# XiYe20/NPVP

Hardware: AMD Instinct MI355X
Metric: predictor train frames/sec (higher is better)
Workload: dtype f32 (two-term fp16 split of amax-scaled operands, 3 MFMAs per product, fp32 accumulate: fp32-grade; small GEMMs: three-term bf16 split)

## Files before the change

include/npvp_hip.h:

```cpp
#ifndef NPVP_HIP_H
#define NPVP_HIP_H
#include <stddef.h>
#ifdef __cplusplus
extern "C" {
#endif

typedef void* npvp_stream_t;

int npvp_version(void);
const char* npvp_last_error(void);
long long npvp_launch_count(void);
void* npvp_stream_create_low_priority(int* least, int* greatest);
int npvp_stream_destroy(void* stream);
void* npvp_event_create(void);
int npvp_event_record(void* event, void* stream);
float npvp_event_elapsed_ms(void* event0, void* event1);
int npvp_event_destroy(void* event);

long long npvp_graph_node_counts(void* graph, long long* counts, long long* memset_bytes, int max_memsets);

long long npvp_gemm_workspace_bytes(int M, int N, int K);
int npvp_gemm_kernel_id(int a_kc, int b_kc, int M, int N, int K, int precision, int has_planes);
int npvp_gemm_route(int a_kc, int b_kc, int M, int N, int K, int precision, int has_planes, int plain_epilogue, int* out4);
int npvp_gemm_f32(int a_kc, int b_kc, int M, int N, int K, const float* A, long long lda, const float* B, long long ldb,
                  float* C, long long ldc, const float* bias, int act, const float* aux_in, float* aux_out,
                  const float* residual, long long ldr, float drop_p, int drop_mode, int drop_g1, int drop_g2,
                  const unsigned long long* seed, unsigned int salt, float alpha, int precision, float* colsum_a,
                  const void* b_pre, int accumulate, float* rowstats, const float* a_amax, const float* b_amax,
                  float* c_amax, unsigned int* range_flag, float adrop_p, int adrop_g1, int adrop_g2, unsigned int adrop_salt,
                  void* workspace, long long ws_bytes, npvp_stream_t stream);
int npvp_frame_stats_finalize(const float* part, int parts_per_frame, float values_per_part, float* mean, float* rstd,
                              int frames, float eps, npvp_stream_t stream);
int npvp_split_weight(const float* w, long long ld, int N, int K, void* F, void* D, npvp_stream_t stream);
int npvp_split_weights_batched(const void* desc, int count, npvp_stream_t stream);
int npvp_amax(const float* x, long long rows, long long cols, long long ld, float* slot, npvp_stream_t stream);

typedef struct npvp_reduce_job {
  const float* ws; float* out; long long ldc; int M, N, splits, accum; float alpha; int blocks; const float* cs_part; float* cs_out;
} npvp_reduce_job_t;
int npvp_wgrad_f16_chainable(int M, int N, int K);
long long npvp_wgrad_f16_chain_workspace_bytes(int M, int N, int K);
int npvp_wgrad_f16_chained(int M, int N, int K, const float* dy, long long lda, const float* x, long long ldb, float* dw,
                           long long ldc, float* db, int accumulate, const float* a_amax, const float* b_amax,
                           unsigned int* range_flag, float adrop_p, int adrop_g1, int adrop_g2, unsigned int adrop_salt,
                           const unsigned long long* seed, const void* prev_job, void* my_job, void* workspace,
                           long long ws_bytes, npvp_stream_t stream);
int npvp_splitk_reduce_job(const void* job, npvp_stream_t stream);
int npvp_splitk_reduce_multi(const void* jobs, int n, npvp_stream_t stream);
int npvp_linear_bwd_f16_takes(int R, int N, int K);
int npvp_linear_bwd_f16(int R, int N, int K, const float* dy, long long ldy, const float* dy_amax, const void* w_planes_d,
                        const float* w_amax, float* dx, long long ldx, int act, const float* aux_in, const float* residual,
                        long long ldr, float drop_p, int drop_mode, int drop_g1, int drop_g2, unsigned int drop_salt, float* dx_amax,
                        const float* x, long long ldxx, const float* x_amax, float* dw, long long ldw, float* db,
                        unsigned int* range_flag, float adrop_p, int adrop_g1, int adrop_g2, unsigned int adrop_salt,
                        const unsigned long long* seed, const void* prev_job, void* my_job, void* workspace, long long ws_bytes,
                        npvp_stream_t stream);
int npvp_split_weight_f16(const float* w, long long ld, int N, int K, void* F, void* D, float* amax_slot, npvp_stream_t stream);
int npvp_split_weights_f16(const void* desc, int count, void* amax_table, long long amax_bytes, npvp_stream_t stream);

int npvp_layernorm_fwd(const float* x, const float* w, const float* b, float* y, float* mean, float* rstd, long long rows,
                       int C, float eps, int relu, float* y_amax, npvp_stream_t stream);
long long npvp_layernorm_bwd_workspace_bytes(long long rows, int C);
int npvp_layernorm_bwd(const float* dy, const float* x, const float* w, const float* b, const float* mean,
                       const float* rstd, float* dx, float* dw, float* db, long long rows, int C, int relu,
                       const float* dres ,
                       int accumulate , float* dx_amax,
                       void* workspace, long long ws_bytes, npvp_stream_t stream);
int npvp_layernorm_bwd_reduce(const void* workspace, float* dw, float* db, long long rows, int C, int accumulate,
                              npvp_stream_t stream);

int npvp_layernorm_bwd_reduce_job(const void* workspace, float* dw, float* db, long long rows, int C, int accumulate, void* job);
int npvp_frameln_act_bwd_reduce_job(const void* workspace, float* dw, float* db, int frames, int per_frame, int accumulate, void* job);
int npvp_mlpdw_mid_bwd_reduce_job(const void* workspace, float* gw, float* gb, int frames, int Ch, void* job);
int npvp_sum_rows_multi(const void* jobs, int n, npvp_stream_t stream);

int npvp_layernorm_nchw_fwd(const float* x, const float* w, const float* b, float* out_nchw, float* mean, float* rstd, int frames,
                            int P, int C, float eps, int relu, npvp_stream_t stream);

int npvp_frame_stats(const float* x, const float* add, float* mean, float* rstd, int frames, int T, int per_frame,
                     float eps, npvp_stream_t stream);
int npvp_posfuse_fwd(const float* x, const float* add, const float* beta, const float* gamma, float* y, float* mean,
                     float* rstd, int N, int T, int per_frame, float eps, float* y_amax, npvp_stream_t stream);
int npvp_ln_posfuse_fwd(const float* x, const float* lw, const float* lb, float ln_eps, float* y1, float* ln_mean, float* ln_rstd,
// ... 5 lines not shown
                     int accumulate, void* workspace, long long ws_bytes , npvp_stream_t stream);

int npvp_posfuse_instance_fwd(const float* x, const float* add, const float* beta, const float* gamma, float* y, float* mean,
                              float* rstd, int N, int T, int P, int C, float eps, float* y_amax, npvp_stream_t stream);
int npvp_posfuse_instance_bwd(const float* dy, const float* x, const float* add, const float* gamma, const float* mean,
                              const float* rstd, float* du, float* dyxh, int N, int T, int P, int C, npvp_stream_t stream);

int npvp_frameln_act_fwd(const float* h, const float* mean, const float* rstd, const float* w, const float* b,
                         const float* res, float* out, int frames, int per_frame, float drop_p, unsigned int salt,
                         float dp_p, unsigned int dp_salt, int frames_per_sample, const unsigned long long* seed,
                         float* out_amax, npvp_stream_t stream);
long long npvp_frameln_act_bwd_workspace_bytes(int frames, int per_frame);
int npvp_frameln_act_bwd(const float* dout, const float* h, const float* mean, const float* rstd, const float* w,
                         const float* b, float* dh, float* dw, float* db, int frames, int per_frame, float drop_p,
                         unsigned int salt, float dp_p, unsigned int dp_salt, int frames_per_sample,
                         const unsigned long long* seed, int accumulate ,
                         float* dh_amax, void* workspace, long long ws_bytes, npvp_stream_t stream);
int npvp_frameln_act_bwd_reduce(const void* workspace, float* dw, float* db, int frames, int per_frame, int accumulate,
                                npvp_stream_t stream);
int npvp_dwconv3x3(const float* a, const float* wt, const float* bias, float* out, int frames, int H, int W, int Ch,
                   int flip, npvp_stream_t stream);
int npvp_dwconv3x3_stats(const float* a, const float* wt, const float* bias, float* out, float* mean, float* rstd, int frames,
                         int H, int W, int Ch, float eps, void* workspace, long long ws_bytes, npvp_stream_t stream);
int npvp_mlpdw_mid_fwd(const float* h1, const float* mean1, const float* rstd1, const float* w1n, const float* b1n,
                       const float* wt, const float* bias, float* h2, float* mean2, float* rstd2, int frames, int H, int W,
                       int Ch, float eps, void* workspace, long long ws_bytes, npvp_stream_t stream);
int npvp_mlpdw_mid_fwd_parts(const float* h1, const float* part1, int J1, float nb1, float* mean1, float* rstd1, const float* w1n,
                             const float* b1n, const float* wt, const float* bias, float* h2, float* part2, int frames, int H,
                             int W, int Ch, float eps, npvp_stream_t stream);
int npvp_frameln_act_fwd_parts(const float* h, const float* part, int J, float nb, float eps, float* mean, float* rstd,
                               const float* w, const float* b, const float* res, float* out, int frames, int per_frame,
                               float drop_p, unsigned int salt, float dp_p, unsigned int dp_salt, int frames_per_sample,
                               const unsigned long long* seed, float* out_amax, npvp_stream_t stream);
long long npvp_mlpdw_mid_bwd_workspace_bytes(int frames, int Ch);
int npvp_mlpdw_mid_bwd(const float* dh2, const float* h1, const float* mean1, const float* rstd1, const float* w1n,
                       const float* b1n, const float* wt, float* da1, float* dwt_db, float* psum, int frames, int H, int W,
                       int Ch, int accumulate, void* workspace, long long ws_bytes, npvp_stream_t stream);
int npvp_mlpdw_mid_bwd_reduce(const void* workspace, float* dwt_db, int frames, int Ch, int accumulate, npvp_stream_t stream);
int npvp_mlpdw_mid_bwd_reduce_into(const void* workspace, float* gw, float* gb, int frames, int Ch, npvp_stream_t stream);
int npvp_mlpdw_mid_bwd_n2(const float* da2, const float* h2, const float* mean2, const float* rstd2, const float* w2n,
                          const float* b2n, const float* psum2, int nparts2, float drop_p, unsigned int salt,
                          const unsigned long long* seed, const float* h1, const float* mean1, const float* rstd1,
                          const float* w1n, const float* b1n, const float* wt, float* da1, float* dwt_db, float* psum, int frames,
                          int H, int W, int Ch, int accumulate, void* workspace, long long ws_bytes, npvp_stream_t stream);
int npvp_frameln_act_bwd_pgrad(const float* dout, const float* h, const float* mean, const float* rstd, const float* w,
                               const float* b, float* psum, float* dw, float* db, int frames, int per_frame, float drop_p,
                               unsigned int salt, float dp_p, unsigned int dp_salt, int frames_per_sample,
                               const unsigned long long* seed, int accumulate, void* workspace, long long ws_bytes,
                               npvp_stream_t stream);
int npvp_frameln_act_bwd_apply(const float* dout, const float* h, const float* mean, const float* rstd, const float* w,
                               const float* b, const float* psum, int nparts, float* dh, float* dw, float* db, int frames,
                               int per_frame, int accumulate, float* dh_amax, void* workspace, long long ws_bytes,
                               npvp_stream_t stream);

int npvp_im2col3x3(const float* in, float* out, int frames, int H, int W, int C, int col2im, npvp_stream_t stream);
long long npvp_dwconv3x3_wgrad_workspace_bytes(int frames, int Ch);
int npvp_dwconv3x3_wgrad(const float* a, const float* dout, float* dwt_db, int frames, int H, int W, int Ch,
                         void* workspace, long long ws_bytes, npvp_stream_t stream);

int npvp_attn_fwd(const float* q, long long ld_q, const float* k, long long ld_k, const float* v, long long ld_v, float* o,
                  long long ld_o, int mode, int dim0, int P, int W, int ws, int Tq, int Tk, int heads, int head_dim,
                  int mask_mode, float drop_p, const unsigned long long* seed, unsigned int salt, float* o_amax,
                  npvp_stream_t stream);
int npvp_attn_bwd(const float* q, long long ld_q, const float* k, long long ld_k, const float* v, long long ld_v,
                  const float* go, long long ld_o, float* dq, long long ld_dq, float* dk, long long ld_dk, float* dv,
                  long long ld_dv, int mode, int dim0, int P, int W, int ws, int Tq, int Tk, int heads, int head_dim,
                  int mask_mode, float drop_p, const unsigned long long* seed, unsigned int salt, float* dq_amax,
                  float* dk_amax , float* dv_amax,
                  npvp_stream_t stream);
int npvp_attn_long_fwd(const float* q, long long ld_q, const float* k, long long ld_k, const float* v, long long ld_v, float* o,
                       long long ld_o, int mode, int dim0, int P, int W, int ws, int Tq, int Tk, int heads, int head_dim,
                       int mask_mode, float drop_p, const unsigned long long* seed, unsigned int salt, float* o_amax,
                       npvp_stream_t stream);
long long npvp_attn_long_bwd_workspace_bytes(int mode, int dim0, int P, int W, int ws, int Tq, int Tk, int heads);
int npvp_attn_long_bwd(const float* q, long long ld_q, const float* k, long long ld_k, const float* v, long long ld_v,
                       const float* go, long long ld_o, float* dq, long long ld_dq, float* dk, long long ld_dk, float* dv,
                       long long ld_dv, int mode, int dim0, int P, int W, int ws, int Tq, int Tk, int heads, int head_dim,
                       int mask_mode, float drop_p, const unsigned long long* seed, unsigned int salt, float* dq_amax,
                       float* dk_amax , float* dv_amax, void* workspace, long long ws_bytes,
                       npvp_stream_t stream);

int npvp_drop_apply(const float* x, float* out, long long rows, int ncols, float p, int mode, int g1, int g2,
                    const unsigned long long* seed, unsigned int salt, float* out_amax, npvp_stream_t stream);
int npvp_transpose(const float* in, float* out, int batch, int R, int C, npvp_stream_t stream);
int npvp_dwtb_accumulate(const float* dwtb, float* gw, float* gb, int C, npvp_stream_t stream);
int npvp_dwtb_build(const float* w, const float* b, float* wtb, int C, npvp_stream_t stream);
int npvp_reduce_mid(const float* in, float* out, int A, int B, long long Cc, float scale, int accumulate, npvp_stream_t stream);
int npvp_broadcast_mid(const float* in, float* out, int A, int B, long long Cc, float scale, npvp_stream_t stream);

long long npvp_colsum_workspace_bytes(long long rows, int N);
int npvp_colsum(const float* x, long long rows, int N, long long ld, float* out, int accumulate ,
                void* workspace, long long ws_bytes, npvp_stream_t stream);

int npvp_l1_mean(const float* a, const float* b, long long n, float lam, float* out, void* workspace, long long ws_bytes,
                 npvp_stream_t stream);
int npvp_l1_mean_bwd(const float* a, const float* b, long long n, const float* gout, float lam, float* da, npvp_stream_t stream);
int npvp_sum_all(const float* x, long long n, float* out, void* workspace, long long ws_bytes, npvp_stream_t stream);

int npvp_grad_norm_clip(const float* g, long long n, float max_norm, float* out2, void* workspace, long long ws_bytes,
                        npvp_stream_t stream);
int npvp_adamw_step(float* p, float* g, float* m, float* v, long long n, const float* hyper, float beta1, float beta2,
                    float eps, float weight_decay, const float* clip, long long clip_begin, long long clip_end,
                    int write_back_grad, npvp_stream_t stream);

long long npvp_sqdiff_workspace_bytes(int N, long long per_image);
int npvp_sqdiff_per_image(const float* x, const float* y, int N, long long per_image, float data_range, float scale, float* out,
// ... 56 lines not shown
```

npvp_amd/_lib.py:

```python
import ctypes
import os

_HERE = os.path.dirname(os.path.abspath(__file__))
LIB_PATH = os.path.join(_HERE, "libnpvp_hip.so")

c_int, c_ll, c_f, c_u, c_p = ctypes.c_int, ctypes.c_longlong, ctypes.c_float, ctypes.c_uint, ctypes.c_void_p

SIGNATURES = {
    "npvp_version": (c_int, []),
    "npvp_last_error": (ctypes.c_char_p, []),
    "npvp_launch_count": (c_ll, []),
    "npvp_dp_unique_id": (c_int, [c_p]),
    "npvp_dp_init": (c_int, [c_int, c_int, c_p]),
    "npvp_dp_world": (c_int, []),
    "npvp_dp_rank": (c_int, []),
    "npvp_dp_allreduce_async": (c_int, [c_p, c_ll, c_p]),
    "npvp_dp_wait": (c_int, [c_p]),
    "npvp_dp_finalize": (c_int, []),
    "npvp_stream_create_low_priority": (c_p, [c_p, c_p]),
    "npvp_stream_destroy": (c_int, [c_p]),
    "npvp_event_create": (c_p, []),
    "npvp_event_record": (c_int, [c_p, c_p]),
    "npvp_event_elapsed_ms": (c_f, [c_p, c_p]),
    "npvp_event_destroy": (c_int, [c_p]),
    "npvp_graph_node_counts": (c_ll, [c_p, c_p, c_p, c_int]),
    "npvp_gemm_workspace_bytes": (c_ll, [c_int, c_int, c_int]),
    "npvp_gemm_kernel_id": (c_int, [c_int, c_int, c_int, c_int, c_int, c_int, c_int]),
    "npvp_gemm_route": (c_int, [c_int, c_int, c_int, c_int, c_int, c_int, c_int, c_int, c_p]),
    "npvp_gemm_f32": (c_int, [c_int, c_int, c_int, c_int, c_int, c_p, c_ll, c_p, c_ll, c_p, c_ll, c_p, c_int, c_p, c_p,
                              c_p, c_ll, c_f, c_int, c_int, c_int, c_p, c_u, c_f, c_int, c_p, c_p, c_int, c_p, c_p, c_p, c_p, c_p,
                              c_f, c_int, c_int, c_u, c_p, c_ll, c_p]),
    "npvp_amax": (c_int, [c_p, c_ll, c_ll, c_ll, c_p, c_p]),
    "npvp_wgrad_f16_chainable": (c_int, [c_int, c_int, c_int]),
    "npvp_wgrad_f16_chain_workspace_bytes": (c_ll, [c_int, c_int, c_int]),
    "npvp_wgrad_f16_chained": (c_int, [c_int, c_int, c_int, c_p, c_ll, c_p, c_ll, c_p, c_ll, c_p, c_int, c_p, c_p, c_p, c_f, c_int, c_int,
                                       c_u, c_p, c_p, c_p, c_p, c_ll, c_p]),
    "npvp_splitk_reduce_job": (c_int, [c_p, c_p]),
    "npvp_splitk_reduce_multi": (c_int, [c_p, c_int, c_p]),
    "npvp_linear_bwd_f16_takes": (c_int, [c_int, c_int, c_int]),
    "npvp_linear_bwd_f16": (c_int, [c_int, c_int, c_int, c_p, c_ll, c_p, c_p, c_p, c_p, c_ll, c_int, c_p, c_p, c_ll, c_f, c_int, c_int, c_int,
                                    c_u, c_p, c_p, c_ll, c_p, c_p, c_ll, c_p, c_p, c_f, c_int, c_int, c_u, c_p, c_p, c_p, c_p, c_ll, c_p]),
    "npvp_split_weight_f16": (c_int, [c_p, c_ll, c_int, c_int, c_p, c_p, c_p, c_p]),
    "npvp_split_weights_f16": (c_int, [c_p, c_int, c_p, c_ll, c_p]),
    "npvp_frame_stats_finalize": (c_int, [c_p, c_int, c_f, c_p, c_p, c_int, c_f, c_p]),
    "npvp_split_weight": (c_int, [c_p, c_ll, c_int, c_int, c_p, c_p, c_p]),
    "npvp_split_weights_batched": (c_int, [c_p, c_int, c_p]),
    "npvp_layernorm_fwd": (c_int, [c_p, c_p, c_p, c_p, c_p, c_p, c_ll, c_int, c_f, c_int, c_p, c_p]),
    "npvp_layernorm_bwd_workspace_bytes": (c_ll, [c_ll, c_int]),
    "npvp_layernorm_bwd": (c_int, [c_p, c_p, c_p, c_p, c_p, c_p, c_p, c_p, c_p, c_ll, c_int, c_int, c_p, c_int, c_p, c_p, c_ll, c_p]),
    "npvp_layernorm_bwd_reduce": (c_int, [c_p, c_p, c_p, c_ll, c_int, c_int, c_p]),
    "npvp_layernorm_bwd_reduce_job": (c_int, [c_p, c_p, c_p, c_ll, c_int, c_int, c_p]),
    "npvp_frameln_act_bwd_reduce_job": (c_int, [c_p, c_p, c_p, c_int, c_int, c_int, c_p]),
    "npvp_mlpdw_mid_bwd_reduce_job": (c_int, [c_p, c_p, c_p, c_int, c_int, c_p]),
    "npvp_sum_rows_multi": (c_int, [c_p, c_int, c_p]),
    "npvp_layernorm_nchw_fwd": (c_int, [c_p, c_p, c_p, c_p, c_p, c_p, c_int, c_int, c_int, c_f, c_int, c_p]),
    "npvp_frameln_act_bwd_reduce": (c_int, [c_p, c_p, c_p, c_int, c_int, c_int, c_p]),
    "npvp_frame_stats": (c_int, [c_p, c_p, c_p, c_p, c_int, c_int, c_int, c_f, c_p]),
    "npvp_posfuse_fwd": (c_int, [c_p, c_p, c_p, c_p, c_p, c_p, c_p, c_int, c_int, c_int, c_f, c_p, c_p]),
    "npvp_posfuse_instance_fwd": (c_int, [c_p, c_p, c_p, c_p, c_p, c_p, c_p, c_int, c_int, c_int, c_int, c_f, c_p, c_p]),
    "npvp_posfuse_instance_bwd": (c_int, [c_p, c_p, c_p, c_p, c_p, c_p, c_p, c_p, c_int, c_int, c_int, c_int, c_p]),
    "npvp_ln_posfuse_fwd": (c_int, [c_p, c_p, c_p, c_f, c_p, c_p, c_p, c_p, c_p, c_p, c_p, c_p, c_p, c_int, c_int, c_int, c_int, c_f,
                                    c_p, c_p, c_p]),
    "npvp_posfuse_bwd_fused": (c_int, [c_int, c_int, c_int]),
    "npvp_posfuse_bwd": (c_int, [c_p, c_p, c_p, c_p, c_p, c_p, c_p, c_p, c_p, c_p, c_int, c_int, c_int, c_int, c_p, c_ll, c_p]),
    "npvp_frameln_act_fwd": (c_int, [c_p, c_p, c_p, c_p, c_p, c_p, c_p, c_int, c_int, c_f, c_u, c_f, c_u, c_int, c_p, c_p, c_p]),
    "npvp_frameln_act_bwd_workspace_bytes": (c_ll, [c_int, c_int]),
    "npvp_frameln_act_bwd": (c_int, [c_p, c_p, c_p, c_p, c_p, c_p, c_p, c_p, c_p, c_int, c_int, c_f, c_u, c_f, c_u, c_int,
                                     c_p, c_int, c_p, c_p, c_ll, c_p]),
    "npvp_dwconv3x3": (c_int, [c_p, c_p, c_p, c_p, c_int, c_int, c_int, c_int, c_int, c_p]),
    "npvp_dwconv3x3_stats": (c_int, [c_p, c_p, c_p, c_p, c_p, c_p, c_int, c_int, c_int, c_int, c_f, c_p, c_ll, c_p]),
    "npvp_mlpdw_mid_fwd": (c_int, [c_p, c_p, c_p, c_p, c_p, c_p, c_p, c_p, c_p, c_p, c_int, c_int, c_int, c_int, c_f, c_p, c_ll, c_p]),
    "npvp_mlpdw_mid_fwd_parts": (c_int, [c_p, c_p, c_int, c_f, c_p, c_p, c_p, c_p, c_p, c_p, c_p, c_p, c_int, c_int, c_int, c_int, c_f, c_p]),
    "npvp_frameln_act_fwd_parts": (c_int, [c_p, c_p, c_int, c_f, c_f, c_p, c_p, c_p, c_p, c_p, c_p, c_int, c_int, c_f, c_u, c_f, c_u, c_int,
                                           c_p, c_p, c_p]),
    "npvp_mlpdw_mid_bwd_workspace_bytes": (c_ll, [c_int, c_int]),
    "npvp_mlpdw_mid_bwd": (c_int, [c_p, c_p, c_p, c_p, c_p, c_p, c_p, c_p, c_p, c_p, c_int, c_int, c_int, c_int, c_int, c_p, c_ll, c_p]),
    "npvp_mlpdw_mid_bwd_reduce": (c_int, [c_p, c_p, c_int, c_int, c_int, c_p]),
    "npvp_mlpdw_mid_bwd_reduce_into": (c_int, [c_p, c_p, c_p, c_int, c_int, c_p]),
    "npvp_mlpdw_mid_bwd_n2": (c_int, [c_p, c_p, c_p, c_p, c_p, c_p, c_p, c_int, c_f, c_u, c_p, c_p, c_p, c_p, c_p, c_p, c_p, c_p, c_p,
                                      c_p, c_int, c_int, c_int, c_int, c_int, c_p, c_ll, c_p]),
    "npvp_frameln_act_bwd_pgrad": (c_int, [c_p, c_p, c_p, c_p, c_p, c_p, c_p, c_p, c_p, c_int, c_int, c_f, c_u, c_f, c_u, c_int,
                                           c_p, c_int, c_p, c_ll, c_p]),
    "npvp_frameln_act_bwd_apply": (c_int, [c_p, c_p, c_p, c_p, c_p, c_p, c_p, c_int, c_p, c_p, c_p, c_int, c_int, c_int, c_p, c_p, c_ll, c_p]),
    "npvp_im2col3x3": (c_int, [c_p, c_p, c_int, c_int, c_int, c_int, c_int, c_p]),
    "npvp_dwconv3x3_wgrad_workspace_bytes": (c_ll, [c_int, c_int]),
    "npvp_dwconv3x3_wgrad": (c_int, [c_p, c_p, c_p, c_int, c_int, c_int, c_int, c_p, c_ll, c_p]),
    "npvp_attn_fwd": (c_int, [c_p, c_ll, c_p, c_ll, c_p, c_ll, c_p, c_ll, c_int, c_int, c_int, c_int, c_int, c_int, c_int,
                              c_int, c_int, c_int, c_f, c_p, c_u, c_p, c_p]),
    "npvp_attn_bwd": (c_int, [c_p, c_ll, c_p, c_ll, c_p, c_ll, c_p, c_ll, c_p, c_ll, c_p, c_ll, c_p, c_ll, c_int, c_int,
                              c_int, c_int, c_int, c_int, c_int, c_int, c_int, c_int, c_f, c_p, c_u, c_p, c_p, c_p, c_p]),
    "npvp_attn_long_fwd": (c_int, [c_p, c_ll, c_p, c_ll, c_p, c_ll, c_p, c_ll, c_int, c_int, c_int, c_int, c_int, c_int, c_int,
                                   c_int, c_int, c_int, c_f, c_p, c_u, c_p, c_p]),
    "npvp_attn_long_bwd_workspace_bytes": (c_ll, [c_int, c_int, c_int, c_int, c_int, c_int, c_int, c_int]),
    "npvp_attn_long_bwd": (c_int, [c_p, c_ll, c_p, c_ll, c_p, c_ll, c_p, c_ll, c_p, c_ll, c_p, c_ll, c_p, c_ll, c_int, c_int,
                                   c_int, c_int, c_int, c_int, c_int, c_int, c_int, c_int, c_f, c_p, c_u, c_p, c_p, c_p, c_p, c_ll, c_p]),
    "npvp_drop_apply": (c_int, [c_p, c_p, c_ll, c_int, c_f, c_int, c_int, c_int, c_p, c_u, c_p, c_p]),
    "npvp_transpose": (c_int, [c_p, c_p, c_int, c_int, c_int, c_p]),
    "npvp_dwtb_accumulate": (c_int, [c_p, c_p, c_p, c_int, c_p]),
    "npvp_dwtb_build": (c_int, [c_p, c_p, c_p, c_int, c_p]),
    "npvp_reduce_mid": (c_int, [c_p, c_p, c_int, c_int, c_ll, c_f, c_int, c_p]),
    "npvp_broadcast_mid": (c_int, [c_p, c_p, c_int, c_int, c_ll, c_f, c_p]),
    "npvp_colsum_workspace_bytes": (c_ll, [c_ll, c_int]),
    "npvp_colsum": (c_int, [c_p, c_ll, c_int, c_ll, c_p, c_int, c_p, c_ll, c_p]),
    "npvp_grad_norm_clip": (c_int, [c_p, c_ll, c_f, c_p, c_p, c_ll, c_p]),
    "npvp_l1_mean": (c_int, [c_p, c_p, c_ll, c_f, c_p, c_p, c_ll, c_p]),
    "npvp_l1_mean_bwd": (c_int, [c_p, c_p, c_ll, c_p, c_f, c_p, c_p]),
    "npvp_sum_all": (c_int, [c_p, c_ll, c_p, c_p, c_ll, c_p]),
    "npvp_adamw_step": (c_int, [c_p, c_p, c_p, c_p, c_ll, c_p, c_f, c_f, c_f, c_f, c_p, c_ll, c_ll, c_int, c_p]),
    "npvp_sqdiff_workspace_bytes": (c_ll, [c_int, c_ll]),
    "npvp_sqdiff_per_image": (c_int, [c_p, c_p, c_int, c_ll, c_f, c_f, c_p, c_p, c_ll, c_p]),
    "npvp_ssim_workspace_bytes": (c_ll, [c_int, c_int, c_int, c_int]),
    "npvp_u8hwc_to_f32chw": (c_int, [c_p, c_p, c_ll, c_int, c_int, c_int, c_p, c_p, c_p]),
    "npvp_bias_act": (c_int, [c_p, c_p, c_p, c_p, c_ll, c_ll, c_int, c_int, c_int, c_p]),
    "npvp_act_bwd": (c_int, [c_p, c_p, c_p, c_ll, c_int, c_p]),
    "npvp_bn_workspace_bytes": (c_int, [c_int]),
    "npvp_bn_stats": (c_int, [c_p, c_ll, c_ll, c_int, c_int, c_p, c_p, c_ll, c_p]),
    "npvp_bn_act_apply": (c_int, [c_p, c_p, c_p, c_p, c_p, c_ll, c_f, c_f, c_p, c_p, c_ll, c_ll, c_int, c_int, c_int, c_p, c_p, c_p, c_p]),
    "npvp_bn_act_bwd": (c_int, [c_p, c_p, c_p, c_p, c_p, c_p, c_ll, c_ll, c_int, c_int, c_int, c_int, c_p, c_p, c_p, c_p, c_ll, c_p]),
    "npvp_bn_act_apply_sync": (c_int, [c_p, c_p, c_p, c_p, c_p, c_f, c_f, c_p, c_p, c_ll, c_ll, c_int, c_int, c_int, c_p, c_p, c_p, c_p]),
    "npvp_bn_bwd_sums": (c_int, [c_p, c_p, c_p, c_p, c_p, c_p, c_ll, c_ll, c_int, c_int, c_int, c_p, c_p, c_p, c_p, c_ll, c_p]),
    "npvp_bn_act_bwd_apply": (c_int, [c_p, c_p, c_p, c_p, c_p, c_p, c_p, c_p, c_ll, c_ll, c_int, c_int, c_int, c_p, c_p]),
    "npvp_reflect_pad": (c_int, [c_p, c_p, c_int, c_int, c_int, c_int, c_int, c_int, c_int, c_p]),
    "npvp_nonlocal_attn_fwd": (c_int, [c_p, c_ll, c_p, c_ll, c_p, c_ll, c_p, c_ll, c_p, c_int, c_int, c_int, c_int, c_int, c_p]),
    "npvp_nonlocal_attn_bwd": (c_int, [c_p, c_ll, c_p, c_ll, c_p, c_ll, c_p, c_ll, c_p, c_p, c_p, c_ll, c_p, c_ll, c_p, c_ll, c_int, c_int,
                                       c_int, c_int, c_int, c_p]),
    "npvp_nonlocal_attn_grid_fwd": (c_int, [c_p, c_ll, c_p, c_ll, c_p, c_ll, c_p, c_ll, c_p, c_int, c_int, c_int, c_int, c_int, c_p]),
    "npvp_nonlocal_attn_grid_bwd": (c_int, [c_p, c_ll, c_p, c_ll, c_p, c_ll, c_p, c_ll, c_p, c_p, c_p, c_ll, c_p, c_ll, c_p, c_ll, c_int,
                                            c_int, c_int, c_int, c_int, c_p]),
    "npvp_ssim_per_image": (c_int, [c_p, c_p, c_int, c_int, c_int, c_int, c_p, c_int, c_p, c_p, c_ll, c_p]),
}

_lib = None


def lib():
    global _lib
# ... 39 lines not shown
```

npvp_amd/csrc/common.h:

```cpp
#pragma once
#include <hip/hip_runtime.h>
#include <stdint.h>

#define NPVP_OK 0
#define NPVP_ERR_ARG (-1)
#define NPVP_ERR_LAUNCH (-2)
#define NPVP_ERR_WORKSPACE (-3)

extern "C" void npvp_set_error(const char* msg);

extern "C" long long npvp_launch_count(void);
namespace npvp { extern long long g_launches; }
#define NPVP_LAUNCH(...)                                                    \
  do {                                                                      \
    __atomic_fetch_add(&npvp::g_launches, 1ll, __ATOMIC_RELAXED);           \
    hipLaunchKernelGGL(__VA_ARGS__);                                        \
  } while (0)

#define NPVP_CHECK_ARG(cond, msg)                    \
  do {                                               \
    if (!(cond)) {                                   \
      npvp_set_error(msg);                           \
      return NPVP_ERR_ARG;                           \
    }                                                \
// ... 134 lines not shown
__host__ __device__ __forceinline__ uint32_t mix32(uint32_t h) {
  h ^= h >> 16; h *= 0x85ebca6bu;
  h ^= h >> 13; h *= 0xc2b2ae35u;
  h ^= h >> 16;
  return h;
}
__host__ __device__ __forceinline__ uint32_t rng_u32(uint64_t seed, uint32_t salt, uint64_t idx) {
  const uint32_t k0 = mix32((uint32_t)seed ^ mix32(salt * 0x9e3779b9u + 0x7f4a7c15u));
  const uint32_t k1 = mix32((uint32_t)(seed >> 32) + mix32(salt ^ 0x85ebca6bu));
  const uint32_t h = mix32((uint32_t)idx ^ k0);
  return mix32(h + k1 + (uint32_t)(idx >> 32) * 0x9e3779b9u);
}
__device__ __forceinline__ float drop_scale(uint64_t seed, uint32_t salt, uint64_t idx, uint32_t thresh, float inv_keep) {
  return rng_u32(seed, salt, idx) >= thresh ? inv_keep : 0.f;
}
__host__ __device__ __forceinline__ uint32_t drop_threshold(float p) {
  double t = (double)p * 4294967296.0;
  if (t < 0) t = 0;
  if (t > 4294967295.0) t = 4294967295.0;
  return (uint32_t)t;
}

struct DropSpec {
  unsigned int thresh; float inv_keep; unsigned int salt; int mode; int g1; int g2;
  unsigned int m1, m2; int s1, s2;
};
__host__ __device__ __forceinline__ void div_magic(unsigned int d, unsigned int& m, int& s) {
  int l = 0;
  while (l < 31 && (1u << l) < d) ++l;
  s = 31 + l;
  m = (unsigned int)(((1ull << s) + d - 1ull) / d);
}
__device__ __forceinline__ unsigned int div_by_magic(unsigned int n, unsigned int m, int s) {
  return (unsigned int)(((unsigned long long)n * m) >> s);
}
__device__ __forceinline__ unsigned int drop_group(const DropSpec& d, long long row) {
  const unsigned int q1 = div_by_magic((unsigned int)row, d.m1, d.s1);
  return q1 - div_by_magic(q1, d.m2, d.s2) * (unsigned int)d.g2;
}
__device__ __forceinline__ float drop_spec_scale(const DropSpec& d, uint64_t seed, long long row, int col, int ncols) {
  const uint64_t key = d.mode == 0 ? (uint64_t)row * (uint64_t)ncols + (uint64_t)col : (uint64_t)drop_group(d, row);
  return rng_u32(seed, d.salt, key) >= d.thresh ? d.inv_keep : 0.f;
}
inline DropSpec make_drop_spec(float p, unsigned int salt, int mode, int g1, int g2) {
  DropSpec d;
  d.thresh = p > 0.f ? drop_threshold(p) : 0u;
  d.inv_keep = p > 0.f ? 1.f / (1.f - p) : 1.f;
  d.salt = salt; d.mode = mode; d.g1 = g1 > 0 ? g1 : 1; d.g2 = g2 > 0 ? g2 : 1;
  div_magic((unsigned int)d.g1, d.m1, d.s1);
  div_magic((unsigned int)d.g2, d.m2, d.s2);
  return d;
}

__device__ __forceinline__ float4 ld4(const float* p) { return *reinterpret_cast<const float4*>(p); }
__device__ __forceinline__ void st4(float* p, float4 v) { *reinterpret_cast<float4*>(p) = v; }

}
```

npvp_amd/csrc/gemm.h:

```cpp
#pragma once
#include <type_traits>
#include "common.h"

namespace npvp {

typedef float f32x16 __attribute__((ext_vector_type(16)));
typedef __bf16 bf16x8 __attribute__((ext_vector_type(8)));
typedef __bf16 bf16x4 __attribute__((ext_vector_type(4)));

struct ReduceJob {
  const float* ws; float* out; long long ldc; int M, N, splits, accum; float alpha; int blocks; const float* cs_part; float* cs_out;
};

struct GemmParams {
  const float* A; const float* B; float* C;
  const float* bias;
  const float* residual;
  float* aux_out;
  const float* aux_in;
  float* rowstats;
  float* colsum;
  const unsigned long long* seed;
  long long lda, ldb, ldc, ldr;
  int M, N, K;
  int act;
  DropSpec drop;
  DropSpec adrop;
  int tiles_m, tiles_n;
  int splits;
  float alpha;
  const void* b_pre;
  long long b_pre_plane;
  int colgroups;
  int accum;
  const float* a_amax; const float* b_amax; float* c_amax;
  unsigned int* range_flag;
  ReduceJob prev;
};

__device__ __forceinline__ void splitk_reduce_body(const ReduceJob& j, int bid, int nblocks, float& cmax) {
  const long long total4 = (long long)j.M * j.N / 4, cs4 = j.cs_out ? j.M / 4 : 0;
  for (long long i = (long long)bid * 256 + threadIdx.x; i < total4 + cs4; i += (long long)nblocks * 256) {
    if (i >= total4) {
      const long long e = (i - total4) * 4;
      float4 s = make_float4(0.f, 0.f, 0.f, 0.f);
      for (int zz = 0; zz < j.splits; ++zz) {
        const float4 v = ld4(j.cs_part + (long long)zz * j.M + e);
        s.x += v.x; s.y += v.y; s.z += v.z; s.w += v.w;
      }
      if (j.accum) { const float4 o = ld4(j.cs_out + e); s.x += o.x; s.y += o.y; s.z += o.z; s.w += o.w; }
      st4(j.cs_out + e, s);
      continue;
    }
    const long long e = i * 4;
    const int m = (int)(e / j.N), n = (int)(e - (long long)m * j.N);
    float4 s = make_float4(0.f, 0.f, 0.f, 0.f);
    for (int zz = 0; zz < j.splits; ++zz) {
      const float4 v = ld4(j.ws + (long long)zz * j.M * j.N + e);
      s.x += v.x; s.y += v.y; s.z += v.z; s.w += v.w;
    }
    s.x *= j.alpha; s.y *= j.alpha; s.z *= j.alpha; s.w *= j.alpha;
    if (j.accum) { const float4 o = ld4(j.out + (long long)m * j.ldc + n); s.x += o.x; s.y += o.y; s.z += o.z; s.w += o.w; }
    st4(j.out + (long long)m * j.ldc + n, s);
    cmax = amax4(cmax, s);
  }
}

__device__ __forceinline__ void store_colsum(const GemmParams& p, long long idx, float v) {
  p.colsum[idx] = (p.accum && p.splits == 1) ? p.colsum[idx] + v : v;
}

constexpr int EPI_LD = 36;
constexpr int EPI_FLOATS = 32 * EPI_LD;

__device__ __forceinline__ void epi_transpose(const f32x16& acc, float* scr, int lane, float4 (&v)[4]) {
  const int r = lane & 31, h = lane >> 5;
#pragma unroll
  for (int g = 0; g < 16; ++g) scr[(((g & 3) + 8 * (g >> 2)) + 4 * h) * EPI_LD + r] = acc[g];
  const int rr = lane >> 3, cq = lane & 7;
#pragma unroll
// ... 236 lines not shown
```

npvp_amd/csrc/gemm.hip:

```cpp
#include "gemm.h"
#include "partials.h"
#include <type_traits>

namespace npvp {

constexpr int BM = 128, BN = 128, BK = 32, GEMM_THREADS = 256;

template <bool KC> struct Stager;

template <> struct Stager<true> {
  static constexpr int LD = 129;
  float4 r[4];
  __device__ __forceinline__ void load(const float* src, long long ld, int row0, int nrows, int k0) {
    const int t = threadIdx.x;
    const int kc = (t & 7) * 4;
#pragma unroll
    for (int i = 0; i < 4; ++i) {
      const int row = row0 + (t >> 3) + 32 * i;
      r[i] = (row < nrows) ? ld4(src + (long long)row * ld + k0 + kc) : make_float4(0.f, 0.f, 0.f, 0.f);
    }
  }
  __device__ __forceinline__ void store(float* s) const {
    const int t = threadIdx.x;
    const int kc = (t & 7) * 4;
// ... 443 lines not shown
  const int M = f.M, N = f.N, K = f.K;
  const bool want_h = f.precision == 6;
  const int precision = want_h ? 4 : f.precision;
  int s128 = pick_splits(M, N, K);
  if (s128 > 1 && (!f.plain || f.ws_bytes < npvp_gemm_workspace_bytes(M, N, K))) s128 = 1;
  const bool planes_ok = f.planes && f.a_kc && K % 16 == 0 && N % 8 == 0;
  const bool wgrad = !f.a_kc && !f.b_kc && f.plain && !f.rowstats;
  auto fits = [&](int s) { return s == 1 || (s > 1 && f.ws_bytes >= splitk_workspace_bytes(s, M, N)); };
  GemmPlan pl = {precision == 0 ? 0 : 1, 0, s128, 0, false};
  int v = 0, s = 0;
  if (want_h && planes_ok && f.amax && (v = gemm_f16_variant(M, N, K)) != 0) {
    pl.id = v == 1 ? 5 : 7; pl.variant = v; pl.splits = 1; pl.planes = true;
  } else if (want_h && wgrad && f.amax && fits(s = f16_wgrad_splits(M, N, K))) {
    pl.id = 6; pl.splits = s;
  } else if (!want_h && precision == 4 && planes_ok && s128 == 1 && (v = wide_variant(M, N, K)) != 0) {
    pl.id = v == 1 ? 2 : 4; pl.variant = v; pl.planes = true;
  } else if (precision == 4 && wgrad && fits(s = wide_wgrad_splits(M, N, K))) {
    pl.id = 3; pl.splits = s;
  } else {
    pl.planes = !want_h && precision == 4 && planes_ok && s128 == 1 && !f.rowstats;
  }
  pl.steps = K / pl.splits / (precision == 0 ? BK : 16);
  return pl;
}

static GemmPlan plan_query(int a_kc, int b_kc, int M, int N, int K, int precision, int has_planes, bool plain) {
  return plan_gemm(GemmFacts{a_kc, b_kc, M, N, K, precision, has_planes != 0, plain, true, false, npvp_gemm_workspace_bytes(M, N, K)});
}

extern "C" int npvp_gemm_kernel_id(int a_kc, int b_kc, int M, int N, int K, int precision, int has_planes) {
  return plan_query(a_kc, b_kc, M, N, K, precision, has_planes, true).id;
}

extern "C" int npvp_gemm_route(int a_kc, int b_kc, int M, int N, int K, int precision, int has_planes, int plain_epilogue, int* out4) {
  NPVP_CHECK_ARG(out4 && M > 0 && N > 0 && K > 0, "gemm_route: empty problem or no result array");
  NPVP_CHECK_ARG(precision == 0 || precision == 4 || precision == 5 || precision == 6, "gemm_route: precision must be 0, 4, 5 or 6");
  NPVP_CHECK_ARG(K % BK == 0 && M % 4 == 0 && N % 4 == 0 && !(a_kc == 0 && b_kc == 1), "gemm_route: not a problem npvp_gemm_f32 accepts");
  const GemmPlan r = plan_query(a_kc, b_kc, M, N, K, precision, has_planes, plain_epilogue != 0);
  out4[0] = r.id; out4[1] = r.variant; out4[2] = r.splits; out4[3] = r.steps;
  return NPVP_OK;
}

static int finish_splitk(const GemmParams& p, float* C, long long ldc, float* colsum_a, hipStream_t stream) {
  const long long total4 = (long long)p.M * p.N / 4;
  int blocks = (int)((total4 + 255) / 256); if (blocks > 2048) blocks = 2048;
  const bool cs_here = colsum_a && ((uintptr_t)colsum_a % 16) == 0;
  NPVP_LAUNCH(splitk_reduce_kernel, dim3(blocks), dim3(256), 0, stream, (const float*)p.C, C, p.M, p.N, ldc, p.splits, p.alpha,
              p.accum, cs_here ? (const float*)p.colsum : nullptr, cs_here ? colsum_a : nullptr, p.c_amax);
  NPVP_CHECK_LAUNCH();
  if (!colsum_a || cs_here) return NPVP_OK;
  return finish_partials(make_partials(p.colsum, 0, p.splits, p.splits, p.M, colsum_a, p.accum).job, 0, stream, "gemm: column-sum reduce launch failed");
}

extern "C" int npvp_gemm_f32(int a_kc, int b_kc, int M, int N, int K, const float* A, long long lda, const float* B,
                             long long ldb, float* C, long long ldc, const float* bias, int act, const float* aux_in,
                             float* aux_out, const float* residual, long long ldr, float drop_p, int drop_mode,
                             int drop_g1, int drop_g2, const unsigned long long* seed, unsigned int salt, float alpha,
                             int precision, float* colsum_a, const void* b_pre, int accumulate, float* rowstats,
                             const float* a_amax, const float* b_amax, float* c_amax, unsigned int* range_flag,
                             float adrop_p, int adrop_g1, int adrop_g2, unsigned int adrop_salt,
                             void* workspace, long long ws_bytes, hipStream_t stream) {
  NPVP_CHECK_ARG(M > 0 && N > 0 && K > 0, "gemm: empty problem");
  NPVP_CHECK_ARG(precision == 0 || precision == 4 || precision == 5 || precision == 6,
                 "gemm: precision must be 0 (exact fp32-input MFMA), 4 (three-term bf16 split, 6 MFMAs per product: "
                 "fp32-grade), 5 (two-term bf16 split, 3 MFMAs per product, ~2^-16) or 6 (two-term fp16 split with amax-scaled "
                 "operands, 3 MFMAs per product: fp32-grade; shapes it does not take run as 4)");
  const bool want_h = precision == 6;
  NPVP_CHECK_ARG(K % BK == 0, "gemm: K must be a multiple of 32");
  NPVP_CHECK_ARG(M % 4 == 0 && N % 4 == 0, "gemm: M and N must be multiples of 4");
  NPVP_CHECK_ARG(((uintptr_t)A % 16) == 0 && ((uintptr_t)B % 16) == 0 && ((uintptr_t)C % 16) == 0, "gemm: pointers must be 16-byte aligned");
  NPVP_CHECK_ARG(lda % 4 == 0 && ldb % 4 == 0, "gemm: lda/ldb must be multiples of 4 floats");
  NPVP_CHECK_ARG(ldc % 4 == 0 && (!residual || (ldr % 4 == 0 && ((uintptr_t)residual % 16) == 0)) && (!bias || ((uintptr_t)bias % 16) == 0) &&
                 (!aux_in || ((uintptr_t)aux_in % 16) == 0) && (!aux_out || ((uintptr_t)aux_out % 16) == 0),
                 "gemm: ldc / ldr must be multiples of 4 floats and bias / aux / residual 16-byte aligned (float4 epilogue)");
  NPVP_CHECK_ARG(!(a_kc == 0 && b_kc == 1), "gemm: (a_kc=0,b_kc=1) is not used by the path");
  NPVP_CHECK_ARG((act != 3 && act != 4) || aux_in, "gemm: act 3/4 need aux_in");
  NPVP_CHECK_ARG(drop_p >= 0.f && drop_p < 1.f, "gemm: dropout p out of range");
  NPVP_CHECK_ARG(drop_p == 0.f || seed, "gemm: dropout needs a device seed");
  NPVP_CHECK_ARG(!colsum_a || a_kc == 0, "gemm: colsum_a is the column sum of a [K][M] operand (a_kc = 0)");
  NPVP_CHECK_ARG(!b_pre || ((uintptr_t)b_pre % 16) == 0, "gemm: b_pre must be 16-byte aligned");

  NPVP_CHECK_ARG(adrop_p >= 0.f && adrop_p < 0.5f, "gemm: adrop_p must be in [0, 0.5) (the masked operand must stay inside its amax scale)");
  NPVP_CHECK_ARG(adrop_p == 0.f || (seed && want_h && adrop_g1 > 0 && adrop_g2 > 0 && (a_kc || adrop_g1 % 16 == 0)),
                 "gemm: adrop needs precision 6, a device seed and (for a weight gradient) groups of a multiple of 16 rows");
  NPVP_CHECK_ARG(!rowstats || ((precision == 4 || want_h) && a_kc && b_kc && M % 64 == 0 && N % 128 == 0 && act == 0 && !aux_out && !residual &&
                               drop_p == 0.f && !accumulate),
                 "gemm: rowstats needs the default (bf16x6) forward layout, M % 64 == 0, N % 128 == 0 and a bias-only epilogue");

  const bool plain = !bias && act == 0 && !aux_out && !residual && drop_p == 0.f;
  const GemmPlan plan = plan_gemm(GemmFacts{a_kc, b_kc, M, N, K, precision, b_pre != nullptr, plain,
                                            a_amax && b_amax, rowstats != nullptr, workspace ? ws_bytes : 0});
  NPVP_CHECK_ARG(adrop_p == 0.f || plan.id >= 5, "gemm: adrop was requested but this shape does not run on the fp16 kernels (npvp_gemm_kernel_id tells)");

  GemmParams p;
  p.A = A; p.B = B; p.bias = bias; p.residual = residual; p.aux_out = aux_out; p.aux_in = aux_in;
  p.seed = seed; p.lda = lda; p.ldb = ldb; p.ldr = ldr; p.M = M; p.N = N; p.act = act;
  p.drop = make_drop_spec(drop_p, salt, drop_mode, drop_g1, drop_g2);
  p.adrop = make_drop_spec(adrop_p, adrop_salt, 1, adrop_g1, adrop_g2);
  p.alpha = alpha;
  p.rowstats = rowstats;
  p.a_amax = a_amax; p.b_amax = b_amax; p.c_amax = c_amax; p.range_flag = range_flag;
  p.prev = ReduceJob{};
  p.accum = accumulate ? 1 : 0;
  p.b_pre = plan.planes ? b_pre : nullptr;
  p.b_pre_plane = (long long)N * K;
  p.splits = plan.splits;
  if (plan.splits > 1) aim_at_workspace(p, K, plan.splits, workspace, colsum_a != nullptr);
  else { p.K = K; p.C = C; p.ldc = ldc; p.colsum = colsum_a; }
  p.tiles_m = (M + BM - 1) / BM; p.tiles_n = (N + BN - 1) / BN;
  p.colgroups = (plan.id <= 1 && plan.splits == 1) ? pick_colgroups((long long)N * K * 4, p.tiles_m, p.tiles_n) : 1;

  const dim3 grid(p.tiles_m * p.tiles_n, plan.splits), block(GEMM_THREADS);
  switch (plan.id) {
    case 5: case 7: launch_gemm_f16(p, plan.variant, stream); break;
    case 6: launch_gemm_wgrad_f16(p, stream); break;
    case 2: case 4: launch_gemm_wide(p, plan.variant, stream); break;
    case 3: launch_gemm_wgrad_wide(p, stream); break;
    case 0:
      if (a_kc && b_kc) NPVP_LAUNCH((gemm_f32_kernel<true, true>), grid, block, 0, stream, p);
      else if (a_kc) NPVP_LAUNCH((gemm_f32_kernel<true, false>), grid, block, 0, stream, p);
      else NPVP_LAUNCH((gemm_f32_kernel<false, false>), grid, block, 0, stream, p);
      break;
    default:
      if (precision == 5) {
        if (a_kc && b_kc) NPVP_LAUNCH((gemm_split_db_kernel<2, true, true, false>), grid, block, 0, stream, p);
        else if (a_kc) NPVP_LAUNCH((gemm_split_db_kernel<2, true, false, false>), grid, block, 0, stream, p);
        else NPVP_LAUNCH((gemm_split_db_kernel<2, false, false, false>), grid, block, 0, stream, p);
      } else if (rowstats) NPVP_LAUNCH((gemm_split_db_kernel<3, true, true, false, true>), grid, block, 0, stream, p);
      else if (plan.planes) NPVP_LAUNCH((gemm_split_db_kernel<3, true, true, true>), grid, block, 0, stream, p);
      else if (a_kc && b_kc) NPVP_LAUNCH((gemm_split_db_kernel<3, true, true, false>), grid, block, 0, stream, p);
      else if (a_kc) NPVP_LAUNCH((gemm_split_db_kernel<3, true, false, false>), grid, block, 0, stream, p);
      else NPVP_LAUNCH((gemm_split_db_kernel<3, false, false, false>), grid, block, 0, stream, p);
  }
  NPVP_CHECK_LAUNCH();
  return plan.splits > 1 ? finish_splitk(p, C, ldc, colsum_a, stream) : NPVP_OK;
}
```

npvp_amd/csrc/gemm_f16.hip:

```cpp
#include "gemm.h"
#include <cstdlib>

namespace npvp {

typedef _Float16 f16x8 __attribute__((ext_vector_type(8)));
typedef _Float16 f16x4 __attribute__((ext_vector_type(4)));
typedef __attribute__((address_space(1))) const void* gptr_t;
typedef __attribute__((address_space(3))) void* lptr_t;
typedef float f32x4 __attribute__((ext_vector_type(4)));

__device__ __forceinline__ void split_f16_scaled(const f32x4 v, const float s, f16x4& hi, f16x4& lo) {
  unsigned int h01, h23, l01, l23;
  asm("v_fma_mixlo_f16 %0, %1, %2, 0" : "=v"(h01) : "v"(v[0]), "v"(s));
  asm("v_fma_mixlo_f16 %0, %1, %2, 0" : "=v"(h23) : "v"(v[2]), "v"(s));
  asm("v_fma_mixhi_f16 %0, %1, %2, 0" : "+v"(h01) : "v"(v[1]), "v"(s));
  asm("v_fma_mixhi_f16 %0, %1, %2, 0" : "+v"(h23) : "v"(v[3]), "v"(s));
  asm("v_fma_mixlo_f16 %0, %1, %2, -%3 op_sel_hi:[0,0,1]" : "=v"(l01) : "v"(v[0]), "v"(s), "v"(h01));
  asm("v_fma_mixlo_f16 %0, %1, %2, -%3 op_sel_hi:[0,0,1]" : "=v"(l23) : "v"(v[2]), "v"(s), "v"(h23));
  asm("v_fma_mixhi_f16 %0, %1, %2, -%3 op_sel:[0,0,1] op_sel_hi:[0,0,1]" : "+v"(l01) : "v"(v[1]), "v"(s), "v"(h01));
  asm("v_fma_mixhi_f16 %0, %1, %2, -%3 op_sel:[0,0,1] op_sel_hi:[0,0,1]" : "+v"(l23) : "v"(v[3]), "v"(s), "v"(h23));
  typedef unsigned int u32x2 __attribute__((ext_vector_type(2)));
  const u32x2 hp = {h01, h23}, lp = {l01, l23};
  hi = __builtin_bit_cast(f16x4, hp);
  lo = __builtin_bit_cast(f16x4, lp);
}

template <int NW>
__device__ __forceinline__ bool block_any(bool pred, int* flags, int wave) {
  const bool w = __builtin_amdgcn_ballot_w64(pred) != 0ull;
  if ((threadIdx.x & 63) == 0) flags[wave] = w ? 1 : 0;
  __syncthreads();
  int any = 0;
#pragma unroll
  for (int i = 0; i < NW; ++i) any |= flags[i];
  __syncthreads();
  return __builtin_amdgcn_readfirstlane(any) != 0;
}

template <int TM, int TN, int WM, int WN, int NST>
constexpr int gemm_f16_lds_bytes() {
  constexpr int NW = WM * WN, BM = WM * TM * 32, BN = WN * TN * 32;
  constexpr int STAGE = 2 * 2 * (BM * 16 + 64) + 2 * 2 * (BN * 16);
  constexpr int EPI_BYTES = (4 + NW * EPI_FLOATS + BM) * 4;
  return NST * STAGE > EPI_BYTES ? NST * STAGE : EPI_BYTES;
}

template <int TM, int TN, int WM, int WN, bool ROWSTATS, int NST>
__device__ __forceinline__ void gemm_f16_body(const GemmParams& p, char* lds, const int bid, const int nwg) {
  constexpr int NW = WM * WN, THREADS = 64 * NW;
  constexpr int BM = WM * TM * 32, BN = WN * TN * 32;
  constexpr int APASS = BM / (THREADS / 4);
  static_assert((APASS == 1 || APASS == 2) && BN % 64 == 0, "A staging: a thread stages one or two rows of the tile");
  constexpr int KGS_A = BM * 16 + 64, A_PLANE = 2 * KGS_A, A_BYTES = 2 * A_PLANE;
  constexpr int KGS_B = BN * 16, B_PLANE = 2 * KGS_B, B_BYTES = 2 * B_PLANE;
  constexpr int STAGE = A_BYTES + B_BYTES;
  constexpr int CPS = BN / 64;
  constexpr int NCHUNK = 4 * CPS, CPW = (NCHUNK + NW - 1) / NW;
  static_assert(NST == 2 || NST == 3, "two or three LDS stages");
  static_assert(gemm_f16_lds_bytes<TM, TN, WM, WN, NST>() >= NST * STAGE, "lds size formula");

  int tile_m, tile_n;
  tile_of_block_unsplit(p, nwg, bid, tile_m, tile_n);
  const int m0 = tile_m * BM, n0 = tile_n * BN;
  const int t = threadIdx.x, lane = t & 63, wave = __builtin_amdgcn_readfirstlane(t >> 6);
  const int wm = wave / WN, wn = wave % WN, r = lane & 31, h = lane >> 5;
  const int nk = p.K >> 4;
  const float sa = amax_scale(amax_slot_read(p.a_amax));
  const unsigned int cpeek = amax_peek_block(p.c_amax);

  f32x16 acc[TM][TN];

  const int quad = t & 3, rl = t >> 2;
  const char* a_base = reinterpret_cast<const char*>(p.A + (long long)m0 * p.lda);
  const unsigned int a_off0 = (unsigned int)(((long long)(min(m0 + rl, p.M - 1) - m0) * p.lda + 4 * quad) * 4);
  const unsigned int a_off1 = (unsigned int)(((long long)(min(m0 + rl + BM / 2, p.M - 1) - m0) * p.lda + 4 * quad) * 4);
  const int a_dst = (quad >> 1) * KGS_A + (quad & 1) * 8 + rl * 16;
  float sa0 = sa, sa1 = sa;
  if (p.adrop.thresh) {
    const unsigned long long aseed = *p.seed;
    sa0 *= drop_spec_scale(p.adrop, aseed, min(m0 + rl, p.M - 1), 0, 1);
    sa1 *= drop_spec_scale(p.adrop, aseed, min(m0 + rl + BM / 2, p.M - 1), 0, 1);
  }
  const char* b_base = reinterpret_cast<const char*>(p.b_pre);
  unsigned int b_off[CPW];
  int b_dst[CPW];
#pragma unroll
  for (int i = 0; i < CPW; ++i) {
    const int c = wave + NW * i;
    const int slab = c / CPS, part = c - slab * CPS, s = slab >> 1, kg = slab & 1;
    const int col = min(n0 + part * 64 + lane, p.N - 1);
    b_off[i] = (unsigned int)(((long long)s * (p.b_pre_plane >> 3) + (long long)kg * p.N + col) * 16);
    b_dst[i] = A_BYTES + s * B_PLANE + kg * KGS_B + part * 1024;
  }
  const long long b_step = 32ll * p.N;
  const unsigned int lds_u32 = (unsigned int)(size_t)((lptr_t)lds);

  const int fa_off = h * KGS_A + (wm * TM * 32 + r) * 16;
  const int fb_off = A_BYTES + h * KGS_B + (wn * TN * 32 + r) * 16;

  f32x4 ea0, ea1 = {0.f, 0.f, 0.f, 0.f}, eb0, eb1 = {0.f, 0.f, 0.f, 0.f};
#define NPVP_H_ALOAD(R0, R1, KT)                                                                           \
  { const char* ab_ = a_base + ((long long)min((KT), nk - 1) << 6);                                        \
    asm volatile("global_load_dwordx4 %0, %1, %2" : "=v"(R0) : "v"(a_off0), "s"(ab_) : "memory");          \
    if constexpr (APASS == 2) asm volatile("global_load_dwordx4 %0, %1, %2" : "=v"(R1) : "v"(a_off1), "s"(ab_) : "memory"); }
#define NPVP_H_WAIT_BUT_NEWEST(...)                                                                        \
  { if constexpr (APASS == 2) asm volatile("s_waitcnt vmcnt(2) lgkmcnt(0)" : __VA_ARGS__ :: "memory");     \
    else asm volatile("s_waitcnt vmcnt(1) lgkmcnt(0)" : __VA_ARGS__ :: "memory"); }
#define NPVP_H_WAIT_BUT_THIS_STEP(...)                                                                     \
  asm volatile("s_waitcnt vmcnt(%2) lgkmcnt(0)" : __VA_ARGS__ : "n"(CPW + APASS) : "memory");
#define NPVP_H_ASTORE(ST, V, ROWOFF)                                                     \
  { if (ROWOFF) rm1 = fmaxf(fmaxf(rm1, fmaxf(fabsf((V)[0]), fabsf((V)[1]))), fmaxf(fabsf((V)[2]), fabsf((V)[3])));  \
    else rm0 = fmaxf(fmaxf(rm0, fmaxf(fabsf((V)[0]), fabsf((V)[1]))), fmaxf(fabsf((V)[2]), fabsf((V)[3])));         \
    f16x4 hi_, lo_; split_f16_scaled((V), (ROWOFF) ? sa1 : sa0, hi_, lo_);               \
    *reinterpret_cast<f16x4*>((ST) + a_dst + (ROWOFF)) = hi_;                            \
    *reinterpret_cast<f16x4*>((ST) + A_PLANE + a_dst + (ROWOFF)) = lo_; }
#define NPVP_H_BLOAD(ST, KT)                                                             \
  { const char* bb_ = b_base + (long long)min((KT), nk - 1) * b_step;                    \
    _Pragma("unroll") for (int i_ = 0; i_ < CPW; ++i_)                                   \
      if (NCHUNK % NW == 0 || wave + NW * i_ < NCHUNK) {                                 \
        const unsigned int m0_ = lds_u32 + (unsigned int)((ST) - lds) + (unsigned int)b_dst[i_];          \
        asm volatile("s_mov_b32 m0, %0\n\ts_nop 0\n\tglobal_load_lds_dwordx4 %1, %2"                     \
                     :: "s"(m0_), "v"(b_off[i_]), "s"(bb_) : "memory", "m0"); } }
  static_assert(NCHUNK % NW == 0, "the hand-counted waits assume CPW LDS-DMA pieces per wave and step");

  __shared__ int guard_flags[NW];
  float rm0 = 0.f, rm1 = 0.f;
  bool rescued = false;
  const float zrow = 1.f;
  float rf0 = zrow, rf1 = zrow;
  const f32x16 zero16 = {0.f, 0.f, 0.f, 0.f, 0.f, 0.f, 0.f, 0.f, 0.f, 0.f, 0.f, 0.f, 0.f, 0.f, 0.f, 0.f};
  auto run_tile = [&]() __attribute__((always_inline)) {
  NPVP_H_BLOAD(lds, 0)
  NPVP_H_ALOAD(ea0, ea1, 0)
  asm volatile("s_waitcnt vmcnt(0)" : "+v"(ea0), "+v"(ea1) :: "memory");
  NPVP_H_ASTORE(lds, ea0, 0)
  if constexpr (APASS == 2) NPVP_H_ASTORE(lds, ea1, (BM / 2) * 16)
  if constexpr (NST == 3) NPVP_H_BLOAD(lds + STAGE, 1)
  NPVP_H_ALOAD(ea0, ea1, 1)
  NPVP_H_ALOAD(eb0, eb1, 2)
  NPVP_H_WAIT_BUT_NEWEST("+v"(ea0), "+v"(ea1))
  __builtin_amdgcn_s_barrier();

#define NPVP_H_STEP(KT, CUR, NXT, R0, R1, RN0, RN1) NPVP_H_STEP_(KT, CUR, NXT, NXT, R0, R1, RN0, RN1, false)
#define NPVP_H_STEP3(KT, CUR, NXT, B2, R0, R1, RN0, RN1) NPVP_H_STEP_(KT, CUR, NXT, B2, R0, R1, RN0, RN1, false)
#define NPVP_H_STEP_(KT, CUR, NXT, B2, R0, R1, RN0, RN1, FIRST)                                            \
  {                                                                                                        \
    const char* st_ = lds + (CUR) * STAGE;                                                                 \
    char* nx_ = lds + (NXT) * STAGE;                                                                       \
    NPVP_H_BLOAD(lds + (B2) * STAGE, (KT) + (NST - 1))                                                     \
    f16x8 fb_[2][TN];                                                                                      \
    _Pragma("unroll") for (int s_ = 0; s_ < 2; ++s_)                                                       \
      _Pragma("unroll") for (int j_ = 0; j_ < TN; ++j_)                                                    \
        fb_[s_][j_] = *reinterpret_cast<const f16x8*>(st_ + fb_off + s_ * B_PLANE + j_ * 512);             \
    _Pragma("unroll") for (int i_ = 0; i_ < TM; ++i_) {                                                    \
      f16x8 fa_[2];                                                                                        \
      _Pragma("unroll") for (int s_ = 0; s_ < 2; ++s_)                                                     \
        fa_[s_] = *reinterpret_cast<const f16x8*>(st_ + fa_off + s_ * A_PLANE + i_ * 512);                 \
      if (i_ == 0) { NPVP_H_ASTORE(nx_, R0, 0) if constexpr (APASS == 2) NPVP_H_ASTORE(nx_, R1, (BM / 2) * 16) } \
      if (i_ == TM - 1) { NPVP_H_ALOAD(R0, R1, (KT) + 3) }                                                 \
                                                                                 \
      _Pragma("unroll") for (int j_ = 0; j_ < TN; ++j_) acc[i_][j_] = __builtin_amdgcn_mfma_f32_32x32x16_f16(fa_[1], fb_[0][j_], (FIRST) ? zero16 : acc[i_][j_], 0, 0, 0); \
      _Pragma("unroll") for (int j_ = 0; j_ < TN; ++j_) acc[i_][j_] = __builtin_amdgcn_mfma_f32_32x32x16_f16(fa_[0], fb_[1][j_], acc[i_][j_], 0, 0, 0); \
      _Pragma("unroll") for (int j_ = 0; j_ < TN; ++j_) acc[i_][j_] = __builtin_amdgcn_mfma_f32_32x32x16_f16(fa_[0], fb_[0][j_], acc[i_][j_], 0, 0, 0); \
    }                                                                                                      \
    __builtin_amdgcn_sched_barrier(0);        \
    if constexpr (NST == 3) { NPVP_H_WAIT_BUT_THIS_STEP("+v"(RN0), "+v"(RN1)) }                            \
    else { NPVP_H_WAIT_BUT_NEWEST("+v"(RN0), "+v"(RN1)) }                                                  \
    __builtin_amdgcn_s_barrier();                                                                          \
  }

  if constexpr (NST == 2) {
  NPVP_H_STEP_(0, 0, 1, 1, ea0, ea1, eb0, eb1, true)
  int kt = 1;
  for (; kt + 1 < nk; kt += 2) {
    NPVP_H_STEP(kt, 1, 0, eb0, eb1, ea0, ea1)
    NPVP_H_STEP(kt + 1, 0, 1, ea0, ea1, eb0, eb1)
  }
  if (kt < nk) NPVP_H_STEP(kt, 1, 0, eb0, eb1, ea0, ea1)
  } else {
  NPVP_H_STEP_(0, 0, 1, 2, ea0, ea1, eb0, eb1, true)
  int kt = 1;
  for (; kt + 5 < nk; kt += 6) {
    NPVP_H_STEP3(kt, 1, 2, 0, eb0, eb1, ea0, ea1)
    NPVP_H_STEP3(kt + 1, 2, 0, 1, ea0, ea1, eb0, eb1)
    NPVP_H_STEP3(kt + 2, 0, 1, 2, eb0, eb1, ea0, ea1)
    NPVP_H_STEP3(kt + 3, 1, 2, 0, ea0, ea1, eb0, eb1)
    NPVP_H_STEP3(kt + 4, 2, 0, 1, eb0, eb1, ea0, ea1)
    NPVP_H_STEP3(kt + 5, 0, 1, 2, ea0, ea1, eb0, eb1)
  }
  if (kt < nk) NPVP_H_STEP3(kt, 1, 2, 0, eb0, eb1, ea0, ea1)
  if (kt + 1 < nk) NPVP_H_STEP3(kt + 1, 2, 0, 1, ea0, ea1, eb0, eb1)
  if (kt + 2 < nk) NPVP_H_STEP3(kt + 2, 0, 1, 2, eb0, eb1, ea0, ea1)
  if (kt + 3 < nk) NPVP_H_STEP3(kt + 3, 1, 2, 0, ea0, ea1, eb0, eb1)
  if (kt + 4 < nk) NPVP_H_STEP3(kt + 4, 2, 0, 1, eb0, eb1, ea0, ea1)
  }
  asm volatile("s_waitcnt vmcnt(0)" : "+v"(ea0), "+v"(ea1), "+v"(eb0), "+v"(eb1) :: "memory");
  if constexpr (NST == 3) __builtin_amdgcn_s_barrier();
  };
  run_tile();
  {
    rm0 = fmaxf(rm0, __shfl_xor(rm0, 1)); rm0 = fmaxf(rm0, __shfl_xor(rm0, 2));
    rm1 = fmaxf(rm1, __shfl_xor(rm1, 1)); rm1 = fmaxf(rm1, __shfl_xor(rm1, 2));
    const int et = (int)((__float_as_uint(sa) >> 23) & 0xffu);
    const int e0 = (int)((__float_as_uint(rm0) >> 23) & 0xffu), e1 = (int)((__float_as_uint(rm1) >> 23) & 0xffu);
    const int d0 = 268 - et - e0, d1 = 268 - et - e1;
    const bool ok0 = e0 >= 16 && e0 != 255 && d0 > 0 && d0 <= 120, ok1 = e1 >= 16 && e1 != 255 && d1 > 0 && d1 <= 120;
    if (block_any<NW>((ok0 && d0 >= 18) || (ok1 && d1 >= 18), guard_flags, wave)) {
      const float g0 = sa0 * pow2_recip(sa), g1 = sa1 * pow2_recip(sa);
      rf0 = ok0 ? __uint_as_float((unsigned int)(127 - d0) << 23) : 1.f;
      rf1 = ok1 ? __uint_as_float((unsigned int)(127 - d1) << 23) : 1.f;
      sa0 = (ok0 ? amax_scale(rm0) : sa) * g0;
      sa1 = (ok1 ? amax_scale(rm1) : sa) * g1;
      rescued = true;
      run_tile();
    }
  }
#undef NPVP_H_STEP
#undef NPVP_H_STEP3
#undef NPVP_H_WAIT_BUT_THIS_STEP
#undef NPVP_H_STEP_
#undef NPVP_H_BLOAD
#undef NPVP_H_ASTORE
#undef NPVP_H_ALOAD
#undef NPVP_H_WAIT_BUT_NEWEST

  const float ia = pow2_recip(sa), ib = pow2_recip(amax_scale(amax_slot_read(p.b_amax)));
  float alpha = p.alpha;
  {
    const float f = ia * ib, af = p.alpha * f, mag = fabsf(af);
    const bool fold = f >= 1.17549435e-38f && f <= 3.0e38f && ((mag >= 1.17549435e-38f && mag <= 3.0e38f) || p.alpha == 0.f);
    if (fold) alpha = af;
    else {
#pragma unroll
      for (int i = 0; i < TM; ++i)
#pragma unroll
        for (int j = 0; j < TN; ++j)
#pragma unroll
          for (int g = 0; g < 16; ++g) acc[i][j][g] = acc[i][j][g] * ia * ib;
    }
  }

  const int row_base = m0 + wm * TM * 32, col_base = n0 + wn * TN * 32;
  float cmax = 0.f;
  float* scr = reinterpret_cast<float*>(lds) + 4 + wave * EPI_FLOATS;
  if (rescued) {
    float* rowfac = reinterpret_cast<float*>(lds) + 4 + NW * EPI_FLOATS;
    if (quad == 0) { rowfac[rl] = rf0; if (APASS == 2) rowfac[rl + BM / 2] = rf1; }
    __syncthreads();
#pragma unroll
    for (int i = 0; i < TM; ++i)
#pragma unroll
      for (int g = 0; g < 16; ++g) {
        const float f = rowfac[wm * TM * 32 + i * 32 + (g & 3) + 8 * (g >> 2) + 4 * h];
// ... 556 lines not shown
```

npvp_amd/csrc/mlpdw.hip:

```cpp
#include "partials.h"
#include <cstring>
#include <cstdlib>

namespace npvp {

__global__ void dwconv3x3_kernel(const float* __restrict__ a, const float* __restrict__ wt, const float* __restrict__ bias,
                                 float* __restrict__ out, int H, int W, int Ch, long long total4, int flip) {
  const int c4n = Ch / 4, P = H * W;
  for (long long i = (long long)blockIdx.x * blockDim.x + threadIdx.x; i < total4; i += (long long)gridDim.x * blockDim.x) {
    const int c = (int)(i % c4n) * 4;
    const long long fp = i / c4n;
    const int p = (int)(fp % P);
    const long long f = fp / P;
    const int h = p / W, w = p - h * W;
    float4 acc = bias ? ld4(bias + c) : make_float4(0.f, 0.f, 0.f, 0.f);
    const float* af = a + f * P * Ch + c;
#pragma unroll
    for (int ky = -1; ky <= 1; ++ky) {
      const int hh = h + ky;
      if (hh < 0 || hh >= H) continue;
#pragma unroll
      for (int kx = -1; kx <= 1; ++kx) {
        const int ww = w + kx;
        if (ww < 0 || ww >= W) continue;
// ... 119 lines not shown
    for (int e = 0; e < VEC; ++e) r0[w].v[e] = 0.f;
  load_row(r1, 0);
  float shift = 0.f, s1 = 0.f, s2 = 0.f;
#pragma unroll 1
  for (int h = 0; h < HH; ++h) {
    if (h + 1 < HH) load_row(r2, h + 1);
    else {
#pragma unroll
      for (int w = 0; w < WW; ++w)
#pragma unroll
        for (int e = 0; e < VEC; ++e) r2[w].v[e] = 0.f;
    }
#pragma unroll
    for (int w = 0; w < WW; ++w) {
      Vec<VEC> acc = bv;
#pragma unroll
      for (int kx = -1; kx <= 1; ++kx) {
        const int ww = w + kx;
        if (ww < 0 || ww >= WW) continue;
#pragma unroll
        for (int e = 0; e < VEC; ++e)
          acc.v[e] += wv[kx + 1].v[e] * r0[ww].v[e] + wv[3 + kx + 1].v[e] * r1[ww].v[e] + wv[6 + kx + 1].v[e] * r2[ww].v[e];
      }
      stv<VEC>(of + (h * WW + w) * Ch + c, acc);
      if (h == 0 && w == 0) shift = acc.v[0];
#pragma unroll
      for (int e = 0; e < VEC; ++e) { const float a = acc.v[e] - shift; s1 += a; s2 += a * a; }
    }
#pragma unroll
    for (int w = 0; w < WW; ++w) { r0[w] = r1[w]; r1[w] = r2[w]; }
  }
  const float n = (float)(HH * WW * VEC), m1 = s1 / n, mean_t = shift + m1, m2_t = s2 - s1 * m1;
  const float mean_b = block_sum<4>(mean_t, red) / 256.f;
  const float d = mean_t - mean_b;
  const float m2_b = block_sum<4>(m2_t + n * d * d, red);
  if (threadIdx.x == 0) { part[blockIdx.x * 2] = mean_b; part[blockIdx.x * 2 + 1] = m2_b; }
}

#ifndef NPVP_MID_BWD_WAVES
#define NPVP_MID_BWD_WAVES 2
#endif
struct MidN2 {
  const float* h2; const float* mean2; const float* rstd2; const float* w2n; const float* b2n;
  const float* psum2; int nparts2;
  const unsigned long long* seed; unsigned int drop_thresh; float drop_inv_keep; unsigned int salt;
};

template <int VEC, bool FUSE2>
__global__ __launch_bounds__(256, NPVP_MID_BWD_WAVES) void mlpdw_mid_bwd_kernel(const float* __restrict__ dh2, const float* __restrict__ h1,
                                                            const float* __restrict__ mean1, const float* __restrict__ rstd1,
                                                            const float* __restrict__ w1n, const float* __restrict__ b1n,
                                                            const float* __restrict__ wt, float* __restrict__ da1,
                                                            float* __restrict__ part, float* __restrict__ psum, int Ch,
                                                            int frames, int frames_per_chunk, MidN2 n2) {
  constexpr int HH = 8, WW = 8;
  __shared__ float red[4];
  const unsigned long long seed2 = (FUSE2 && n2.seed && n2.drop_thresh) ? *n2.seed : 0ull;
  const int c = (blockIdx.x * blockDim.x + threadIdx.x) * VEC;
  const int nblk = gridDim.x;
  Vec<VEC> wv[9], aw[9], ab;
#pragma unroll
  for (int t = 0; t < 9; ++t) {
    wv[t] = ldv<VEC>(wt + t * Ch + c);
#pragma unroll
    for (int e = 0; e < VEC; ++e) aw[t].v[e] = 0.f;
  }
#pragma unroll
  for (int e = 0; e < VEC; ++e) ab.v[e] = 0.f;
  const int f0 = blockIdx.y * frames_per_chunk, f1 = min(frames, f0 + frames_per_chunk);
  for (long long f = f0; f < f1; ++f) {
    const float mu = mean1[f], rs = rstd1[f];
    const float* hf = h1 + f * (HH * WW) * Ch;
    const float* gf = dh2 + f * (HH * WW) * Ch;
    float* of = da1 + f * (HH * WW) * Ch;
    float mu2 = 0.f, rs2 = 0.f, c1 = 0.f, c2 = 0.f;
    const float* h2f = nullptr;
    if constexpr (FUSE2) {
      mu2 = n2.mean2[f]; rs2 = n2.rstd2[f];
      h2f = n2.h2 + f * (HH * WW) * Ch;
      const int j = threadIdx.x;
      const float p1 = j < n2.nparts2 ? n2.psum2[(f * n2.nparts2 + j) * 2] : 0.f;
      const float p2 = j < n2.nparts2 ? n2.psum2[(f * n2.nparts2 + j) * 2 + 1] : 0.f;
      const float inv = 1.f / (float)(HH * WW * Ch);
      c1 = block_sum<4>(p1, red) * inv;
      c2 = block_sum<4>(p2, red) * inv;
    }
    Vec<VEC> a0[WW], a1r[WW], a2[WW], g0[WW], g1[WW], g2[WW], gp1[WW], xh1[WW], gp2[WW], xh2[WW];
    auto load_row = [&](Vec<VEC>* arow, Vec<VEC>* grow, Vec<VEC>* gprow, Vec<VEC>* xhrow, int hh) {
      if constexpr (FUSE2) {
#pragma unroll
        for (int w0 = 0; w0 < WW; w0 += 4) {
#pragma unroll
          for (int w = w0; w < w0 + 4; ++w) {
            const int off = (hh * WW + w) * Ch + c;
            const Vec<VEC> d2 = ldv<VEC>(gf + off), x2 = ldv<VEC>(h2f + off), w2 = ldv<VEC>(n2.w2n + off), b2 = ldv<VEC>(n2.b2n + off);
#pragma unroll
            for (int e = 0; e < VEC; ++e) {
              const float xh2 = (x2.v[e] - mu2) * rs2;
              float m = 1.f;
              if (n2.drop_thresh)
                m = drop_scale(seed2, n2.salt, (unsigned long long)(f * (HH * WW) * Ch + off + e), n2.drop_thresh, n2.drop_inv_keep);
              const float dyln = d2.v[e] * m * gelu_grad_f(xh2 * w2.v[e] + b2.v[e]);
              grow[w].v[e] = rs2 * (dyln * w2.v[e] - c1 - xh2 * c2);
            }
          }
          __builtin_amdgcn_sched_barrier(0);
        }
      }
#pragma unroll
      for (int w = 0; w < WW; ++w) {
        const int pix = hh * WW + w, off = pix * Ch + c;
        const Vec<VEC> x = ldv<VEC>(hf + off), ww = ldv<VEC>(w1n + off), bb = ldv<VEC>(b1n + off);
        if constexpr (!FUSE2) grow[w] = ldv<VEC>(gf + off);
#pragma unroll
        for (int e = 0; e < VEC; ++e) {
          const float xh = (x.v[e] - mu) * rs, y = xh * ww.v[e] + bb.v[e];
          float E;
          const float phi = gelu_phi(y, E);
          arow[w].v[e] = y * phi;
          gprow[w].v[e] = fmaf(y * 0.39894228040143267794f, E, phi) * ww.v[e];
          xhrow[w].v[e] = xh;
        }
      }
    };
#pragma unroll
    for (int w = 0; w < WW; ++w)
#pragma unroll
// ... 227 lines not shown
  NPVP_CHECK_ARG(frames > 0 && H == 8 && W == 8 && Ch > 0 && Ch % 1024 == 0, "dwconv_stats: needs an 8x8 grid and Ch % 1024 == 0");
  const int J = Ch / 1024;
  NPVP_CHECK_ARG(workspace && ws_bytes >= (long long)frames * J * 8, "dwconv_stats: workspace too small");
  const long long nthreads = (long long)frames * (Ch / 4);
  NPVP_LAUNCH((dwconv3x3_win_kernel<8, 8, true>), dim3((unsigned)(nthreads / 256)), dim3(256), 0, stream, a, wt, bias, out,
                     Ch, nthreads, 0, (float*)workspace);
  NPVP_CHECK_LAUNCH();
  NPVP_LAUNCH(frame_stats_finalize_kernel, dim3((frames + 255) / 256), dim3(256), 0, stream, (const float*)workspace, J,
                     65536.f, mean, rstd, frames, eps);
  NPVP_CHECK_LAUNCH();
  return NPVP_OK;
}

extern "C" int npvp_mlpdw_mid_fwd(const float* h1, const float* mean1, const float* rstd1, const float* w1n, const float* b1n,
                                  const float* wt, const float* bias, float* h2, float* mean2, float* rstd2, int frames,
                                  int H, int W, int Ch, float eps, void* workspace, long long ws_bytes, hipStream_t stream) {
  NPVP_CHECK_ARG(frames > 0 && H == 8 && W == 8 && Ch > 0 && Ch % 512 == 0, "mlpdw_mid_fwd: needs an 8x8 grid and Ch % 512 == 0");
  const int J = Ch / 512;
  NPVP_CHECK_ARG(workspace && ws_bytes >= (long long)frames * J * 8, "mlpdw_mid_fwd: workspace too small");
  const long long nthreads = (long long)frames * (Ch / 2);
  NPVP_LAUNCH((mlpdw_mid_fwd_kernel<2>), dim3((unsigned)(nthreads / 256)), dim3(256), 0, stream, h1, mean1, rstd1, w1n, b1n,
                     wt, bias, h2, (float*)workspace, Ch, (const float*)nullptr, 0, 0.f, 0.f, (float*)nullptr, (float*)nullptr);
  NPVP_CHECK_LAUNCH();
  NPVP_LAUNCH(frame_stats_finalize_kernel, dim3((frames + 255) / 256), dim3(256), 0, stream, (const float*)workspace, J,
                     32768.f, mean2, rstd2, frames, eps);
  NPVP_CHECK_LAUNCH();
  return NPVP_OK;
}

extern "C" int npvp_mlpdw_mid_fwd_parts(const float* h1, const float* part1, int J1, float nb1, float* mean1, float* rstd1,
                                        const float* w1n, const float* b1n, const float* wt, const float* bias, float* h2,
                                        float* part2, int frames, int H, int W, int Ch, float eps, hipStream_t stream) {
  NPVP_CHECK_ARG(frames > 0 && H == 8 && W == 8 && Ch > 0 && Ch % 512 == 0, "mlpdw_mid_fwd_parts: needs an 8x8 grid and Ch % 512 == 0");
  NPVP_CHECK_ARG(part1 && J1 > 0 && nb1 > 0.f && mean1 && rstd1 && part2, "mlpdw_mid_fwd_parts: bad arguments");
  const long long nthreads = (long long)frames * (Ch / 2);
  NPVP_LAUNCH((mlpdw_mid_fwd_kernel<2>), dim3((unsigned)(nthreads / 256)), dim3(256), 0, stream, h1, (const float*)nullptr,
                     (const float*)nullptr, w1n, b1n, wt, bias, h2, part2, Ch, part1, J1, nb1, eps, mean1, rstd1);
  NPVP_CHECK_LAUNCH();
  return NPVP_OK;
}

static int mid_chunks(int frames) { return frames < 128 ? frames : 128; }

static Partials mid_partials(const void* ws, float* out, float* out_b, int frames, int Ch, int accumulate) {
  return make_partials(ws, 0, frames, mid_chunks(frames), 10 * Ch, out, accumulate, out_b, out_b ? Ch : 0, out_b ? 1 : 0);
}

extern "C" long long npvp_mlpdw_mid_bwd_workspace_bytes(int frames, int Ch) {
  return mid_partials(nullptr, nullptr, nullptr, frames, Ch, 0).bytes;
}

static int mid_bwd_launch(const float* dh2, const float* h1, const float* mean1, const float* rstd1, const float* w1n,
                          const float* b1n, const float* wt, float* da1, float* dwt_db, float* psum, int frames, int H, int W,
                          int Ch, int accumulate, void* workspace, long long ws_bytes, hipStream_t stream, const MidN2* n2) {
  NPVP_CHECK_ARG(frames > 0 && H == 8 && W == 8 && Ch > 0 && Ch % 512 == 0, "mlpdw_mid_bwd: needs an 8x8 grid and Ch % 512 == 0");
  NPVP_CHECK_ARG(workspace && ws_bytes >= npvp_mlpdw_mid_bwd_workspace_bytes(frames, Ch), "mlpdw_mid_bwd: workspace too small");
  const Partials P = mid_partials(workspace, dwt_db, nullptr, frames, Ch, accumulate);
  if (n2)
    NPVP_LAUNCH((mlpdw_mid_bwd_kernel<1, true>), dim3(Ch / 256, P.job.nb), dim3(256), 0, stream, dh2, h1, mean1, rstd1, w1n,
                       b1n, wt, da1, P.part(), psum, Ch, frames, P.per, *n2);
  else
    NPVP_LAUNCH((mlpdw_mid_bwd_kernel<1, false>), dim3(Ch / 256, P.job.nb), dim3(256), 0, stream, dh2, h1, mean1, rstd1, w1n,
                       b1n, wt, da1, P.part(), psum, Ch, frames, P.per, MidN2{});
  NPVP_CHECK_LAUNCH();
  return finish_partials(P.job, accumulate, stream, "mlpdw_mid_bwd: reduce launch failed");
}

extern "C" int npvp_mlpdw_mid_bwd(const float* dh2, const float* h1, const float* mean1, const float* rstd1, const float* w1n,
                                  const float* b1n, const float* wt, float* da1, float* dwt_db, float* psum, int frames, int H,
                                  int W, int Ch, int accumulate, void* workspace, long long ws_bytes, hipStream_t stream) {
  return mid_bwd_launch(dh2, h1, mean1, rstd1, w1n, b1n, wt, da1, dwt_db, psum, frames, H, W, Ch, accumulate, workspace, ws_bytes,
                        stream, nullptr);
}

extern "C" int npvp_mlpdw_mid_bwd_n2(const float* da2, const float* h2, const float* mean2, const float* rstd2, const float* w2n,
                                     const float* b2n, const float* psum2, int nparts2, float drop_p, unsigned int salt,
                                     const unsigned long long* seed, const float* h1, const float* mean1, const float* rstd1,
                                     const float* w1n, const float* b1n, const float* wt, float* da1, float* dwt_db, float* psum,
                                     int frames, int H, int W, int Ch, int accumulate, void* workspace, long long ws_bytes,
                                     hipStream_t stream) {
  NPVP_CHECK_ARG(h2 && mean2 && rstd2 && w2n && b2n && psum2 && nparts2 > 0 && nparts2 <= 256, "mlpdw_mid_bwd_n2: bad norm2 arguments");
  NPVP_CHECK_ARG(drop_p >= 0.f && drop_p < 1.f && (drop_p == 0.f || seed), "mlpdw_mid_bwd_n2: bad dropout arguments");
  MidN2 n2;
  n2.h2 = h2; n2.mean2 = mean2; n2.rstd2 = rstd2; n2.w2n = w2n; n2.b2n = b2n; n2.psum2 = psum2; n2.nparts2 = nparts2;
  n2.seed = seed; n2.drop_thresh = drop_p > 0.f ? drop_threshold(drop_p) : 0u;
  n2.drop_inv_keep = drop_p > 0.f ? 1.f / (1.f - drop_p) : 1.f; n2.salt = salt;
  return mid_bwd_launch(da2, h1, mean1, rstd1, w1n, b1n, wt, da1, dwt_db, psum, frames, H, W, Ch, accumulate, workspace, ws_bytes,
                        stream, &n2);
}

__global__ void mid_bwd_reduce_into_kernel(const float* __restrict__ part, float* __restrict__ gw, float* __restrict__ gb, int Ch,
                                           int nchunks) {
  const int i = blockIdx.x * blockDim.x + threadIdx.x;
  if (i >= 10 * Ch) return;
  float s = 0.f;
  for (int k = 0; k < nchunks; ++k) s += part[(long long)k * 10 * Ch + i];
  const int tap = i / Ch, c = i - tap * Ch;
  if (tap < 9) gw[c * 9 + tap] += s; else gb[c] += s;
}

extern "C" int npvp_mlpdw_mid_bwd_reduce_into(const void* workspace, float* gw, float* gb, int frames, int Ch,
                                              hipStream_t stream) {
  NPVP_CHECK_ARG(workspace && gw && gb && frames > 0 && Ch > 0, "mlpdw_mid_bwd_reduce_into: bad arguments");
  const SumRowsJob j = mid_partials(workspace, gw, gb, frames, Ch, 1).job;
  NPVP_LAUNCH(mid_bwd_reduce_into_kernel, dim3((10 * Ch + 255) / 256), dim3(256), 0, stream, j.in, gw, gb, Ch, j.nb);
  NPVP_CHECK_LAUNCH();
  return NPVP_OK;
}

extern "C" int npvp_mlpdw_mid_bwd_reduce_job(const void* workspace, float* gw, float* gb, int frames, int Ch, void* job) {
  NPVP_CHECK_ARG(workspace && gw && gb && frames > 0 && Ch > 0 && job, "mlpdw_mid_bwd_reduce_job: bad arguments");
  return put_job(job, mid_partials(workspace, gw, gb, frames, Ch, 1).job);
}

extern "C" int npvp_mlpdw_mid_bwd_reduce(const void* workspace, float* dwt_db, int frames, int Ch, int accumulate,
                                         hipStream_t stream) {
  return finish_partials(mid_partials(workspace, dwt_db, nullptr, frames, Ch, accumulate).job, 0, stream, "mlpdw_mid_bwd_reduce: launch failed");
}

extern "C" int npvp_im2col3x3(const float* in, float* out, int frames, int H, int W, int C, int col2im, hipStream_t stream) {
  NPVP_CHECK_ARG(frames > 0 && H > 0 && W > 0 && C % 4 == 0, "im2col: bad shape");
  const long long total4 = (long long)frames * H * W * (col2im ? 1 : 9) * C / 4;
  long long blocks = (total4 + 255) / 256; if (blocks > 8192) blocks = 8192;
  NPVP_LAUNCH(im2col3x3_kernel, dim3((unsigned)blocks), dim3(256), 0, stream, in, out, H, W, C, total4, col2im);
  NPVP_CHECK_LAUNCH();
  return NPVP_OK;
}

static Partials dw_partials(const void* ws, float* dwt_db, int frames, int Ch) {
  return make_partials(ws, 0, frames, dw_chunks(frames), 10 * Ch, dwt_db, 0);
}

extern "C" long long npvp_dwconv3x3_wgrad_workspace_bytes(int frames, int Ch) { return dw_partials(nullptr, nullptr, frames, Ch).bytes; }

extern "C" int npvp_dwconv3x3_wgrad(const float* a, const float* dout, float* dwt_db, int frames, int H, int W, int Ch,
                                    void* workspace, long long ws_bytes, hipStream_t stream) {
  NPVP_CHECK_ARG(frames > 0 && H > 0 && W > 0 && Ch % 4 == 0, "dwconv_wgrad: bad shape");
  NPVP_CHECK_ARG(workspace && ws_bytes >= npvp_dwconv3x3_wgrad_workspace_bytes(frames, Ch), "dwconv_wgrad: workspace too small");
  const Partials P = dw_partials(workspace, dwt_db, frames, Ch);
  if (H == 8 && W == 8)
    NPVP_LAUNCH((dwconv3x3_wgrad_win_kernel<8, 8>), dim3((Ch / 4 + 255) / 256, P.job.nb), dim3(256), 0, stream, a, dout,
// ... 8 lines not shown
```

npvp_amd/csrc/norm.hip:

```cpp
#include "partials.h"
#include <cstring>
#include <cstdlib>

namespace npvp {

template <int NV>
__global__ __launch_bounds__(256) void ln_fwd_kernel(const float* __restrict__ x, const float* __restrict__ w,
                                                     const float* __restrict__ b, float* __restrict__ y,
                                                     float* __restrict__ mean, float* __restrict__ rstd, long long rows,
                                                     float eps, int relu, float* __restrict__ amax) {
  constexpr int C = NV * 256;
  __shared__ float ared[4];
  const unsigned int peek = amax_peek_block(amax);
  const int lane = threadIdx.x & 63;
  float4 ww[NV], bb[NV];
#pragma unroll
  for (int i = 0; i < NV; ++i) { ww[i] = ld4(w + (i * 64 + lane) * 4); bb[i] = ld4(b + (i * 64 + lane) * 4); }
  float am = 0.f;
  for (long long row = (long long)blockIdx.x * 4 + (threadIdx.x >> 6); row < rows; row += (long long)gridDim.x * 4) {
    float4 v[NV];
    float s = 0.f;
#pragma unroll
    for (int i = 0; i < NV; ++i) {
      v[i] = ld4(x + row * C + (i * 64 + lane) * 4);
// ... 553 lines not shown
    const long long g0 = f * p.per_frame + e;
    float4 o;
    o.x = gelu_f((v.x - mu) * rs * ww.x + bb.x) * fln_scale(p, seed, fsc, g0 + 0);
    o.y = gelu_f((v.y - mu) * rs * ww.y + bb.y) * fln_scale(p, seed, fsc, g0 + 1);
    o.z = gelu_f((v.z - mu) * rs * ww.z + bb.z) * fln_scale(p, seed, fsc, g0 + 2);
    o.w = gelu_f((v.w - mu) * rs * ww.w + bb.w) * fln_scale(p, seed, fsc, g0 + 3);
    if (p.res) { const float4 r = ld4(p.res + g0); o.x += r.x; o.y += r.y; o.z += r.z; o.w += r.w; }
    st4(out + g0, o);
    am = amax4(am, o);
  }
  amax_slot_commit_block(amax, am, ared, peek);
}

__global__ __launch_bounds__(256) void frameln_act_fwd_parts_kernel(FlnParams p, const float* __restrict__ part, int J, float nb,
                                                                    float eps, float* __restrict__ mean_out,
                                                                    float* __restrict__ rstd_out, float* __restrict__ out,
                                                                    float* __restrict__ amax) {
  __shared__ float ared[16];
  const unsigned int peek = amax_peek_block(amax);
  const int bpf = p.per_frame / 4096;
  const long long f = blockIdx.x / bpf;
  const int e0 = (blockIdx.x - (int)f * bpf) * 4096;
  const unsigned long long seed = (p.seed && (p.drop_thresh || p.dp_thresh)) ? *p.seed : 0ull;
  float mu, rs;
  frame_stats_merge(part, f, J, nb, eps, mu, rs);
  if (e0 == 0 && threadIdx.x == 0) { mean_out[f] = mu; rstd_out[f] = rs; }
  const float fsc = fln_frame_scale(p, seed, f);
  float am = 0.f;
#pragma unroll
  for (int k = 0; k < 4; ++k) {
    const int e = e0 + (k * 256 + threadIdx.x) * 4;
    const long long g0 = f * p.per_frame + e;
    const float4 v = ld4(p.h + g0), ww = ld4(p.w + e), bb = ld4(p.b + e);
    float4 o;
    o.x = gelu_f((v.x - mu) * rs * ww.x + bb.x) * fln_scale(p, seed, fsc, g0 + 0);
    o.y = gelu_f((v.y - mu) * rs * ww.y + bb.y) * fln_scale(p, seed, fsc, g0 + 1);
    o.z = gelu_f((v.z - mu) * rs * ww.z + bb.z) * fln_scale(p, seed, fsc, g0 + 2);
    o.w = gelu_f((v.w - mu) * rs * ww.w + bb.w) * fln_scale(p, seed, fsc, g0 + 3);
    if (p.res) { const float4 r = ld4(p.res + g0); o.x += r.x; o.y += r.y; o.z += r.z; o.w += r.w; }
    st4(out + g0, o);
    am = amax4(am, o);
  }
  amax_slot_commit_block(amax, am, ared, peek);
}

constexpr int FLN_PARTS = 4;
__global__ __launch_bounds__(512) void frameln_act_bwd_stats_kernel(FlnParams p, const float* __restrict__ dout,
                                                                    float* __restrict__ psum) {
  __shared__ float red[8];
  const long long f = blockIdx.x;
  const unsigned long long seed = (p.seed && (p.drop_thresh || p.dp_thresh)) ? *p.seed : 0ull;
  const float mu = p.mean[f], rs = p.rstd[f];
  const float fsc = fln_frame_scale(p, seed, f);
  float s1 = 0.f, s2 = 0.f;
  const int span = p.per_frame / FLN_PARTS, e0 = blockIdx.y * span, e1 = blockIdx.y == FLN_PARTS - 1 ? p.per_frame : e0 + span;
  for (int e = e0 + threadIdx.x * 4; e < e1; e += 512 * 4) {
    const long long g0 = f * p.per_frame + e;
    const float4 v = ld4(p.h + g0), ww = ld4(p.w + e), bb = ld4(p.b + e), d = ld4(dout + g0);
    const float hx = (v.x - mu) * rs, hy = (v.y - mu) * rs, hz = (v.z - mu) * rs, hw = (v.w - mu) * rs;
    const float gx = d.x * fln_scale(p, seed, fsc, g0 + 0) * gelu_grad_f(hx * ww.x + bb.x) * ww.x;
    const float gy = d.y * fln_scale(p, seed, fsc, g0 + 1) * gelu_grad_f(hy * ww.y + bb.y) * ww.y;
    const float gz = d.z * fln_scale(p, seed, fsc, g0 + 2) * gelu_grad_f(hz * ww.z + bb.z) * ww.z;
    const float gw = d.w * fln_scale(p, seed, fsc, g0 + 3) * gelu_grad_f(hw * ww.w + bb.w) * ww.w;
    s1 += gx + gy + gz + gw;
    s2 += gx * hx + gy * hy + gz * hz + gw * hw;
  }
  s1 = block_sum<8>(s1, red);
  s2 = block_sum<8>(s2, red);
  if (threadIdx.x == 0) { psum[(f * FLN_PARTS + blockIdx.y) * 2] = s1; psum[(f * FLN_PARTS + blockIdx.y) * 2 + 1] = s2; }
}

__global__ void frameln_act_bwd_fused_kernel(FlnParams p, const float* __restrict__ dout, const float* __restrict__ psum,
                                             float* __restrict__ dh, float* __restrict__ part, int frames,
                                             int frames_per_chunk, int nparts, float* __restrict__ amax) {
  const int e = (blockIdx.x * blockDim.x + threadIdx.x) * 4;
  __shared__ float ared[16];
  const unsigned int peek = amax_peek_block(amax);
  float am = 0.f;
  if (e >= p.per_frame) { amax_slot_commit_block(amax, am, ared, peek); return; }
  const unsigned long long seed = (p.seed && (p.drop_thresh || p.dp_thresh)) ? *p.seed : 0ull;
  const float4 ww = ld4(p.w + e), bb = ld4(p.b + e);
  float4 aw = make_float4(0.f, 0.f, 0.f, 0.f), ab = make_float4(0.f, 0.f, 0.f, 0.f);
  const int f0 = blockIdx.y * frames_per_chunk;
  const int f1 = min(frames, f0 + frames_per_chunk);
  for (long long f = f0; f < f1; ++f) {
    const long long g0 = f * p.per_frame + e;
    const float mu = p.mean[f], rs = p.rstd[f];
    const float fsc = fln_frame_scale(p, seed, f);
    float a1 = 0.f, a2 = 0.f;
    for (int j = 0; j < nparts; ++j) { a1 += psum[(f * nparts + j) * 2]; a2 += psum[(f * nparts + j) * 2 + 1]; }
    a1 /= p.per_frame; a2 /= p.per_frame;
    const float4 v = ld4(p.h + g0), d = ld4(dout + g0);
    const float hx = (v.x - mu) * rs, hy = (v.y - mu) * rs, hz = (v.z - mu) * rs, hw = (v.w - mu) * rs;
    const float dx_ = d.x * fln_scale(p, seed, fsc, g0 + 0) * gelu_grad_f(hx * ww.x + bb.x);
    const float dy_ = d.y * fln_scale(p, seed, fsc, g0 + 1) * gelu_grad_f(hy * ww.y + bb.y);
    const float dz_ = d.z * fln_scale(p, seed, fsc, g0 + 2) * gelu_grad_f(hz * ww.z + bb.z);
    const float dw_ = d.w * fln_scale(p, seed, fsc, g0 + 3) * gelu_grad_f(hw * ww.w + bb.w);
    aw.x += dx_ * hx; aw.y += dy_ * hy; aw.z += dz_ * hz; aw.w += dw_ * hw;
    ab.x += dx_; ab.y += dy_; ab.z += dz_; ab.w += dw_;
    float4 o;
    o.x = rs * (dx_ * ww.x - a1 - hx * a2); o.y = rs * (dy_ * ww.y - a1 - hy * a2);
    o.z = rs * (dz_ * ww.z - a1 - hz * a2); o.w = rs * (dw_ * ww.w - a1 - hw * a2);
    st4(dh + g0, o);
    am = amax4(am, o);
  }
  amax_slot_commit_block(amax, am, ared, peek);
  float* o = part + (long long)blockIdx.y * 2 * p.per_frame;
  st4(o + e, aw);
  st4(o + p.per_frame + e, ab);
}

__global__ __launch_bounds__(256) void frameln_act_bwd_pgrad_kernel(FlnParams p, const float* __restrict__ dout,
                                                                    float* __restrict__ psum, float* __restrict__ part, int frames,
                                                                    int frames_per_chunk) {
  __shared__ float red[4];
  const int e = (blockIdx.x * blockDim.x + threadIdx.x) * 4;
  const int nblk = gridDim.x;
  const unsigned long long seed = (p.seed && (p.drop_thresh || p.dp_thresh)) ? *p.seed : 0ull;
  const float4 ww = ld4(p.w + e), bb = ld4(p.b + e);
  float4 aw = make_float4(0.f, 0.f, 0.f, 0.f), ab = make_float4(0.f, 0.f, 0.f, 0.f);
  const int f0 = blockIdx.y * frames_per_chunk;
  const int f1 = min(frames, f0 + frames_per_chunk);
  for (long long f = f0; f < f1; ++f) {
    const long long g0 = f * p.per_frame + e;
    const float mu = p.mean[f], rs = p.rstd[f];
    const float fsc = fln_frame_scale(p, seed, f);
    const float4 v = ld4(p.h + g0), d = ld4(dout + g0);
    const float hx = (v.x - mu) * rs, hy = (v.y - mu) * rs, hz = (v.z - mu) * rs, hw = (v.w - mu) * rs;
    const float dx_ = d.x * fln_scale(p, seed, fsc, g0 + 0) * gelu_grad_f(hx * ww.x + bb.x);
    const float dy_ = d.y * fln_scale(p, seed, fsc, g0 + 1) * gelu_grad_f(hy * ww.y + bb.y);
    const float dz_ = d.z * fln_scale(p, seed, fsc, g0 + 2) * gelu_grad_f(hz * ww.z + bb.z);
    const float dw_ = d.w * fln_scale(p, seed, fsc, g0 + 3) * gelu_grad_f(hw * ww.w + bb.w);
    aw.x += dx_ * hx; aw.y += dy_ * hy; aw.z += dz_ * hz; aw.w += dw_ * hw;
    ab.x += dx_; ab.y += dy_; ab.z += dz_; ab.w += dw_;
    const float gx = dx_ * ww.x, gy = dy_ * ww.y, gz = dz_ * ww.z, gw = dw_ * ww.w;
    const float s1 = block_sum<4>((gx + gy) + (gz + gw), red);
    const float s2 = block_sum<4>((gx * hx + gy * hy) + (gz * hz + gw * hw), red);
    if (threadIdx.x == 0) { psum[(f * nblk + blockIdx.x) * 2] = s1; psum[(f * nblk + blockIdx.x) * 2 + 1] = s2; }
  }
  float* o = part + (long long)blockIdx.y * 2 * p.per_frame;
  st4(o + e, aw);
  st4(o + p.per_frame + e, ab);
}

struct SumRowsPlan { int cw, threads; };
static SumRowsPlan plan_sum_rows(const SumRowsJob& q) {
  if (q.mode == 0 && q.nb < 64 && q.ncols >= 4096 && q.ncols % 4 == 0 && q.stride % 4 == 0 && (!q.out_b || q.split % 4 == 0)
      && ((uintptr_t)q.in & 15) == 0)
    return {sum_rows_wide_cols(), 1024};
  if (q.nb >= 64 && q.ncols <= 8192) return {16, 1024};
  return {64, q.nb >= 64 ? 1024 : 256};
}

int launch_sum_rows(const SumRowsJob& q, hipStream_t stream) {
  if (q.mode != 0) return NPVP_ERR_ARG;
  const SumRowsPlan pl = plan_sum_rows(q);
  const auto kernel = pl.cw == sum_rows_wide_cols() ? sum_rows_wide_kernel : pl.cw == 16 ? sum_rows_kernel<16> : sum_rows_kernel<64>;
  NPVP_LAUNCH(kernel, dim3((q.ncols + pl.cw - 1) / pl.cw), dim3(pl.threads), 0, stream, q.in, q.out, q.nb, q.stride, q.ncols, q.accum,
              q.out_b, q.out_b ? q.split : 0);
  return hipGetLastError() == hipSuccess ? NPVP_OK : NPVP_ERR_LAUNCH;
}

struct SumRowsBatch { SumRowsJob j[SRJ_MAX]; int first[SRJ_MAX + 1]; int cw[SRJ_MAX]; int n; };

__global__ __launch_bounds__(1024) void sum_rows_multi_kernel(SumRowsBatch b) {
  __shared__ float red[1024];
  int lo = 0, hi = b.n - 1;
  while (lo < hi) { const int mid = (lo + hi + 1) >> 1; if (b.first[mid] <= (int)blockIdx.x) lo = mid; else hi = mid - 1; }
  const SumRowsJob& J = b.j[lo];
  const int CW = b.cw[lo], sh = CW == 16 ? 4 : 6;
  if (CW == sum_rows_wide_cols()) {
    sum_rows_wide(J.in, J.out, J.out_b, J.nb, J.stride, J.ncols, J.out_b ? J.split : 0, J.accum,
                  (((int)blockIdx.x - b.first[lo]) * 1024 + (int)threadIdx.x) * 4);
    return;
  }
  const int cx = threadIdx.x & (CW - 1), rl = threadIdx.x >> sh, nrl = 1024 >> sh;
  const int c = ((int)blockIdx.x - b.first[lo]) * CW + cx;
  float s = 0.f;
  if (c < J.ncols)
// ... 228 lines not shown
extern "C" int npvp_frameln_act_fwd_parts(const float* h, const float* part, int J, float nb, float eps, float* mean, float* rstd,
                                          const float* w, const float* b, const float* res, float* out, int frames,
                                          int per_frame, float drop_p, unsigned int salt, float dp_p, unsigned int dp_salt,
                                          int frames_per_sample, const unsigned long long* seed, float* amax, hipStream_t stream) {
  NPVP_CHECK_ARG(frames > 0 && per_frame % 4096 == 0 && part && J > 0 && nb > 0.f && mean && rstd, "frameln_act_fwd_parts: bad arguments");
  NPVP_CHECK_ARG((drop_p == 0.f && dp_p == 0.f) || seed, "frameln_act: dropout needs a device seed");
  NPVP_CHECK_ARG((long long)frames * (per_frame / 4096) < (1ll << 31), "frameln_act_fwd_parts: too many blocks");
  FlnParams p;
  fill_fln(p, h, nullptr, nullptr, w, b, res, frames, per_frame, drop_p, salt, dp_p, dp_salt, frames_per_sample, seed);
  NPVP_LAUNCH(frameln_act_fwd_parts_kernel, dim3((unsigned)((long long)frames * (per_frame / 4096))), dim3(256), 0, stream, p,
                     part, J, nb, eps, mean, rstd, out, amax);
  NPVP_CHECK_LAUNCH();
  return NPVP_OK;
}

static int fln_chunks(int frames) {
  if (frames >= 512) return 32;
  const int c = frames / 2 < 16 ? frames / 2 : 16;
  return c < 1 ? 1 : c;
}

static Partials fln_partials(const void* ws, float* dw, float* db, int frames, int per_frame, int accumulate) {
  return make_partials(ws, (long long)frames * 2 * FLN_PARTS, frames, fln_chunks(frames), 2 * per_frame, dw, accumulate, db, per_frame);
}

extern "C" long long npvp_frameln_act_bwd_workspace_bytes(int frames, int per_frame) {
  return fln_partials(nullptr, nullptr, nullptr, frames, per_frame, 0).bytes;
}

static int fln_bwd_fused(const FlnParams& p, const float* dout, const float* psum, int nparts, float* dh, const Partials& P, int frames,
                         int accumulate, float* amax, hipStream_t stream, const char* error) {
  NPVP_LAUNCH(frameln_act_bwd_fused_kernel, dim3((p.per_frame / 4 + 255) / 256, P.job.nb), dim3(256), 0, stream, p,
                     dout, psum, dh, P.part(), frames, P.per, nparts, amax);
  NPVP_CHECK_LAUNCH();
  return finish_partials(P.job, accumulate, stream, error);
}

extern "C" int npvp_frameln_act_bwd(const float* dout, const float* h, const float* mean, const float* rstd, const float* w,
                                    const float* b, float* dh, float* dw, float* db, int frames, int per_frame,
                                    float drop_p, unsigned int salt, float dp_p, unsigned int dp_salt,
                                    int frames_per_sample, const unsigned long long* seed, int accumulate, float* amax,
                                    void* workspace, long long ws_bytes, hipStream_t stream) {
  NPVP_CHECK_ARG(frames > 0 && per_frame % 4 == 0, "frameln_act_bwd: bad shape");
  const Partials P = fln_partials(workspace, dw, db, frames, per_frame, accumulate);
  NPVP_CHECK_ARG(workspace && ws_bytes >= P.bytes, "frameln_act_bwd: workspace too small");
  FlnParams p;
  fill_fln(p, h, mean, rstd, w, b, nullptr, frames, per_frame, drop_p, salt, dp_p, dp_salt, frames_per_sample, seed);
  NPVP_CHECK_ARG(per_frame % (4 * FLN_PARTS) == 0, "frameln_act_bwd: per_frame must be a multiple of 16");
  NPVP_LAUNCH(frameln_act_bwd_stats_kernel, dim3(frames, FLN_PARTS), dim3(512), 0, stream, p, dout, (float*)workspace);
  NPVP_CHECK_LAUNCH();
  return fln_bwd_fused(p, dout, (const float*)workspace, FLN_PARTS, dh, P, frames, accumulate, amax, stream, "frameln_act_bwd: reduce launch failed");
}

extern "C" int npvp_frameln_act_bwd_apply(const float* dout, const float* h, const float* mean, const float* rstd, const float* w,
                                          const float* b, const float* psum, int nparts, float* dh, float* dw, float* db,
                                          int frames, int per_frame, int accumulate, float* amax, void* workspace,
                                          long long ws_bytes, hipStream_t stream) {
  NPVP_CHECK_ARG(frames > 0 && per_frame % 4 == 0 && psum && nparts > 0, "frameln_act_bwd_apply: bad arguments");
  const Partials P = fln_partials(workspace, dw, db, frames, per_frame, accumulate);
  NPVP_CHECK_ARG(workspace && ws_bytes >= P.bytes, "frameln_act_bwd_apply: workspace too small");
  FlnParams p;
  fill_fln(p, h, mean, rstd, w, b, nullptr, frames, per_frame, 0.f, 0u, 0.f, 0u, 1, nullptr);
  return fln_bwd_fused(p, dout, psum, nparts, dh, P, frames, accumulate, amax, stream, "frameln_act_bwd_apply: reduce launch failed");
}

extern "C" int npvp_frameln_act_bwd_pgrad(const float* dout, const float* h, const float* mean, const float* rstd, const float* w,
                                          const float* b, float* psum, float* dw, float* db, int frames, int per_frame,
                                          float drop_p, unsigned int salt, float dp_p, unsigned int dp_salt, int frames_per_sample,
                                          const unsigned long long* seed, int accumulate, void* workspace, long long ws_bytes,
                                          hipStream_t stream) {
  NPVP_CHECK_ARG(frames > 0 && per_frame % 1024 == 0 && psum, "frameln_act_bwd_pgrad: per_frame must be a multiple of 1024");
  const Partials P = fln_partials(workspace, dw, db, frames, per_frame, accumulate);
  NPVP_CHECK_ARG(workspace && ws_bytes >= P.bytes, "frameln_act_bwd_pgrad: workspace too small");
  FlnParams p;
  fill_fln(p, h, mean, rstd, w, b, nullptr, frames, per_frame, drop_p, salt, dp_p, dp_salt, frames_per_sample, seed);
  NPVP_LAUNCH(frameln_act_bwd_pgrad_kernel, dim3(per_frame / 1024, P.job.nb), dim3(256), 0, stream, p, dout, psum,
                     P.part(), frames, P.per);
  NPVP_CHECK_LAUNCH();
  return finish_partials(P.job, accumulate, stream, "frameln_act_bwd_pgrad: reduce launch failed");
}

extern "C" int npvp_frameln_act_bwd_reduce_job(const void* workspace, float* dw, float* db, int frames, int per_frame, int accumulate,
                                               void* job) {
  NPVP_CHECK_ARG(workspace && dw && db && frames > 0 && job, "frameln_act_bwd_reduce_job: bad arguments");
  return put_job(job, fln_partials(workspace, dw, db, frames, per_frame, accumulate).job);
}

extern "C" int npvp_frameln_act_bwd_reduce(const void* workspace, float* dw, float* db, int frames, int per_frame,
                                           int accumulate, hipStream_t stream) {
  NPVP_CHECK_ARG(workspace && dw && db && frames > 0, "frameln_act_bwd_reduce: bad arguments");
  return finish_partials(fln_partials(workspace, dw, db, frames, per_frame, accumulate).job, 0, stream, "frameln_act_bwd_reduce: launch failed");
}
```

npvp_amd/ops.py:

```python
import ctypes
import os

import torch

from ._lib import lib, check
from . import sched as _S
from .sched import (_p, _ptr, _stream, _ws, AmaxSlot, GemmProbe, HbmProbe, ProbeEvent, probe_pair, AuxStream, StepContext, current, use, scoped,
                    remember, rng, GradSink, WgradStream, WgradChain, ReduceQueue, RangeGuard)


def amax_of(t, slot=None):
    if slot is not None:
        return slot
    for cand in (t, t._base):
        tag = getattr(cand, "_npvp_amax", None) if cand is not None else None
        if tag is not None and tag[1] == cand._version:
            return tag[0]
    s = AmaxSlot.new(t.device)
    t2 = t if t.dim() == 2 else t.reshape(-1, t.shape[-1])
    if t2.stride(1) != 1:
        t2 = t2.contiguous()
    check(lib().npvp_amax(_ptr(t2), t2.shape[0], t2.shape[1], t2.stride(0), _ptr(s), _stream()), "npvp_amax")
    t._npvp_amax = (s, t._version)
    return s
# ... 178 lines not shown
    def refresh_all(cls, owner=None):
        cls.epoch += 1
        if not cls.enabled:
            return
        if cls._dirty or cls._tables is None:
            owner = None
            groups = {}
            for ent in cls._entries():
                if ent.w.is_cuda:
                    groups.setdefault((ent.w.untyped_storage().data_ptr(), ent.fmt, ent.w.device), []).append(ent)
            cls._tables = []
            kept = {}
            for gkey, ents in groups.items():
                own_id, fmt, dev = gkey
                ids = tuple(id(e) for e in ents)
                old = cls._group_tensors.get(gkey)
                if old is not None and old[0] == ids and (fmt != 6 or all(e.amax_t is old[2] for e in ents)):
                    table, amax_t = old[1], old[2]
                else:
                    amax_t = None
                    if fmt == 6:
                        amax_t = torch.zeros(len(ents), AmaxSlot.FLOATS, dtype=torch.float32, device=dev)
                        for i, ent in enumerate(ents):
                            ent.amax_t = amax_t
                            ent.amax.ptr, ent.amax.chunk = amax_t.data_ptr() + AmaxSlot.BYTES * i, amax_t
                    rows = []
                    for ent in ents:
                        N, K = ent.w.shape
                        r = [ent.w.data_ptr(), ent.w.stride(0), N, K, ent.planes[0].data_ptr(), ent.planes[1].data_ptr()]
                        rows.append(r + [ent.amax.ptr, 0] if fmt == 6 else r)
                    table = torch.tensor(rows, dtype=torch.int64).to(dev)
                kept[gkey] = (ids, table, amax_t)
                cls._tables.append((fmt, table, amax_t, ents, own_id))
            cls._group_tensors = kept
            cls._dirty = False
        only = None if owner is None else owner.untyped_storage().data_ptr()
        for fmt, table, amax_t, ents, own_id in cls._tables:
            if only is not None and own_id != only:
                continue
            with torch.cuda.device(table.device):
                if fmt == 6:
                    check(lib().npvp_split_weights_f16(_p(table.data_ptr()), table.shape[0], _p(amax_t.data_ptr()),
                                                       amax_t.numel() * 4, _stream()), "npvp_split_weights_f16")
                else:
                    check(lib().npvp_split_weights_batched(_p(table.data_ptr()), table.shape[0], _stream()), "npvp_split_weights_batched")
            for ent in ents:
                ent.version = ent.w._version




def gemm(a_kc, b_kc, M, N, K, A, lda, B, ldb, out, bias=None, act=0, aux_in=None, aux_out=None, residual=None,
         drop=NO_DROP, alpha=1.0, colsum_a=None, b_pre=None, accumulate=False, rowstats=None, precision=None,
         replay=False, a_amax=None, b_amax=None, c_amax=None, a_drop=NO_DROP, range_flag=None):
    for t in (A, B, out, bias, aux_in, aux_out, residual, colsum_a):
        if t is not None and not (t.is_cuda and t.dtype is torch.float32):
            _chk(t)
    prec = GEMM_PRECISION if precision is None else precision
    planes = None
    if b_pre is not None:
        planes, b_amax = b_pre
    if prec == 6:
        kid = _gemm_kernel_id(a_kc, b_kc, M, N, K, 6, planes is not None)
        if kid == 5 or kid == 7:
            if a_amax is None:
                a_amax = amax_of(A)
        elif kid == 6:
            if a_amax is None:
                a_amax = amax_of(A)
            if b_amax is None:
                b_amax = amax_of(B)
        else:
            planes = None
    wsb = _gemm_ws_bytes(M, N, K)
    ws, wsn = (None, 0)
    if wsb > 0:
        ws, wsn = _ws(wsb, A.device)
    masked = drop.p > 0.0 or a_drop.p > 0.0
    seed = _S._cur.rng.seed_tensor(A.device) if masked else None
    if DropRecorder.sites is not None and not replay:
        DropRecorder.note(drop, "elem" if drop.mode == 0 else "group", M * N if drop.mode == 0 else drop.g2)
    probe = GemmProbe.armed
    if probe:
        kid = _gemm_kernel_id(a_kc, b_kc, M, N, K, prec, planes is not None)
        probe = GemmProbe.only is None or kid in GemmProbe.only
    if probe:
        e0, e1 = probe_pair()
    rc = lib().npvp_gemm_f32(
        a_kc, b_kc, M, N, K, A.data_ptr(), lda, B.data_ptr(), ldb, out.data_ptr(), out.stride(0),
        None if bias is None else bias.data_ptr(), act, None if aux_in is None else aux_in.data_ptr(),
        None if aux_out is None else aux_out.data_ptr(), None if residual is None else residual.data_ptr(),
        0 if residual is None else residual.stride(0), drop.p, drop.mode, drop.g1, drop.g2,
        None if seed is None else seed.data_ptr(), drop.salt, alpha, prec, None if colsum_a is None else colsum_a.data_ptr(),
        None if planes is None else planes.data_ptr(), 1 if accumulate else 0, None if rowstats is None else rowstats.data_ptr(),
        None if a_amax is None else a_amax.data_ptr(), None if b_amax is None else b_amax.data_ptr(),
        None if c_amax is None else c_amax.data_ptr(), None if range_flag is None else range_flag.data_ptr(),
        a_drop.p, a_drop.g1, a_drop.g2, a_drop.salt, None if ws is None else ws.data_ptr(), wsn, _stream())
    if rc:
        check(rc, "npvp_gemm_f32")
    if probe:
        e1.record()
        GemmProbe.records.append((e0, e1, 2.0 * M * N * K, 4.0 * (M * K + N * K + M * N), ((a_kc, b_kc), kid)))
    return out


_KID_CACHE, _WSB_CACHE = {}, {}


def _gemm_kernel_id(a_kc, b_kc, M, N, K, prec, has_planes):
    key = (a_kc, b_kc, M, N, K, prec, has_planes)
    v = _KID_CACHE.get(key)
    if v is None:
        v = _KID_CACHE[key] = lib().npvp_gemm_kernel_id(a_kc, b_kc, M, N, K, prec, int(has_planes))
    return v


def _gemm_ws_bytes(M, N, K):
    v = _WSB_CACHE.get((M, N, K))
    if v is None:
        v = _WSB_CACHE[(M, N, K)] = lib().npvp_gemm_workspace_bytes(M, N, K)
    return v


def _planes(w, want, R):
    return WeightPlanes.get(w, want) if R >= 256 else None


def _new_slot(dev, want=True):
    return AmaxSlot.new(dev) if (want and GEMM_PRECISION == 6) else None


def linear_fwd(x, w, b, act=0, aux_out=None, residual=None, drop=NO_DROP, rowstats=None, x_amax=None, y_amax=None):
    R, K = x.shape
    N = w.shape[0]
    y = torch.empty(R, N, dtype=torch.float32, device=x.device)
    return gemm(1, 1, R, N, K, x, x.stride(0), w, w.stride(0), y, bias=b, act=act, aux_out=aux_out, residual=residual,
                drop=drop, b_pre=_planes(w, "F", R), rowstats=rowstats, a_amax=x_amax, c_amax=y_amax)


def linear_frame_stats_supported(R, N):
    return GEMM_PRECISION in (4, 6) and R % 64 == 0 and N % 128 == 0


def linear_dgrad(dy, w, act=0, aux_in=None, drop=NO_DROP, residual=None, dy_amax=None, dx_amax=None, a_drop=NO_DROP, out=None,
                 accumulate=False):
    R, N = dy.shape
    K = w.shape[1]
    dx = torch.empty(R, K, dtype=torch.float32, device=dy.device) if out is None else out
    return gemm(1, 0, R, K, N, dy, dy.stride(0), w, w.stride(0), dx, act=act, aux_in=aux_in, drop=drop, residual=residual,
                b_pre=_planes(w, "D", R), replay=True, a_amax=dy_amax, c_amax=dx_amax, a_drop=a_drop, accumulate=accumulate)


def masked_grad(dy2, drop, w):
    if not drop.on:
        return dy2, NO_DROP
    R, N = dy2.shape
    K = w.shape[1]
    if (drop.mode == 1 and drop.g1 % 16 == 0 and drop.p < 0.5 and GEMM_PRECISION == 6 and R <= DROP_PATH_IN_GEMM_ROWS
            and _planes(w, "D", R) is not None and _gemm_kernel_id(1, 0, R, K, N, 6, True) in (5, 7)
            and _gemm_kernel_id(0, 0, N, K, R, 6, False) == 6):
        return dy2, drop
    return drop_apply(dy2, drop), NO_DROP


DROP_PATH_IN_GEMM_ROWS = 1 << 30


def linear_wgrad(dy, x, with_bias_grad=False, into=None, into_b=None, dy_amax=None, x_amax=None, a_drop=NO_DROP):
    R, N = dy.shape
    K = x.shape[1]
    acc = into is not None
    dw = into if acc else torch.empty(N, K, dtype=torch.float32, device=dy.device)
    db = (into_b if acc else torch.empty(N, dtype=torch.float32, device=dy.device)) if with_bias_grad else None
    prec = WGRAD_PRECISION if GEMM_PRECISION == 4 else None
    watch = GEMM_PRECISION == 6 and _gemm_kernel_id(0, 0, N, K, R, 6, False) == 6
    if watch and _S._cur.range_guard.fallback and not a_drop.on:
        prec, watch = 4, False
    if watch and _S._cur.range_guard.strict and not a_drop.on:
        flag = _S._cur.range_guard.flag(dy.device)
        tw = torch.empty(N, K, dtype=torch.float32, device=dy.device)
        tb = torch.empty(N, dtype=torch.float32, device=dy.device) if with_bias_grad else None
        gemm(0, 0, N, K, R, dy, dy.stride(0), x, x.stride(0), tw, colsum_a=tb, a_amax=dy_amax, b_amax=x_amax, range_flag=flag)
        if _S._cur.range_guard.poll(dy.device):
            _S._cur.range_guard.fallback = False
            gemm(0, 0, N, K, R, dy, dy.stride(0), x, x.stride(0), tw, colsum_a=tb, precision=4)
        if acc:
            dw.add_(tw)
            if tb is not None:
                db.add_(tb)
        else:
            dw, db = tw, tb
        return (dw, db) if with_bias_grad else dw
    flag = _S._cur.range_guard.flag(dy.device) if watch else None
    on_side = _S._cur.wgrad.in_flush
    if (watch and acc and prec is None and _S._cur.chain.enabled and _S._cur.chain.takes(N, K, R)
            and (on_side or (not _S._cur.wgrad.enabled and _S._cur.grad_sink.listener is None))
            and dy.stride(1) == 1 and x.stride(1) == 1 and dw.stride(1) == 1):
        _S._cur.chain.launch(dy, x, dw, db, amax_of(dy, dy_amax), amax_of(x, x_amax), a_drop, flag)
        if not on_side:
            _S._cur.reduce._arm()
        return (dw, db) if with_bias_grad else dw
    gemm(0, 0, N, K, R, dy, dy.stride(0), x, x.stride(0), dw, colsum_a=db, accumulate=acc, precision=prec, a_amax=dy_amax, b_amax=x_amax,
         a_drop=a_drop, range_flag=flag)
    return (dw, db) if with_bias_grad else dw


class FusedLinearBwd:
    enabled = True
    MAX_ROWS = 16384
    with_gradient_stream = False
    _ok = {}

    @classmethod
    def takes(cls, R, N, K):
        key = (R, N, K)
        v = cls._ok.get(key)
        if v is None:
            v = cls._ok[key] = bool(lib().npvp_linear_bwd_f16_takes(R, N, K)) and _S._cur.chain.takes(N, K, R)
        return v and R <= cls.MAX_ROWS


def linear_bwd(dy, x, w, b, sk, act=0, aux_in=None, drop=NO_DROP, residual=None, dy_amax=None, dx_amax=None, a_drop=NO_DROP):
    R, N = dy.shape
    K = w.shape[1]
    has_b = b is not None
    if (FusedLinearBwd.enabled and GEMM_PRECISION == 6 and sk and has_b == (sk[1] is not None) and FusedLinearBwd.takes(R, N, K)
            and (FusedLinearBwd.with_gradient_stream or not _S._cur.wgrad.enabled) and not _S._cur.range_guard.fallback and not _S._cur.range_guard.strict and dy.stride(1) == 1 and x.stride(1) == 1):
        pl = _planes(w, "D", R)
        gw = sk[0][0]
        if pl is not None and gw.stride(1) == 1:
            planes, w_amax = pl
            gb = sk[1][0] if has_b else None
            dev = dy.device
            dy_amax, x_amax = amax_of(dy, dy_amax), amax_of(x)
            dx = torch.empty(R, K, dtype=torch.float32, device=dev)
            ws, wsn = _ws(_S._cur.chain._wsb[(N, K, R)], dev)
            st = _stream()
            seed = _S._cur.rng.seed_tensor(dev) if (drop.on or a_drop.on) else None
            outs = (gw.data_ptr(),) if gb is None else (gw.data_ptr(), gb.data_ptr())
            chain = not _S._cur.wgrad.enabled
            if chain:
                job = ctypes.create_string_buffer(64)
                prev = _S._cur.chain._pending.pop(st, None)
                job_addr, prev_addr = ctypes.addressof(job), (ctypes.addressof(prev[0]) if prev is not None else None)
            else:
                job_addr, prev_addr = _S._cur.reduce.splitk_slot(outs), None
            probe = GemmProbe.armed and (GemmProbe.only is None or 8 in GemmProbe.only)
            if probe:
                e0, e1 = probe_pair()
            check(lib().npvp_linear_bwd_f16(R, N, K, dy.data_ptr(), dy.stride(0), dy_amax.data_ptr(), planes.data_ptr(), w_amax.data_ptr(),
                                            dx.data_ptr(), dx.stride(0), act, _ptr(aux_in), _ptr(residual),
                                            0 if residual is None else residual.stride(0), drop.p, drop.mode, drop.g1, drop.g2, drop.salt,
                                            _ptr(dx_amax), x.data_ptr(), x.stride(0), x_amax.data_ptr(), gw.data_ptr(), gw.stride(0),
                                            _ptr(gb), _ptr(_S._cur.range_guard.flag(dev)), a_drop.p, a_drop.g1, a_drop.g2, a_drop.salt, _ptr(seed),
                                            prev_addr, job_addr, ws.data_ptr(), wsn, st), "npvp_linear_bwd_f16")
            if probe:
                e1.record()
                GemmProbe.records.append((e0, e1, 4.0 * R * N * K, 4.0 * (2 * R * N + 2 * R * K + 2 * N * K), ((1, 0), 8)))
            if chain:
                if prev is not None and prev[4] is not None:
                    _S._cur.grad_sink.wrote(*prev[4])
                _S._cur.chain._pending[st] = (job, ws, gw, gb, sk)
                _S._cur.reduce._arm()
            else:
                _S._cur.reduce.splitk_added(outs, ws, sk)
            return dx, None, None
    dx = linear_dgrad(dy, w, act=act, aux_in=aux_in, drop=drop, residual=residual, dy_amax=dy_amax, dx_amax=dx_amax, a_drop=a_drop)
    gw, gb = _lin_grads(dy, x, w, b, sk, a_drop=a_drop)
    return dx, gw, gb


def colsum(x):
    R, N = x.shape
    L = lib()
    out = torch.empty(N, dtype=torch.float32, device=x.device)
    ws, wsn = _ws(L.npvp_colsum_workspace_bytes(R, N), x.device)
    check(L.npvp_colsum(_ptr(x), R, N, x.stride(0), _ptr(out), 0, _ptr(ws), wsn, _stream()), "npvp_colsum")
    return out


def drop_apply(x2d, drop):
    out = torch.empty_like(x2d)
    slot = _new_slot(x2d.device)
    check(lib().npvp_drop_apply(_ptr(x2d), _ptr(out), x2d.shape[0], x2d.shape[1], drop.p, drop.mode, drop.g1, drop.g2,
                                _ptr(_S._cur.rng.seed_tensor(x2d.device)), drop.salt, _ptr(slot), _stream()), "npvp_drop_apply")
    return tag_amax(out, slot)


def transpose(x):
    _chk(x)
    x = _c(x)
    B, R, C = x.shape
    out = torch.empty(B, C, R, dtype=torch.float32, device=x.device)
    check(lib().npvp_transpose(_ptr(x), _ptr(out), B, R, C, _stream()), "npvp_transpose")
    return out


def reduce_mid(x, scale=1.0, out=None, accumulate=False):
    _chk(x)
    x = _c(x)
    A, B, C = x.shape
    if out is None:
        out = torch.empty(A, C, dtype=torch.float32, device=x.device)
    check(lib().npvp_reduce_mid(_ptr(x), _ptr(out), A, B, C, scale, 1 if accumulate else 0, _stream()), "npvp_reduce_mid")
    return out


class ActSink:
    __slots__ = ("buf",)
    enabled = True

    def __init__(self):
        self.buf = None

    def target(self, shape, dev):
        if self.buf is None:
            self.buf = torch.empty(shape, dtype=torch.float32, device=dev)
            return self.buf, False
        if self.buf.numel() != torch.Size(shape).numel():
            raise RuntimeError(f"ActSink: a consumer contributes a gradient of shape {tuple(shape)} to a buffer of shape {tuple(self.buf.shape)}")
# ... 514 lines not shown

class _AttnPacked(torch.autograd.Function):

    @staticmethod
    def forward(ctx, qk, v, cfg):
        remember(ctx)
        _chk(qk, v)
        C = v.shape[1]
        o = torch.empty_like(v)
        _attn_fwd(qk[:, :C], qk[:, C:], v, o, cfg)
        ctx.save_for_backward(qk, v)
        ctx.cfg = cfg
        return o

    @scoped
    def backward(ctx, go):
        qk, v = ctx.saved_tensors
        C = v.shape[1]
        go = _c(go)
        dqk, dv = torch.empty_like(qk), torch.empty_like(v)
        _attn_bwd(qk[:, :C], qk[:, C:], v, go, dqk[:, :C], dqk[:, C:], dv, ctx.cfg, packed=dqk)
        return dqk, dv, None


class _Attn(torch.autograd.Function):

    @staticmethod
    def forward(ctx, q, k, v, cfg):
        remember(ctx)
        _chk(q, k, v)
        o = torch.empty_like(q)
        _attn_fwd(q, k, v, o, cfg)
        ctx.save_for_backward(q, k, v)
        ctx.cfg = cfg
        return o

    @scoped
    def backward(ctx, go):
        q, k, v = ctx.saved_tensors
        go = _c(go)
        dq, dk, dv = torch.empty_like(q), torch.empty_like(k), torch.empty_like(v)
        _attn_bwd(q, k, v, go, dq, dk, dv, ctx.cfg)
        return dq, dk, dv, None


def attn_packed(qk, v, cfg):
    return _AttnPacked.apply(qk, v, cfg)


def attn(q, k, v, cfg):
    return _Attn.apply(q, k, v, cfg)


def _fln_bwd(dout, h, mean, rstd, w, b, frames, PF, d, dp, T, sk, psum=None, nparts=0, want_amax=True):
    L = lib()
    dev = h.device
    dh = torch.empty_like(h)
    slot = _new_slot(dev, want_amax)
    tag_amax(dh, slot)
    dw, db = (sk[0][0], sk[1][0]) if sk else (torch.empty_like(w), torch.empty_like(b))
    ws, wsn = _ws(L.npvp_frameln_act_bwd_workspace_bytes(frames, PF), dev)
    mode = _sink_mode(sk)
    if psum is None:
        seed = _S._cur.rng.seed_tensor(dev) if (d.on or dp.on) else None
        check(L.npvp_frameln_act_bwd(_ptr(dout), _ptr(h), _ptr(mean), _ptr(rstd), _ptr(w), _ptr(b), _ptr(dh), _ptr(dw), _ptr(db),
                                     frames, PF, d.p, d.salt, dp.p, dp.salt, T, _ptr(seed), mode, _ptr(slot), _ptr(ws), wsn,
                                     _stream()), "npvp_frameln_act_bwd")
    else:
        pe = HbmProbe.begin()
        check(L.npvp_frameln_act_bwd_apply(_ptr(dout), _ptr(h), _ptr(mean), _ptr(rstd), _ptr(w), _ptr(b), _ptr(psum), nparts,
                                           _ptr(dh), _ptr(dw), _ptr(db), frames, PF, mode, _ptr(slot), _ptr(ws), wsn, _stream()),
              "npvp_frameln_act_bwd_apply")
        HbmProbe.end(pe, "npvp::frameln_act_bwd_fused_kernel", 4.0 * 3 * frames * PF)
    if sk:
        _reduce_partials(sk, ws, dw, db, L.npvp_frameln_act_bwd_reduce, L.npvp_frameln_act_bwd_reduce_job, "npvp_frameln_act_bwd_reduce",
                         (frames, PF, 1), True)
        return dh, None, None
    return dh, dw, db


def _fln_pgrad(dout, h, mean, rstd, w, b, frames, PF, d, sk):
    L = lib()
    dev = h.device
    psum = torch.empty(frames * (PF // 1024) * 2, dtype=torch.float32, device=dev)
    dw, db = (sk[0][0], sk[1][0]) if sk else (torch.empty_like(w), torch.empty_like(b))
    ws, wsn = _ws(L.npvp_frameln_act_bwd_workspace_bytes(frames, PF), dev)
    seed = _S._cur.rng.seed_tensor(dev) if d.on else None
    check(L.npvp_frameln_act_bwd_pgrad(_ptr(dout), _ptr(h), mean, rstd, _ptr(w), _ptr(b), _ptr(psum), _ptr(dw), _ptr(db),
                                       frames, PF, d.p, d.salt, 0.0, 0, 1, _ptr(seed), _sink_mode(sk), _ptr(ws), wsn, _stream()),
          "npvp_frameln_act_bwd_pgrad")
    if sk:
        _reduce_partials(sk, ws, dw, db, L.npvp_frameln_act_bwd_reduce, L.npvp_frameln_act_bwd_reduce_job, "npvp_frameln_act_bwd_reduce",
                         (frames, PF, 1), True)
        return psum, None, None
    return psum, dw, db


class _FrameLnAct(torch.autograd.Function):

    @staticmethod
    def forward(ctx, h, w_cl, b_cl, res, frames, p_drop, p_dp, frames_per_sample, mean=None, rstd=None):
        remember(ctx)
        _chk(h, w_cl, b_cl, res)
        h = _c(h)
        PF = h.numel() // frames
        w_cl, b_cl = _c(w_cl), _c(b_cl)
        res_c = None if res is None else _c(res)
        L = lib()
        if mean is None:
            mean = torch.empty(frames, dtype=torch.float32, device=h.device)
            rstd = torch.empty_like(mean)
            check(L.npvp_frame_stats(_ptr(h), _p(0), _ptr(mean), _ptr(rstd), frames, 1, PF, 1e-5, _stream()), "npvp_frame_stats")
        d, dp = Drop(p_drop), Drop(p_dp, 1)
        DropRecorder.note(d, "elem", h.numel())
        DropRecorder.note(dp, "group", frames // max(1, frames_per_sample))
        out = torch.empty_like(h)
        seed = _S._cur.rng.seed_tensor(h.device) if (d.on or dp.on) else None
        slot = _new_slot(h.device)
        check(L.npvp_frameln_act_fwd(_ptr(h), _ptr(mean), _ptr(rstd), _ptr(w_cl), _ptr(b_cl), _ptr(res_c), _ptr(out), frames,
                                     PF, d.p, d.salt, dp.p, dp.salt, frames_per_sample, _ptr(seed), _ptr(slot), _stream()),
              "npvp_frameln_act_fwd")
        tag_amax(out, slot)
        ctx.save_for_backward(h, mean, rstd, w_cl, b_cl)
        ctx.cfg = (frames, PF, d, dp, frames_per_sample, res is not None)
        ctx.sink = _ln_sink(w_cl, b_cl)
        return out

    @scoped
    def backward(ctx, dout):
        h, mean, rstd, w_cl, b_cl = ctx.saved_tensors
        frames, PF, d, dp, fps, has_res = ctx.cfg
        dout = _c(dout)
        dh, dw, db = _fln_bwd(dout, h, mean, rstd, w_cl, b_cl, frames, PF, d, dp, fps, ctx.sink)
        return dh, dw, db, (dout if has_res else None), None, None, None, None, None, None


def frameln_act(h, w_cl, b_cl, res, frames, p_drop=0.0, p_dp=0.0, frames_per_sample=1, stats=None):
    mean, rstd = stats if stats is not None else (None, None)
    return _FrameLnAct.apply(h, w_cl, b_cl, res, frames, p_drop, p_dp, frames_per_sample, mean, rstd)


class _DwConv(torch.autograd.Function):

# ... 55 lines not shown
        gemm(1, 1, R, hid, C, x, x.stride(0), w1, w1.stride(0), h1, bias=b1, b_pre=_planes(w1, "F", R),
             rowstats=part)
        stats = torch.empty(6, frames, dtype=f32, device=dev)
        key = (WeightPlanes.epoch, dww._version, dwb._version, dww.data_ptr(), dwb.data_ptr())
        hit = dww.__dict__.get("_npvp_wtb")
        if hit is not None and hit[0] == key:
            wtb = hit[1]
        else:
            wtb = torch.empty(10, hid, dtype=f32, device=dev)
            check(L.npvp_dwtb_build(_ptr(_c(dww)), _ptr(dwb), _ptr(wtb), hid, st), "npvp_dwtb_build")
            dww.__dict__["_npvp_wtb"] = (key, wtb)
        h2 = torch.empty(R, hid, dtype=f32, device=dev)
        part2 = torch.empty(frames * (hid // 512) * 2, dtype=f32, device=dev)
        check(L.npvp_mlpdw_mid_fwd_parts(_ptr(h1), _ptr(part), hid // 64, 4096.0, _row(stats, 0), _row(stats, 1), _ptr(n1w), _ptr(n1b),
                                         _ptr(wtb), _row(wtb, 9), _ptr(h2), _ptr(part2), frames, 8, 8, hid, 1e-5, st),
              "npvp_mlpdw_mid_fwd_parts")
        d2, d3, dp = Drop(p_drop), Drop(p_drop), Drop(p_dp, 1)
        DropRecorder.note(d2, "elem", R * hid)
        seed = _S._cur.rng.seed_tensor(dev) if (d2.on or dp.on) else None
        a2 = torch.empty(R, hid, dtype=f32, device=dev)
        a2_slot = _new_slot(dev)
        check(L.npvp_frameln_act_fwd_parts(_ptr(h2), _ptr(part2), hid // 512, 32768.0, 1e-5, _row(stats, 2), _row(stats, 3), _ptr(n2w),
                                           _ptr(n2b), None, _ptr(a2), frames, PFh, d2.p, d2.salt, 0.0, 0, 1, _ptr(seed), _ptr(a2_slot),
                                           st), "npvp_frameln_act_fwd_parts")
        tag_amax(a2, a2_slot)
        h3 = torch.empty(R, Co, dtype=f32, device=dev)
        part3 = torch.empty(frames * (Co // 64) * 2, dtype=f32, device=dev)
        gemm(1, 1, R, Co, hid, a2, hid, w2, w2.stride(0), h3, bias=b2, b_pre=_planes(w2, "F", R),
             rowstats=part3)
        DropRecorder.note(d3, "elem", R * Co)
        DropRecorder.note(dp, "group", frames // max(1, T))
        out = torch.empty(R, Co, dtype=f32, device=dev)
        check(L.npvp_frameln_act_fwd_parts(_ptr(h3), _ptr(part3), Co // 64, 4096.0, 1e-5, _row(stats, 4), _row(stats, 5), _ptr(n3w),
                                           _ptr(n3b), _ptr(res), _ptr(out), frames, PFo, d3.p, d3.salt, dp.p, dp.salt, T, _ptr(seed),
                                           None, st), "npvp_frameln_act_fwd_parts")
        ctx.save_for_backward(x, h1, h2, a2, h3, stats, wtb, w1, w2, n1w, n1b, n2w, n2b, n3w, n3b)
        ctx.cfg = (frames, T, d2, d3, dp, res is not None, b1 is not None, b2 is not None)
        ctx.sinks = (_wb_sink(w1, b1), _wb_sink(w2, b2), _ln_sink(n1w, n1b), _ln_sink(n2w, n2b), _ln_sink(n3w, n3b))
        sd = _wb_sink(dww, dwb) if (dww.is_contiguous() and dwb is not None) else None
        ctx.sink_dw = sd if (sd and sd[1] is not None) else None
        return out

    @scoped
    def backward(ctx, dout):
        x, h1, h2, a2, h3, stats, wtb, w1, w2, n1w, n1b, n2w, n2b, n3w, n3b = ctx.saved_tensors
        frames, T, d2, d3, dp, has_res, has_b1, has_b2 = ctx.cfg
        s_fc1, s_fc2, s_n1, s_n2, s_n3 = ctx.sinks
        L = lib()
        R, hid = h1.shape
        Co = h3.shape[1]
        dev = x.device
        dout = _c(dout)
        dh3, gn3w, gn3b = _fln_bwd(dout, h3, stats[4], stats[5], n3w, n3b, frames, 64 * Co, d3, dp, T, s_n3)
        da2, gw2, gb2 = linear_bwd(dh3, a2, w2, True if has_b2 else None, s_fc2)
        fuse_n2 = MID_BWD_N2 and hid // 16 <= 256
        if fuse_n2:
            psum2, gn2w, gn2b = _fln_pgrad(da2, h2, _row(stats, 2), _row(stats, 3), n2w, n2b, frames, 64 * hid, d2, s_n2)
        else:
            dh2, gn2w, gn2b = _fln_bwd(da2, h2, stats[2], stats[3], n2w, n2b, frames, 64 * hid, d2, NO_DROP, 1, s_n2,
                                          want_amax=False)
            del da2
        da1 = torch.empty_like(h1)
        dwtb = torch.empty(10, hid, dtype=torch.float32, device=dev)
        nparts = hid // 256
        psum = torch.empty(frames * nparts * 2, dtype=torch.float32, device=dev)
        ws, wsn = _ws(L.npvp_mlpdw_mid_bwd_workspace_bytes(frames, hid), dev)
        sk_dw = ctx.sink_dw if ctx.needs_input_grad[6] and ctx.needs_input_grad[7] else None
        wmode = 2 if sk_dw else 0
        if fuse_n2:
            seed = _S._cur.rng.seed_tensor(dev) if d2.on else None
            pe = HbmProbe.begin()
            check(L.npvp_mlpdw_mid_bwd_n2(_ptr(da2), _ptr(h2), _row(stats, 2), _row(stats, 3), _ptr(n2w), _ptr(n2b), _ptr(psum2),
                                          hid // 16, d2.p, d2.salt, _ptr(seed), _ptr(h1), _row(stats, 0), _row(stats, 1), _ptr(n1w),
                                          _ptr(n1b), _ptr(wtb), _ptr(da1), _ptr(dwtb), _ptr(psum), frames, 8, 8, hid, wmode, _ptr(ws), wsn,
                                          _stream()), "npvp_mlpdw_mid_bwd_n2")
            HbmProbe.end(pe, "npvp::mlpdw_mid_bwd_kernel<1, true>", 4.0 * 4 * frames * 64 * hid)
            del da2, psum2
        else:
            check(L.npvp_mlpdw_mid_bwd(_ptr(dh2), _ptr(h1), _row(stats, 0), _row(stats, 1), _ptr(n1w), _ptr(n1b), _ptr(wtb), _ptr(da1),
                                       _ptr(dwtb), _ptr(psum), frames, 8, 8, hid, wmode, _ptr(ws), wsn, _stream()), "npvp_mlpdw_mid_bwd")
            del dh2
        if sk_dw:
            _reduce_partials(sk_dw, ws, sk_dw[0][0], sk_dw[1][0], L.npvp_mlpdw_mid_bwd_reduce_into, L.npvp_mlpdw_mid_bwd_reduce_job,
                             "npvp_mlpdw_mid_bwd_reduce_into", (frames, hid), False)
            gdww = gdwb = None
        else:
            gdww = torch.empty(hid, 1, 3, 3, dtype=torch.float32, device=dev)
            check(L.npvp_transpose(_ptr(dwtb), _ptr(gdww), 1, 9, hid, _stream()), "npvp_transpose")
            gdwb = dwtb[9]
        dh1, gn1w, gn1b = _fln_bwd(da1, h1, stats[0], stats[1], n1w, n1b, frames, 64 * hid, NO_DROP, NO_DROP, 1, s_n1,
                                      psum=psum, nparts=nparts)
        del da1
        dx, gw1, gb1 = linear_bwd(dh1, x, w1, True if has_b1 else None, s_fc1)
        return (dx, dout if has_res else None, gw1, gb1, gn1w, gn1b, gdww, gdwb, gn2w, gn2b, gw2, gb2, gn3w, gn3b,
                None, None, None, None)


MID_BWD_N2 = True


def mlpdwbn_fused_supported(R, C, hid, Co, H, W):
    return (GEMM_PRECISION in (4, 6) and H == 8 and W == 8 and R % 64 == 0 and hid % 512 == 0 and Co % 128 == 0 and hid % 128 == 0
            and C % 32 == 0)


def mlpdwbn(x, res, w1, b1, n1w, n1b, dww, dwb, n2w, n2b, w2, b2, n3w, n3b, frames, T, p_drop, p_dp):
    return _MlpDwbn.apply(x, res, w1, b1, n1w, n1b, dww, dwb, n2w, n2b, w2, b2, n3w, n3b, frames, T, p_drop, p_dp)


def _raw_ln_fwd(x2, w, b, eps, relu=0):
    rows, C = x2.shape
    y = torch.empty_like(x2)
    st = torch.empty(2, rows, dtype=torch.float32, device=x2.device)
    slot = _new_slot(x2.device)
    check(lib().npvp_layernorm_fwd(_ptr(x2), _ptr(w), _ptr(b), _ptr(y), _row(st, 0), _row(st, 1), rows, C, eps, relu, _ptr(slot),
                                   _stream()), "npvp_layernorm_fwd")
    return tag_amax(y, slot), st


def _raw_ln_bwd(dy2, x2, w, b, st, dres, sk, relu=0, probe=False):
    L = lib()
    rows, C = x2.shape
    dx = torch.empty_like(x2)
    dw, db = (sk[0][0], sk[1][0]) if sk else (torch.empty_like(w), torch.empty_like(b))
    ws, wsn = _ws(L.npvp_layernorm_bwd_workspace_bytes(rows, C), x2.device)
    slot = _new_slot(x2.device)
    pe = HbmProbe.begin() if probe else None
    check(L.npvp_layernorm_bwd(_ptr(dy2), _ptr(x2), _ptr(w), _ptr(b), _row(st, 0), _row(st, 1), _ptr(dx), _ptr(dw), _ptr(db), rows, C,
                               relu, _ptr(dres), _sink_mode(sk), _ptr(slot), _ptr(ws), wsn, _stream()), "npvp_layernorm_bwd")
    HbmProbe.end(pe, "npvp::ln_bwd_kernel<2>", 4.0 * (3 + (dres is not None)) * rows * C)
    tag_amax(dx, slot)
    if sk:
        _reduce_partials(sk, ws, dw, db, L.npvp_layernorm_bwd_reduce, L.npvp_layernorm_bwd_reduce_job, "npvp_layernorm_bwd_reduce",
                         (rows, C, 1), True)
        return dx, None, None
    return dx, dw, db


def _raw_posfuse_fwd(x, add, beta, gamma, N, T):
    PF = x.numel() // (N * T)
    y = torch.empty_like(x)
    st = torch.empty(2, N * T, dtype=torch.float32, device=x.device)
    slot = _new_slot(x.device)
    check(lib().npvp_posfuse_fwd(_ptr(x), _ptr(add), _ptr(beta), _ptr(gamma), _ptr(y), _row(st, 0), _row(st, 1), N, T, PF, 1e-5,
                                 _ptr(slot), _stream()), "npvp_posfuse_fwd")
    return tag_amax(y, slot), st
# ... 480 lines not shown
```

Before: 8381.

## Skip backward work for frames zeroed by drop-path in MLP-dwconv block

```diff
diff --git a/include/npvp_hip.h b/include/npvp_hip.h
--- a/include/npvp_hip.h
+++ b/include/npvp_hip.h
@@ -29,6 +29,13 @@
                   const void* b_pre, int accumulate, float* rowstats, const float* a_amax, const float* b_amax,
                   float* c_amax, unsigned int* range_flag, float adrop_p, int adrop_g1, int adrop_g2, unsigned int adrop_salt,
                   void* workspace, long long ws_bytes, npvp_stream_t stream);
+int npvp_gemm_f32_skip(int a_kc, int b_kc, int M, int N, int K, const float* A, long long lda, const float* B, long long ldb,
+                       float* C, long long ldc, const float* bias, int act, const float* aux_in, float* aux_out,
+                       const float* residual, long long ldr, float drop_p, int drop_mode, int drop_g1, int drop_g2,
+                       const unsigned long long* seed, unsigned int salt, float alpha, int precision, float* colsum_a,
+                       const void* b_pre, int accumulate, float* rowstats, const float* a_amax, const float* b_amax,
+                       float* c_amax, unsigned int* range_flag, float adrop_p, int adrop_g1, int adrop_g2, unsigned int adrop_salt,
+                       void* workspace, long long ws_bytes, npvp_stream_t stream);
 int npvp_frame_stats_finalize(const float* part, int parts_per_frame, float values_per_part, float* mean, float* rstd,
                               int frames, float eps, npvp_stream_t stream);
 int npvp_split_weight(const float* w, long long ld, int N, int K, void* F, void* D, npvp_stream_t stream);
@@ -140,6 +147,26 @@
                                const float* b, const float* psum, int nparts, float* dh, float* dw, float* db, int frames,
                                int per_frame, int accumulate, float* dh_amax, void* workspace, long long ws_bytes,
                                npvp_stream_t stream);
+int npvp_frameln_act_bwd_pgrad_skip(const float* dout, const float* h, const float* mean, const float* rstd, const float* w,
+                                    const float* b, float* psum, float* dw, float* db, int frames, int per_frame, float drop_p,
+                                    unsigned int salt, float dp_p, unsigned int dp_salt, int frames_per_sample,
+                                    const unsigned long long* seed, int accumulate, void* workspace, long long ws_bytes,
+                                    npvp_stream_t stream);
+int npvp_frameln_act_bwd_apply_skip(const float* dout, const float* h, const float* mean, const float* rstd, const float* w,
+                                    const float* b, const float* psum, int nparts, float* dh, float* dw, float* db, int frames,
+                                    int per_frame, int accumulate, float* dh_amax, float dp_p, unsigned int dp_salt,
+                                    int frames_per_sample, const unsigned long long* seed, void* workspace, long long ws_bytes,
+                                    npvp_stream_t stream);
+int npvp_mlpdw_mid_bwd_skip(const float* dh2, const float* h1, const float* mean1, const float* rstd1, const float* w1n,
+                            const float* b1n, const float* wt, float* da1, float* dwt_db, float* psum, int frames, int H, int W,
+                            int Ch, int accumulate, float dp_p, unsigned int dp_salt, int frames_per_sample,
+                            const unsigned long long* seed, void* workspace, long long ws_bytes, npvp_stream_t stream);
+int npvp_mlpdw_mid_bwd_n2_skip(const float* da2, const float* h2, const float* mean2, const float* rstd2, const float* w2n,
+                               const float* b2n, const float* psum2, int nparts2, float drop_p, unsigned int salt,
+                               const unsigned long long* seed, const float* h1, const float* mean1, const float* rstd1,
+                               const float* w1n, const float* b1n, const float* wt, float* da1, float* dwt_db, float* psum,
+                               int frames, int H, int W, int Ch, int accumulate, float dp_p, unsigned int dp_salt,
+                               int frames_per_sample, void* workspace, long long ws_bytes, npvp_stream_t stream);
 
 int npvp_im2col3x3(const float* in, float* out, int frames, int H, int W, int C, int col2im, npvp_stream_t stream);
 long long npvp_dwconv3x3_wgrad_workspace_bytes(int frames, int Ch);
diff --git a/npvp_amd/_lib.py b/npvp_amd/_lib.py
--- a/npvp_amd/_lib.py
+++ b/npvp_amd/_lib.py
@@ -30,6 +30,9 @@
     "npvp_gemm_f32": (c_int, [c_int, c_int, c_int, c_int, c_int, c_p, c_ll, c_p, c_ll, c_p, c_ll, c_p, c_int, c_p, c_p,
                               c_p, c_ll, c_f, c_int, c_int, c_int, c_p, c_u, c_f, c_int, c_p, c_p, c_int, c_p, c_p, c_p, c_p, c_p,
                               c_f, c_int, c_int, c_u, c_p, c_ll, c_p]),
+    "npvp_gemm_f32_skip": (c_int, [c_int, c_int, c_int, c_int, c_int, c_p, c_ll, c_p, c_ll, c_p, c_ll, c_p, c_int, c_p, c_p,
+                                   c_p, c_ll, c_f, c_int, c_int, c_int, c_p, c_u, c_f, c_int, c_p, c_p, c_int, c_p, c_p, c_p, c_p, c_p,
+                                   c_f, c_int, c_int, c_u, c_p, c_ll, c_p]),
     "npvp_amax": (c_int, [c_p, c_ll, c_ll, c_ll, c_p, c_p]),
     "npvp_wgrad_f16_chainable": (c_int, [c_int, c_int, c_int]),
     "npvp_wgrad_f16_chain_workspace_bytes": (c_ll, [c_int, c_int, c_int]),
@@ -82,6 +85,14 @@
     "npvp_frameln_act_bwd_pgrad": (c_int, [c_p, c_p, c_p, c_p, c_p, c_p, c_p, c_p, c_p, c_int, c_int, c_f, c_u, c_f, c_u, c_int,
                                            c_p, c_int, c_p, c_ll, c_p]),
     "npvp_frameln_act_bwd_apply": (c_int, [c_p, c_p, c_p, c_p, c_p, c_p, c_p, c_int, c_p, c_p, c_p, c_int, c_int, c_int, c_p, c_p, c_ll, c_p]),
+    "npvp_frameln_act_bwd_pgrad_skip": (c_int, [c_p, c_p, c_p, c_p, c_p, c_p, c_p, c_p, c_p, c_int, c_int, c_f, c_u, c_f, c_u, c_int,
+                                                c_p, c_int, c_p, c_ll, c_p]),
+    "npvp_frameln_act_bwd_apply_skip": (c_int, [c_p, c_p, c_p, c_p, c_p, c_p, c_p, c_int, c_p, c_p, c_p, c_int, c_int, c_int, c_p,
+                                                c_f, c_u, c_int, c_p, c_p, c_ll, c_p]),
+    "npvp_mlpdw_mid_bwd_skip": (c_int, [c_p, c_p, c_p, c_p, c_p, c_p, c_p, c_p, c_p, c_p, c_int, c_int, c_int, c_int, c_int,
+                                        c_f, c_u, c_int, c_p, c_p, c_ll, c_p]),
+    "npvp_mlpdw_mid_bwd_n2_skip": (c_int, [c_p, c_p, c_p, c_p, c_p, c_p, c_p, c_int, c_f, c_u, c_p, c_p, c_p, c_p, c_p, c_p, c_p, c_p, c_p,
+                                           c_p, c_int, c_int, c_int, c_int, c_int, c_f, c_u, c_int, c_p, c_ll, c_p]),
     "npvp_im2col3x3": (c_int, [c_p, c_p, c_int, c_int, c_int, c_int, c_int, c_p]),
     "npvp_dwconv3x3_wgrad_workspace_bytes": (c_ll, [c_int, c_int]),
     "npvp_dwconv3x3_wgrad": (c_int, [c_p, c_p, c_p, c_int, c_int, c_int, c_int, c_p, c_ll, c_p]),
diff --git a/npvp_amd/csrc/common.h b/npvp_amd/csrc/common.h
--- a/npvp_amd/csrc/common.h
+++ b/npvp_amd/csrc/common.h
@@ -210,6 +210,16 @@
   return d;
 }
 
+struct FrameSkip { const unsigned long long* seed; unsigned int thresh; unsigned int salt; int frames_per_sample; };
+inline FrameSkip make_frame_skip(float p, unsigned int salt, int frames_per_sample, const unsigned long long* seed) {
+  FrameSkip s;
+  s.seed = seed; s.thresh = p > 0.f ? drop_threshold(p) : 0u; s.salt = salt; s.frames_per_sample = frames_per_sample > 0 ? frames_per_sample : 1;
+  return s;
+}
+__device__ __forceinline__ bool frame_skipped(const FrameSkip& s, uint64_t seed, long long f) {
+  return s.thresh && rng_u32(seed, s.salt, (uint64_t)((unsigned int)f / (unsigned int)s.frames_per_sample)) < s.thresh;
+}
+
 __device__ __forceinline__ float4 ld4(const float* p) { return *reinterpret_cast<const float4*>(p); }
 __device__ __forceinline__ void st4(float* p, float4 v) { *reinterpret_cast<float4*>(p) = v; }
 
diff --git a/npvp_amd/csrc/gemm.h b/npvp_amd/csrc/gemm.h
--- a/npvp_amd/csrc/gemm.h
+++ b/npvp_amd/csrc/gemm.h
@@ -26,6 +26,7 @@
   int act;
   DropSpec drop;
   DropSpec adrop;
+  int adrop_applied;
   int tiles_m, tiles_n;
   int splits;
   float alpha;
diff --git a/npvp_amd/csrc/gemm.hip b/npvp_amd/csrc/gemm.hip
--- a/npvp_amd/csrc/gemm.hip
+++ b/npvp_amd/csrc/gemm.hip
@@ -519,13 +519,13 @@
   return finish_partials(make_partials(p.colsum, 0, p.splits, p.splits, p.M, colsum_a, p.accum).job, 0, stream, "gemm: column-sum reduce launch failed");
 }
 
-extern "C" int npvp_gemm_f32(int a_kc, int b_kc, int M, int N, int K, const float* A, long long lda, const float* B,
+static int gemm_f32_launch(int a_kc, int b_kc, int M, int N, int K, const float* A, long long lda, const float* B,
                              long long ldb, float* C, long long ldc, const float* bias, int act, const float* aux_in,
                              float* aux_out, const float* residual, long long ldr, float drop_p, int drop_mode,
                              int drop_g1, int drop_g2, const unsigned long long* seed, unsigned int salt, float alpha,
                              int precision, float* colsum_a, const void* b_pre, int accumulate, float* rowstats,
                              const float* a_amax, const float* b_amax, float* c_amax, unsigned int* range_flag,
-                             float adrop_p, int adrop_g1, int adrop_g2, unsigned int adrop_salt,
+                             float adrop_p, int adrop_g1, int adrop_g2, unsigned int adrop_salt, int adrop_applied,
                              void* workspace, long long ws_bytes, hipStream_t stream) {
   NPVP_CHECK_ARG(M > 0 && N > 0 && K > 0, "gemm: empty problem");
   NPVP_CHECK_ARG(precision == 0 || precision == 4 || precision == 5 || precision == 6,
@@ -547,7 +547,7 @@
   NPVP_CHECK_ARG(!colsum_a || a_kc == 0, "gemm: colsum_a is the column sum of a [K][M] operand (a_kc = 0)");
   NPVP_CHECK_ARG(!b_pre || ((uintptr_t)b_pre % 16) == 0, "gemm: b_pre must be 16-byte aligned");
 
-  NPVP_CHECK_ARG(adrop_p >= 0.f && adrop_p < 0.5f, "gemm: adrop_p must be in [0, 0.5) (the masked operand must stay inside its amax scale)");
+  NPVP_CHECK_ARG(adrop_p >= 0.f && adrop_p < (adrop_applied ? 1.f : 0.5f), "gemm: adrop_p must be in [0, 0.5) (the masked operand must stay inside its amax scale)");
   NPVP_CHECK_ARG(adrop_p == 0.f || (seed && want_h && adrop_g1 > 0 && adrop_g2 > 0 && (a_kc || adrop_g1 % 16 == 0)),
                  "gemm: adrop needs precision 6, a device seed and (for a weight gradient) groups of a multiple of 16 rows");
   NPVP_CHECK_ARG(!rowstats || ((precision == 4 || want_h) && a_kc && b_kc && M % 64 == 0 && N % 128 == 0 && act == 0 && !aux_out && !residual &&
@@ -557,6 +557,7 @@
   const bool plain = !bias && act == 0 && !aux_out && !residual && drop_p == 0.f;
   const GemmPlan plan = plan_gemm(GemmFacts{a_kc, b_kc, M, N, K, precision, b_pre != nullptr, plain,
                                             a_amax && b_amax, rowstats != nullptr, workspace ? ws_bytes : 0});
+  NPVP_CHECK_ARG(!adrop_applied || adrop_p == 0.f || a_kc, "gemm: an already applied row-group mask is taken by forward / dgrad launches only");
   NPVP_CHECK_ARG(adrop_p == 0.f || plan.id >= 5, "gemm: adrop was requested but this shape does not run on the fp16 kernels (npvp_gemm_kernel_id tells)");
 
   GemmParams p;
@@ -564,6 +565,7 @@
   p.seed = seed; p.lda = lda; p.ldb = ldb; p.ldr = ldr; p.M = M; p.N = N; p.act = act;
   p.drop = make_drop_spec(drop_p, salt, drop_mode, drop_g1, drop_g2);
   p.adrop = make_drop_spec(adrop_p, adrop_salt, 1, adrop_g1, adrop_g2);
+  p.adrop_applied = adrop_applied ? 1 : 0;
   p.alpha = alpha;
   p.rowstats = rowstats;
   p.a_amax = a_amax; p.b_amax = b_amax; p.c_amax = c_amax; p.range_flag = range_flag;
@@ -602,3 +604,29 @@
   NPVP_CHECK_LAUNCH();
   return plan.splits > 1 ? finish_splitk(p, C, ldc, colsum_a, stream) : NPVP_OK;
 }
+
+extern "C" int npvp_gemm_f32(int a_kc, int b_kc, int M, int N, int K, const float* A, long long lda, const float* B,
+                             long long ldb, float* C, long long ldc, const float* bias, int act, const float* aux_in,
+                             float* aux_out, const float* residual, long long ldr, float drop_p, int drop_mode,
+                             int drop_g1, int drop_g2, const unsigned long long* seed, unsigned int salt, float alpha,
+                             int precision, float* colsum_a, const void* b_pre, int accumulate, float* rowstats,
+                             const float* a_amax, const float* b_amax, float* c_amax, unsigned int* range_flag,
+                             float adrop_p, int adrop_g1, int adrop_g2, unsigned int adrop_salt,
+                             void* workspace, long long ws_bytes, hipStream_t stream) {
+  return gemm_f32_launch(a_kc, b_kc, M, N, K, A, lda, B, ldb, C, ldc, bias, act, aux_in, aux_out, residual, ldr, drop_p, drop_mode,
+                         drop_g1, drop_g2, seed, salt, alpha, precision, colsum_a, b_pre, accumulate, rowstats, a_amax, b_amax, c_amax,
+                         range_flag, adrop_p, adrop_g1, adrop_g2, adrop_salt, 0, workspace, ws_bytes, stream);
+}
+
+extern "C" int npvp_gemm_f32_skip(int a_kc, int b_kc, int M, int N, int K, const float* A, long long lda, const float* B,
+                                  long long ldb, float* C, long long ldc, const float* bias, int act, const float* aux_in,
+                                  float* aux_out, const float* residual, long long ldr, float drop_p, int drop_mode,
+                                  int drop_g1, int drop_g2, const unsigned long long* seed, unsigned int salt, float alpha,
+                                  int precision, float* colsum_a, const void* b_pre, int accumulate, float* rowstats,
+                                  const float* a_amax, const float* b_amax, float* c_amax, unsigned int* range_flag,
+                                  float adrop_p, int adrop_g1, int adrop_g2, unsigned int adrop_salt,
+                                  void* workspace, long long ws_bytes, hipStream_t stream) {
+  return gemm_f32_launch(a_kc, b_kc, M, N, K, A, lda, B, ldb, C, ldc, bias, act, aux_in, aux_out, residual, ldr, drop_p, drop_mode,
+                         drop_g1, drop_g2, seed, salt, alpha, precision, colsum_a, b_pre, accumulate, rowstats, a_amax, b_amax, c_amax,
+                         range_flag, adrop_p, adrop_g1, adrop_g2, adrop_salt, 1, workspace, ws_bytes, stream);
+}
diff --git a/npvp_amd/csrc/gemm_f16.hip b/npvp_amd/csrc/gemm_f16.hip
--- a/npvp_amd/csrc/gemm_f16.hip
+++ b/npvp_amd/csrc/gemm_f16.hip
@@ -75,11 +75,15 @@
   const unsigned int a_off0 = (unsigned int)(((long long)(min(m0 + rl, p.M - 1) - m0) * p.lda + 4 * quad) * 4);
   const unsigned int a_off1 = (unsigned int)(((long long)(min(m0 + rl + BM / 2, p.M - 1) - m0) * p.lda + 4 * quad) * 4);
   const int a_dst = (quad >> 1) * KGS_A + (quad & 1) * 8 + rl * 16;
+  __shared__ int guard_flags[NW];
   float sa0 = sa, sa1 = sa;
+  bool dead_tile = false;
   if (p.adrop.thresh) {
     const unsigned long long aseed = *p.seed;
-    sa0 *= drop_spec_scale(p.adrop, aseed, min(m0 + rl, p.M - 1), 0, 1);
-    sa1 *= drop_spec_scale(p.adrop, aseed, min(m0 + rl + BM / 2, p.M - 1), 0, 1);
+    const float f0 = drop_spec_scale(p.adrop, aseed, min(m0 + rl, p.M - 1), 0, 1);
+    const float f1 = APASS == 2 ? drop_spec_scale(p.adrop, aseed, min(m0 + rl + BM / 2, p.M - 1), 0, 1) : f0;
+    if (!p.adrop_applied) { sa0 *= f0; sa1 *= f1; }
+    dead_tile = !block_any<NW>(f0 != 0.f || f1 != 0.f, guard_flags, wave);
   }
   const char* b_base = reinterpret_cast<const char*>(p.b_pre);
   unsigned int b_off[CPW];
@@ -123,7 +127,6 @@
                      :: "s"(m0_), "v"(b_off[i_]), "s"(bb_) : "memory", "m0"); } }
   static_assert(NCHUNK % NW == 0, "the hand-counted waits assume CPW LDS-DMA pieces per wave and step");
 
-  __shared__ int guard_flags[NW];
   float rm0 = 0.f, rm1 = 0.f;
   bool rescued = false;
   const float zrow = 1.f;
@@ -197,8 +200,13 @@
   asm volatile("s_waitcnt vmcnt(0)" : "+v"(ea0), "+v"(ea1), "+v"(eb0), "+v"(eb1) :: "memory");
   if constexpr (NST == 3) __builtin_amdgcn_s_barrier();
   };
-  run_tile();
-  {
+  if (dead_tile) {
+#pragma unroll
+    for (int i = 0; i < TM; ++i)
+#pragma unroll
+      for (int j = 0; j < TN; ++j) acc[i][j] = zero16;
+  } else {
+    run_tile();
     rm0 = fmaxf(rm0, __shfl_xor(rm0, 1)); rm0 = fmaxf(rm0, __shfl_xor(rm0, 2));
     rm1 = fmaxf(rm1, __shfl_xor(rm1, 1)); rm1 = fmaxf(rm1, __shfl_xor(rm1, 2));
     const int et = (int)((__float_as_uint(sa) >> 23) & 0xffu);
diff --git a/npvp_amd/csrc/mlpdw.hip b/npvp_amd/csrc/mlpdw.hip
--- a/npvp_amd/csrc/mlpdw.hip
+++ b/npvp_amd/csrc/mlpdw.hip
@@ -195,10 +195,11 @@
                                                             const float* __restrict__ w1n, const float* __restrict__ b1n,
                                                             const float* __restrict__ wt, float* __restrict__ da1,
                                                             float* __restrict__ part, float* __restrict__ psum, int Ch,
-                                                            int frames, int frames_per_chunk, MidN2 n2) {
+                                                            int frames, int frames_per_chunk, MidN2 n2, FrameSkip skip) {
   constexpr int HH = 8, WW = 8;
   __shared__ float red[4];
   const unsigned long long seed2 = (FUSE2 && n2.seed && n2.drop_thresh) ? *n2.seed : 0ull;
+  const unsigned long long seed_skip = skip.thresh ? *skip.seed : 0ull;
   const int c = (blockIdx.x * blockDim.x + threadIdx.x) * VEC;
   const int nblk = gridDim.x;
   Vec<VEC> wv[9], aw[9], ab;
@@ -212,10 +213,18 @@
   for (int e = 0; e < VEC; ++e) ab.v[e] = 0.f;
   const int f0 = blockIdx.y * frames_per_chunk, f1 = min(frames, f0 + frames_per_chunk);
   for (long long f = f0; f < f1; ++f) {
+    float* of = da1 + f * (HH * WW) * Ch;
+    if (frame_skipped(skip, seed_skip, f)) {
+      Vec<VEC> z;
+#pragma unroll
+      for (int e = 0; e < VEC; ++e) z.v[e] = 0.f;
+      for (int pix = 0; pix < HH * WW; ++pix) stv<VEC>(of + pix * Ch + c, z);
+      if (threadIdx.x == 0) { psum[(f * nblk + blockIdx.x) * 2] = 0.f; psum[(f * nblk + blockIdx.x) * 2 + 1] = 0.f; }
+      continue;
+    }
     const float mu = mean1[f], rs = rstd1[f];
     const float* hf = h1 + f * (HH * WW) * Ch;
     const float* gf = dh2 + f * (HH * WW) * Ch;
-    float* of = da1 + f * (HH * WW) * Ch;
     float mu2 = 0.f, rs2 = 0.f, c1 = 0.f, c2 = 0.f;
     const float* h2f = nullptr;
     if constexpr (FUSE2) {
@@ -549,16 +558,18 @@
 
 static int mid_bwd_launch(const float* dh2, const float* h1, const float* mean1, const float* rstd1, const float* w1n,
                           const float* b1n, const float* wt, float* da1, float* dwt_db, float* psum, int frames, int H, int W,
-                          int Ch, int accumulate, void* workspace, long long ws_bytes, hipStream_t stream, const MidN2* n2) {
+                          int Ch, int accumulate, void* workspace, long long ws_bytes, hipStream_t stream, const MidN2* n2,
+                          const FrameSkip& skip) {
   NPVP_CHECK_ARG(frames > 0 && H == 8 && W == 8 && Ch > 0 && Ch % 512 == 0, "mlpdw_mid_bwd: needs an 8x8 grid and Ch % 512 == 0");
+  NPVP_CHECK_ARG(!skip.thresh || skip.seed, "mlpdw_mid_bwd: a skip site needs a device seed");
   NPVP_CHECK_ARG(workspace && ws_bytes >= npvp_mlpdw_mid_bwd_workspace_bytes(frames, Ch), "mlpdw_mid_bwd: workspace too small");
   const Partials P = mid_partials(workspace, dwt_db, nullptr, frames, Ch, accumulate);
   if (n2)
     NPVP_LAUNCH((mlpdw_mid_bwd_kernel<1, true>), dim3(Ch / 256, P.job.nb), dim3(256), 0, stream, dh2, h1, mean1, rstd1, w1n,
-                       b1n, wt, da1, P.part(), psum, Ch, frames, P.per, *n2);
+                       b1n, wt, da1, P.part(), psum, Ch, frames, P.per, *n2, skip);
   else
     NPVP_LAUNCH((mlpdw_mid_bwd_kernel<1, false>), dim3(Ch / 256, P.job.nb), dim3(256), 0, stream, dh2, h1, mean1, rstd1, w1n,
-                       b1n, wt, da1, P.part(), psum, Ch, frames, P.per, MidN2{});
+                       b1n, wt, da1, P.part(), psum, Ch, frames, P.per, MidN2{}, skip);
   NPVP_CHECK_LAUNCH();
   return finish_partials(P.job, accumulate, stream, "mlpdw_mid_bwd: reduce launch failed");
 }
@@ -567,15 +578,24 @@
                                   const float* b1n, const float* wt, float* da1, float* dwt_db, float* psum, int frames, int H,
                                   int W, int Ch, int accumulate, void* workspace, long long ws_bytes, hipStream_t stream) {
   return mid_bwd_launch(dh2, h1, mean1, rstd1, w1n, b1n, wt, da1, dwt_db, psum, frames, H, W, Ch, accumulate, workspace, ws_bytes,
-                        stream, nullptr);
-}
-
-extern "C" int npvp_mlpdw_mid_bwd_n2(const float* da2, const float* h2, const float* mean2, const float* rstd2, const float* w2n,
-                                     const float* b2n, const float* psum2, int nparts2, float drop_p, unsigned int salt,
-                                     const unsigned long long* seed, const float* h1, const float* mean1, const float* rstd1,
-                                     const float* w1n, const float* b1n, const float* wt, float* da1, float* dwt_db, float* psum,
-                                     int frames, int H, int W, int Ch, int accumulate, void* workspace, long long ws_bytes,
-                                     hipStream_t stream) {
+                        stream, nullptr, FrameSkip{});
+}
+
+extern "C" int npvp_mlpdw_mid_bwd_skip(const float* dh2, const float* h1, const float* mean1, const float* rstd1, const float* w1n,
+                                       const float* b1n, const float* wt, float* da1, float* dwt_db, float* psum, int frames, int H,
+                                       int W, int Ch, int accumulate, float dp_p, unsigned int dp_salt, int frames_per_sample,
+                                       const unsigned long long* seed, void* workspace, long long ws_bytes, hipStream_t stream) {
+  NPVP_CHECK_ARG(dp_p >= 0.f && dp_p < 1.f && frames_per_sample > 0, "mlpdw_mid_bwd_skip: bad drop-path arguments");
+  return mid_bwd_launch(dh2, h1, mean1, rstd1, w1n, b1n, wt, da1, dwt_db, psum, frames, H, W, Ch, accumulate, workspace, ws_bytes,
+                        stream, nullptr, make_frame_skip(dp_p, dp_salt, frames_per_sample, seed));
+}
+
+static int mid_bwd_n2_launch(const float* da2, const float* h2, const float* mean2, const float* rstd2, const float* w2n,
+                             const float* b2n, const float* psum2, int nparts2, float drop_p, unsigned int salt,
+                             const unsigned long long* seed, const float* h1, const float* mean1, const float* rstd1,
+                             const float* w1n, const float* b1n, const float* wt, float* da1, float* dwt_db, float* psum,
+                             int frames, int H, int W, int Ch, int accumulate, void* workspace, long long ws_bytes,
+                             hipStream_t stream, const FrameSkip& skip) {
   NPVP_CHECK_ARG(h2 && mean2 && rstd2 && w2n && b2n && psum2 && nparts2 > 0 && nparts2 <= 256, "mlpdw_mid_bwd_n2: bad norm2 arguments");
   NPVP_CHECK_ARG(drop_p >= 0.f && drop_p < 1.f && (drop_p == 0.f || seed), "mlpdw_mid_bwd_n2: bad dropout arguments");
   MidN2 n2;
@@ -583,7 +603,30 @@
   n2.seed = seed; n2.drop_thresh = drop_p > 0.f ? drop_threshold(drop_p) : 0u;
   n2.drop_inv_keep = drop_p > 0.f ? 1.f / (1.f - drop_p) : 1.f; n2.salt = salt;
   return mid_bwd_launch(da2, h1, mean1, rstd1, w1n, b1n, wt, da1, dwt_db, psum, frames, H, W, Ch, accumulate, workspace, ws_bytes,
-                        stream, &n2);
+                        stream, &n2, skip);
+}
+
+extern "C" int npvp_mlpdw_mid_bwd_n2(const float* da2, const float* h2, const float* mean2, const float* rstd2, const float* w2n,
+                                     const float* b2n, const float* psum2, int nparts2, float drop_p, unsigned int salt,
+                                     const unsigned long long* seed, const float* h1, const float* mean1, const float* rstd1,
+                                     const float* w1n, const float* b1n, const float* wt, float* da1, float* dwt_db, float* psum,
+                                     int frames, int H, int W, int Ch, int accumulate, void* workspace, long long ws_bytes,
+                                     hipStream_t stream) {
+  return mid_bwd_n2_launch(da2, h2, mean2, rstd2, w2n, b2n, psum2, nparts2, drop_p, salt, seed, h1, mean1, rstd1, w1n, b1n, wt, da1,
+                           dwt_db, psum, frames, H, W, Ch, accumulate, workspace, ws_bytes, stream, FrameSkip{});
+}
+
+extern "C" int npvp_mlpdw_mid_bwd_n2_skip(const float* da2, const float* h2, const float* mean2, const float* rstd2, const float* w2n,
+                                          const float* b2n, const float* psum2, int nparts2, float drop_p, unsigned int salt,
+                                          const unsigned long long* seed, const float* h1, const float* mean1, const float* rstd1,
+                                          const float* w1n, const float* b1n, const float* wt, float* da1, float* dwt_db,
+                                          float* psum, int frames, int H, int W, int Ch, int accumulate, float dp_p,
+                                          unsigned int dp_salt, int frames_per_sample, void* workspace, long long ws_bytes,
+                                          hipStream_t stream) {
+  NPVP_CHECK_ARG(dp_p >= 0.f && dp_p < 1.f && frames_per_sample > 0, "mlpdw_mid_bwd_n2_skip: bad drop-path arguments");
+  return mid_bwd_n2_launch(da2, h2, mean2, rstd2, w2n, b2n, psum2, nparts2, drop_p, salt, seed, h1, mean1, rstd1, w1n, b1n, wt, da1,
+                           dwt_db, psum, frames, H, W, Ch, accumulate, workspace, ws_bytes, stream,
+                           make_frame_skip(dp_p, dp_salt, frames_per_sample, seed));
 }
 
 __global__ void mid_bwd_reduce_into_kernel(const float* __restrict__ part, float* __restrict__ gw, float* __restrict__ gb, int Ch,
diff --git a/npvp_amd/csrc/norm.hip b/npvp_amd/csrc/norm.hip
--- a/npvp_amd/csrc/norm.hip
+++ b/npvp_amd/csrc/norm.hip
@@ -629,6 +629,10 @@
   const unsigned long long seed = (p.seed && (p.drop_thresh || p.dp_thresh)) ? *p.seed : 0ull;
   const float mu = p.mean[f], rs = p.rstd[f];
   const float fsc = fln_frame_scale(p, seed, f);
+  if (fsc == 0.f) {
+    if (threadIdx.x == 0) { psum[(f * FLN_PARTS + blockIdx.y) * 2] = 0.f; psum[(f * FLN_PARTS + blockIdx.y) * 2 + 1] = 0.f; }
+    return;
+  }
   float s1 = 0.f, s2 = 0.f;
   const int span = p.per_frame / FLN_PARTS, e0 = blockIdx.y * span, e1 = blockIdx.y == FLN_PARTS - 1 ? p.per_frame : e0 + span;
   for (int e = e0 + threadIdx.x * 4; e < e1; e += 512 * 4) {
@@ -664,6 +668,7 @@
     const long long g0 = f * p.per_frame + e;
     const float mu = p.mean[f], rs = p.rstd[f];
     const float fsc = fln_frame_scale(p, seed, f);
+    if (fsc == 0.f) { st4(dh + g0, make_float4(0.f, 0.f, 0.f, 0.f)); continue; }
     float a1 = 0.f, a2 = 0.f;
     for (int j = 0; j < nparts; ++j) { a1 += psum[(f * nparts + j) * 2]; a2 += psum[(f * nparts + j) * 2 + 1]; }
     a1 /= p.per_frame; a2 /= p.per_frame;
@@ -702,6 +707,10 @@
     const long long g0 = f * p.per_frame + e;
     const float mu = p.mean[f], rs = p.rstd[f];
     const float fsc = fln_frame_scale(p, seed, f);
+    if (fsc == 0.f) {
+      if (threadIdx.x == 0) { psum[(f * nblk + blockIdx.x) * 2] = 0.f; psum[(f * nblk + blockIdx.x) * 2 + 1] = 0.f; }
+      continue;
+    }
     const float4 v = ld4(p.h + g0), d = ld4(dout + g0);
     const float hx = (v.x - mu) * rs, hy = (v.y - mu) * rs, hz = (v.z - mu) * rs, hw = (v.w - mu) * rs;
     const float dx_ = d.x * fln_scale(p, seed, fsc, g0 + 0) * gelu_grad_f(hx * ww.x + bb.x);
@@ -1036,16 +1045,53 @@
   return fln_bwd_fused(p, dout, (const float*)workspace, FLN_PARTS, dh, P, frames, accumulate, amax, stream, "frameln_act_bwd: reduce launch failed");
 }
 
+static int fln_bwd_apply_launch(const float* dout, const float* h, const float* mean, const float* rstd, const float* w,
+                                const float* b, const float* psum, int nparts, float* dh, float* dw, float* db, int frames,
+                                int per_frame, int accumulate, float* amax, void* workspace, long long ws_bytes, float skip_p,
+                                unsigned int skip_salt, int frames_per_sample, const unsigned long long* seed, hipStream_t stream) {
+  NPVP_CHECK_ARG(frames > 0 && per_frame % 4 == 0 && psum && nparts > 0, "frameln_act_bwd_apply: bad arguments");
+  NPVP_CHECK_ARG(skip_p >= 0.f && skip_p < 1.f && (skip_p == 0.f || (seed && frames_per_sample > 0)), "frameln_act_bwd_apply: a skip site needs a device seed");
+  const Partials P = fln_partials(workspace, dw, db, frames, per_frame, accumulate);
+  NPVP_CHECK_ARG(workspace && ws_bytes >= P.bytes, "frameln_act_bwd_apply: workspace too small");
+  FlnParams p;
+  fill_fln(p, h, mean, rstd, w, b, nullptr, frames, per_frame, 0.f, 0u, skip_p, skip_salt, frames_per_sample, skip_p > 0.f ? seed : nullptr);
+  p.dp_inv_keep = 1.f;
+  return fln_bwd_fused(p, dout, psum, nparts, dh, P, frames, accumulate, amax, stream, "frameln_act_bwd_apply: reduce launch failed");
+}
+
 extern "C" int npvp_frameln_act_bwd_apply(const float* dout, const float* h, const float* mean, const float* rstd, const float* w,
                                           const float* b, const float* psum, int nparts, float* dh, float* dw, float* db,
                                           int frames, int per_frame, int accumulate, float* amax, void* workspace,
                                           long long ws_bytes, hipStream_t stream) {
-  NPVP_CHECK_ARG(frames > 0 && per_frame % 4 == 0 && psum && nparts > 0, "frameln_act_bwd_apply: bad arguments");
+  return fln_bwd_apply_launch(dout, h, mean, rstd, w, b, psum, nparts, dh, dw, db, frames, per_frame, accumulate, amax, workspace,
+                              ws_bytes, 0.f, 0u, 1, nullptr, stream);
+}
+
+extern "C" int npvp_frameln_act_bwd_apply_skip(const float* dout, const float* h, const float* mean, const float* rstd, const float* w,
+                                               const float* b, const float* psum, int nparts, float* dh, float* dw, float* db,
+                                               int frames, int per_frame, int accumulate, float* amax, float dp_p,
+                                               unsigned int dp_salt, int frames_per_sample, const unsigned long long* seed,
+                                               void* workspace, long long ws_bytes, hipStream_t stream) {
+  return fln_bwd_apply_launch(dout, h, mean, rstd, w, b, psum, nparts, dh, dw, db, frames, per_frame, accumulate, amax, workspace,
+                              ws_bytes, dp_p, dp_salt, frames_per_sample, seed, stream);
+}
+
+static int fln_bwd_pgrad_launch(const float* dout, const float* h, const float* mean, const float* rstd, const float* w,
+                                const float* b, float* psum, float* dw, float* db, int frames, int per_frame,
+                                float drop_p, unsigned int salt, float dp_p, unsigned int dp_salt, int frames_per_sample,
+                                const unsigned long long* seed, int accumulate, void* workspace, long long ws_bytes,
+                                bool dp_applied, hipStream_t stream) {
+  NPVP_CHECK_ARG(frames > 0 && per_frame % 1024 == 0 && psum, "frameln_act_bwd_pgrad: per_frame must be a multiple of 1024");
+  NPVP_CHECK_ARG(!dp_applied || dp_p == 0.f || seed, "frameln_act_bwd_pgrad_skip: a skip site needs a device seed");
   const Partials P = fln_partials(workspace, dw, db, frames, per_frame, accumulate);
-  NPVP_CHECK_ARG(workspace && ws_bytes >= P.bytes, "frameln_act_bwd_apply: workspace too small");
+  NPVP_CHECK_ARG(workspace && ws_bytes >= P.bytes, "frameln_act_bwd_pgrad: workspace too small");
   FlnParams p;
-  fill_fln(p, h, mean, rstd, w, b, nullptr, frames, per_frame, 0.f, 0u, 0.f, 0u, 1, nullptr);
-  return fln_bwd_fused(p, dout, psum, nparts, dh, P, frames, accumulate, amax, stream, "frameln_act_bwd_apply: reduce launch failed");
+  fill_fln(p, h, mean, rstd, w, b, nullptr, frames, per_frame, drop_p, salt, dp_p, dp_salt, frames_per_sample, seed);
+  if (dp_applied) p.dp_inv_keep = 1.f;
+  NPVP_LAUNCH(frameln_act_bwd_pgrad_kernel, dim3(per_frame / 1024, P.job.nb), dim3(256), 0, stream, p, dout, psum,
+                     P.part(), frames, P.per);
+  NPVP_CHECK_LAUNCH();
+  return finish_partials(P.job, accumulate, stream, "frameln_act_bwd_pgrad: reduce launch failed");
 }
 
 extern "C" int npvp_frameln_act_bwd_pgrad(const float* dout, const float* h, const float* mean, const float* rstd, const float* w,
@@ -1053,15 +1099,17 @@
                                           float drop_p, unsigned int salt, float dp_p, unsigned int dp_salt, int frames_per_sample,
                                           const unsigned long long* seed, int accumulate, void* workspace, long long ws_bytes,
                                           hipStream_t stream) {
-  NPVP_CHECK_ARG(frames > 0 && per_frame % 1024 == 0 && psum, "frameln_act_bwd_pgrad: per_frame must be a multiple of 1024");
-  const Partials P = fln_partials(workspace, dw, db, frames, per_frame, accumulate);
-  NPVP_CHECK_ARG(workspace && ws_bytes >= P.bytes, "frameln_act_bwd_pgrad: workspace too small");
-  FlnParams p;
-  fill_fln(p, h, mean, rstd, w, b, nullptr, frames, per_frame, drop_p, salt, dp_p, dp_salt, frames_per_sample, seed);
-  NPVP_LAUNCH(frameln_act_bwd_pgrad_kernel, dim3(per_frame / 1024, P.job.nb), dim3(256), 0, stream, p, dout, psum,
-                     P.part(), frames, P.per);
-  NPVP_CHECK_LAUNCH();
-  return finish_partials(P.job, accumulate, stream, "frameln_act_bwd_pgrad: reduce launch failed");
+  return fln_bwd_pgrad_launch(dout, h, mean, rstd, w, b, psum, dw, db, frames, per_frame, drop_p, salt, dp_p, dp_salt,
+                              frames_per_sample, seed, accumulate, workspace, ws_bytes, false, stream);
+}
+
+extern "C" int npvp_frameln_act_bwd_pgrad_skip(const float* dout, const float* h, const float* mean, const float* rstd, const float* w,
+                                               const float* b, float* psum, float* dw, float* db, int frames, int per_frame,
+                                               float drop_p, unsigned int salt, float dp_p, unsigned int dp_salt,
+                                               int frames_per_sample, const unsigned long long* seed, int accumulate, void* workspace,
+                                               long long ws_bytes, hipStream_t stream) {
+  return fln_bwd_pgrad_launch(dout, h, mean, rstd, w, b, psum, dw, db, frames, per_frame, drop_p, salt, dp_p, dp_salt,
+                              frames_per_sample, seed, accumulate, workspace, ws_bytes, true, stream);
 }
 
 extern "C" int npvp_frameln_act_bwd_reduce_job(const void* workspace, float* dw, float* db, int frames, int per_frame, int accumulate,
diff --git a/npvp_amd/ops.py b/npvp_amd/ops.py
--- a/npvp_amd/ops.py
+++ b/npvp_amd/ops.py
@@ -254,7 +254,7 @@
 
 def gemm(a_kc, b_kc, M, N, K, A, lda, B, ldb, out, bias=None, act=0, aux_in=None, aux_out=None, residual=None,
          drop=NO_DROP, alpha=1.0, colsum_a=None, b_pre=None, accumulate=False, rowstats=None, precision=None,
-         replay=False, a_amax=None, b_amax=None, c_amax=None, a_drop=NO_DROP, range_flag=None):
+         replay=False, a_amax=None, b_amax=None, c_amax=None, a_drop=NO_DROP, range_flag=None, a_drop_applied=False):
     for t in (A, B, out, bias, aux_in, aux_out, residual, colsum_a):
         if t is not None and not (t.is_cuda and t.dtype is torch.float32):
             _chk(t)
@@ -274,6 +274,12 @@
                 b_amax = amax_of(B)
         else:
             planes = None
+    entry = lib().npvp_gemm_f32
+    if a_drop_applied:
+        if DROP_PATH_SKIP and a_drop.p > 0.0 and prec == 6 and a_kc == 1 and (kid == 5 or kid == 7):
+            entry = lib().npvp_gemm_f32_skip
+        else:
+            a_drop = NO_DROP
     wsb = _gemm_ws_bytes(M, N, K)
     ws, wsn = (None, 0)
     if wsb > 0:
@@ -288,7 +294,7 @@
         probe = GemmProbe.only is None or kid in GemmProbe.only
     if probe:
         e0, e1 = probe_pair()
-    rc = lib().npvp_gemm_f32(
+    rc = entry(
         a_kc, b_kc, M, N, K, A.data_ptr(), lda, B.data_ptr(), ldb, out.data_ptr(), out.stride(0),
         None if bias is None else bias.data_ptr(), act, None if aux_in is None else aux_in.data_ptr(),
         None if aux_out is None else aux_out.data_ptr(), None if residual is None else residual.data_ptr(),
@@ -345,12 +351,13 @@
 
 
 def linear_dgrad(dy, w, act=0, aux_in=None, drop=NO_DROP, residual=None, dy_amax=None, dx_amax=None, a_drop=NO_DROP, out=None,
-                 accumulate=False):
+                 accumulate=False, a_drop_applied=False):
     R, N = dy.shape
     K = w.shape[1]
     dx = torch.empty(R, K, dtype=torch.float32, device=dy.device) if out is None else out
     return gemm(1, 0, R, K, N, dy, dy.stride(0), w, w.stride(0), dx, act=act, aux_in=aux_in, drop=drop, residual=residual,
-                b_pre=_planes(w, "D", R), replay=True, a_amax=dy_amax, c_amax=dx_amax, a_drop=a_drop, accumulate=accumulate)
+                b_pre=_planes(w, "D", R), replay=True, a_amax=dy_amax, c_amax=dx_amax, a_drop=a_drop, accumulate=accumulate,
+                a_drop_applied=a_drop_applied)
 
 
 def masked_grad(dy2, drop, w):
@@ -366,6 +373,8 @@
 
 
 DROP_PATH_IN_GEMM_ROWS = 1 << 30
+
+DROP_PATH_SKIP = True
 
 
 def linear_wgrad(dy, x, with_bias_grad=False, into=None, into_b=None, dy_amax=None, x_amax=None, a_drop=NO_DROP):
@@ -422,7 +431,8 @@
         return v and R <= cls.MAX_ROWS
 
 
-def linear_bwd(dy, x, w, b, sk, act=0, aux_in=None, drop=NO_DROP, residual=None, dy_amax=None, dx_amax=None, a_drop=NO_DROP):
+def linear_bwd(dy, x, w, b, sk, act=0, aux_in=None, drop=NO_DROP, residual=None, dy_amax=None, dx_amax=None, a_drop=NO_DROP,
+               applied=NO_DROP):
     R, N = dy.shape
     K = w.shape[1]
     has_b = b is not None
@@ -467,7 +477,11 @@
             else:
                 _S._cur.reduce.splitk_added(outs, ws, sk)
             return dx, None, None
-    dx = linear_dgrad(dy, w, act=act, aux_in=aux_in, drop=drop, residual=residual, dy_amax=dy_amax, dx_amax=dx_amax, a_drop=a_drop)
+    if applied.on and not a_drop.on:
+        dx = linear_dgrad(dy, w, act=act, aux_in=aux_in, drop=drop, residual=residual, dy_amax=dy_amax, dx_amax=dx_amax, a_drop=applied,
+                          a_drop_applied=True)
+    else:
+        dx = linear_dgrad(dy, w, act=act, aux_in=aux_in, drop=drop, residual=residual, dy_amax=dy_amax, dx_amax=dx_amax, a_drop=a_drop)
     gw, gb = _lin_grads(dy, x, w, b, sk, a_drop=a_drop)
     return dx, gw, gb
 
@@ -1088,7 +1102,7 @@
     return _Attn.apply(q, k, v, cfg)
 
 
-def _fln_bwd(dout, h, mean, rstd, w, b, frames, PF, d, dp, T, sk, psum=None, nparts=0, want_amax=True):
+def _fln_bwd(dout, h, mean, rstd, w, b, frames, PF, d, dp, T, sk, psum=None, nparts=0, want_amax=True, applied=NO_DROP):
     L = lib()
     dev = h.device
     dh = torch.empty_like(h)
@@ -1104,9 +1118,15 @@
                                      _stream()), "npvp_frameln_act_bwd")
     else:
         pe = HbmProbe.begin()
-        check(L.npvp_frameln_act_bwd_apply(_ptr(dout), _ptr(h), _ptr(mean), _ptr(rstd), _ptr(w), _ptr(b), _ptr(psum), nparts,
-                                           _ptr(dh), _ptr(dw), _ptr(db), frames, PF, mode, _ptr(slot), _ptr(ws), wsn, _stream()),
-              "npvp_frameln_act_bwd_apply")
+        if applied.on and DROP_PATH_SKIP:
+            check(L.npvp_frameln_act_bwd_apply_skip(_ptr(dout), _ptr(h), _ptr(mean), _ptr(rstd), _ptr(w), _ptr(b), _ptr(psum), nparts,
+                                                    _ptr(dh), _ptr(dw), _ptr(db), frames, PF, mode, _ptr(slot), applied.p, applied.salt,
+                                                    T, _ptr(_S._cur.rng.seed_tensor(dev)), _ptr(ws), wsn, _stream()),
+                  "npvp_frameln_act_bwd_apply_skip")
+        else:
+            check(L.npvp_frameln_act_bwd_apply(_ptr(dout), _ptr(h), _ptr(mean), _ptr(rstd), _ptr(w), _ptr(b), _ptr(psum), nparts,
+                                               _ptr(dh), _ptr(dw), _ptr(db), frames, PF, mode, _ptr(slot), _ptr(ws), wsn, _stream()),
+                  "npvp_frameln_act_bwd_apply")
         HbmProbe.end(pe, "npvp::frameln_act_bwd_fused_kernel", 4.0 * 3 * frames * PF)
     if sk:
         _reduce_partials(sk, ws, dw, db, L.npvp_frameln_act_bwd_reduce, L.npvp_frameln_act_bwd_reduce_job, "npvp_frameln_act_bwd_reduce",
@@ -1115,16 +1135,21 @@
     return dh, dw, db
 
 
-def _fln_pgrad(dout, h, mean, rstd, w, b, frames, PF, d, sk):
+def _fln_pgrad(dout, h, mean, rstd, w, b, frames, PF, d, sk, applied=NO_DROP, T=1):
     L = lib()
     dev = h.device
     psum = torch.empty(frames * (PF // 1024) * 2, dtype=torch.float32, device=dev)
     dw, db = (sk[0][0], sk[1][0]) if sk else (torch.empty_like(w), torch.empty_like(b))
     ws, wsn = _ws(L.npvp_frameln_act_bwd_workspace_bytes(frames, PF), dev)
-    seed = _S._cur.rng.seed_tensor(dev) if d.on else None
-    check(L.npvp_frameln_act_bwd_pgrad(_ptr(dout), _ptr(h), mean, rstd, _ptr(w), _ptr(b), _ptr(psum), _ptr(dw), _ptr(db),
-                                       frames, PF, d.p, d.salt, 0.0, 0, 1, _ptr(seed), _sink_mode(sk), _ptr(ws), wsn, _stream()),
-          "npvp_frameln_act_bwd_pgrad")
+    if applied.on and DROP_PATH_SKIP:
+        check(L.npvp_frameln_act_bwd_pgrad_skip(_ptr(dout), _ptr(h), mean, rstd, _ptr(w), _ptr(b), _ptr(psum), _ptr(dw), _ptr(db),
+                                                frames, PF, d.p, d.salt, applied.p, applied.salt, T, _ptr(_S._cur.rng.seed_tensor(dev)),
+                                                _sink_mode(sk), _ptr(ws), wsn, _stream()), "npvp_frameln_act_bwd_pgrad_skip")
+    else:
+        seed = _S._cur.rng.seed_tensor(dev) if d.on else None
+        check(L.npvp_frameln_act_bwd_pgrad(_ptr(dout), _ptr(h), mean, rstd, _ptr(w), _ptr(b), _ptr(psum), _ptr(dw), _ptr(db),
+                                           frames, PF, d.p, d.salt, 0.0, 0, 1, _ptr(seed), _sink_mode(sk), _ptr(ws), wsn, _stream()),
+              "npvp_frameln_act_bwd_pgrad")
     if sk:
         _reduce_partials(sk, ws, dw, db, L.npvp_frameln_act_bwd_reduce, L.npvp_frameln_act_bwd_reduce_job, "npvp_frameln_act_bwd_reduce",
                          (frames, PF, 1), True)
@@ -1286,10 +1311,13 @@
         dev = x.device
         dout = _c(dout)
         dh3, gn3w, gn3b = _fln_bwd(dout, h3, stats[4], stats[5], n3w, n3b, frames, 64 * Co, d3, dp, T, s_n3)
-        da2, gw2, gb2 = linear_bwd(dh3, a2, w2, True if has_b2 else None, s_fc2)
+        skip = DROP_PATH_SKIP and dp.on
+        dpr = Drop._like(dp, 1, 64 * T, frames // max(1, T)) if skip else NO_DROP
+        dpf = dp if skip else NO_DROP
+        da2, gw2, gb2 = linear_bwd(dh3, a2, w2, True if has_b2 else None, s_fc2, applied=dpr)
         fuse_n2 = MID_BWD_N2 and hid // 16 <= 256
         if fuse_n2:
-            psum2, gn2w, gn2b = _fln_pgrad(da2, h2, _row(stats, 2), _row(stats, 3), n2w, n2b, frames, 64 * hid, d2, s_n2)
+            psum2, gn2w, gn2b = _fln_pgrad(da2, h2, _row(stats, 2), _row(stats, 3), n2w, n2b, frames, 64 * hid, d2, s_n2, dpf, T)
         else:
             dh2, gn2w, gn2b = _fln_bwd(da2, h2, stats[2], stats[3], n2w, n2b, frames, 64 * hid, d2, NO_DROP, 1, s_n2,
                                           want_amax=False)
@@ -1302,14 +1330,25 @@
         sk_dw = ctx.sink_dw if ctx.needs_input_grad[6] and ctx.needs_input_grad[7] else None
         wmode = 2 if sk_dw else 0
         if fuse_n2:
-            seed = _S._cur.rng.seed_tensor(dev) if d2.on else None
+            seed = _S._cur.rng.seed_tensor(dev) if (d2.on or skip) else None
             pe = HbmProbe.begin()
-            check(L.npvp_mlpdw_mid_bwd_n2(_ptr(da2), _ptr(h2), _row(stats, 2), _row(stats, 3), _ptr(n2w), _ptr(n2b), _ptr(psum2),
-                                          hid // 16, d2.p, d2.salt, _ptr(seed), _ptr(h1), _row(stats, 0), _row(stats, 1), _ptr(n1w),
-                                          _ptr(n1b), _ptr(wtb), _ptr(da1), _ptr(dwtb), _ptr(psum), frames, 8, 8, hid, wmode, _ptr(ws), wsn,
-                                          _stream()), "npvp_mlpdw_mid_bwd_n2")
+            if skip:
+                check(L.npvp_mlpdw_mid_bwd_n2_skip(_ptr(da2), _ptr(h2), _row(stats, 2), _row(stats, 3), _ptr(n2w), _ptr(n2b), _ptr(psum2),
+                                                   hid // 16, d2.p, d2.salt, _ptr(seed), _ptr(h1), _row(stats, 0), _row(stats, 1),
+                                                   _ptr(n1w), _ptr(n1b), _ptr(wtb), _ptr(da1), _ptr(dwtb), _ptr(psum), frames, 8, 8, hid,
+                                                   wmode, dp.p, dp.salt, T, _ptr(ws), wsn, _stream()), "npvp_mlpdw_mid_bwd_n2_skip")
+            else:
+                check(L.npvp_mlpdw_mid_bwd_n2(_ptr(da2), _ptr(h2), _row(stats, 2), _row(stats, 3), _ptr(n2w), _ptr(n2b), _ptr(psum2),
+                                              hid // 16, d2.p, d2.salt, _ptr(seed), _ptr(h1), _row(stats, 0), _row(stats, 1), _ptr(n1w),
+                                              _ptr(n1b), _ptr(wtb), _ptr(da1), _ptr(dwtb), _ptr(psum), frames, 8, 8, hid, wmode, _ptr(ws),
+                                              wsn, _stream()), "npvp_mlpdw_mid_bwd_n2")
             HbmProbe.end(pe, "npvp::mlpdw_mid_bwd_kernel<1, true>", 4.0 * 4 * frames * 64 * hid)
             del da2, psum2
+        elif skip:
+            check(L.npvp_mlpdw_mid_bwd_skip(_ptr(dh2), _ptr(h1), _row(stats, 0), _row(stats, 1), _ptr(n1w), _ptr(n1b), _ptr(wtb), _ptr(da1),
+                                            _ptr(dwtb), _ptr(psum), frames, 8, 8, hid, wmode, dp.p, dp.salt, T,
+                                            _ptr(_S._cur.rng.seed_tensor(dev)), _ptr(ws), wsn, _stream()), "npvp_mlpdw_mid_bwd_skip")
+            del dh2
         else:
             check(L.npvp_mlpdw_mid_bwd(_ptr(dh2), _ptr(h1), _row(stats, 0), _row(stats, 1), _ptr(n1w), _ptr(n1b), _ptr(wtb), _ptr(da1),
                                        _ptr(dwtb), _ptr(psum), frames, 8, 8, hid, wmode, _ptr(ws), wsn, _stream()), "npvp_mlpdw_mid_bwd")
@@ -1322,10 +1361,10 @@
             gdww = torch.empty(hid, 1, 3, 3, dtype=torch.float32, device=dev)
             check(L.npvp_transpose(_ptr(dwtb), _ptr(gdww), 1, 9, hid, _stream()), "npvp_transpose")
             gdwb = dwtb[9]
-        dh1, gn1w, gn1b = _fln_bwd(da1, h1, stats[0], stats[1], n1w, n1b, frames, 64 * hid, NO_DROP, NO_DROP, 1, s_n1,
-                                      psum=psum, nparts=nparts)
+        dh1, gn1w, gn1b = _fln_bwd(da1, h1, stats[0], stats[1], n1w, n1b, frames, 64 * hid, NO_DROP, NO_DROP, T, s_n1,
+                                      psum=psum, nparts=nparts, applied=dpf)
         del da1
-        dx, gw1, gb1 = linear_bwd(dh1, x, w1, True if has_b1 else None, s_fc1)
+        dx, gw1, gb1 = linear_bwd(dh1, x, w1, True if has_b1 else None, s_fc1, applied=dpr)
         return (dx, dout if has_res else None, gw1, gb1, gn1w, gn1b, gdww, gdwb, gn2w, gn2b, gw2, gb2, gn3w, gn3b,
                 None, None, None, None)
 
```

Result: slower. 8177 (-2.4%).
